# mattiagualtieri/multimodal-path-omic

Hardware: AMD Instinct MI355X
Metric: slides/sec (fwd+bwd) at 15k-patch bags (higher is better)
Workload: dtype bf16; 1 GPU; MCAT medium whole model fwd+bwd+Adam, 15000x1024 bf16 patch bag + 6x256 omic tokens per slide, ces loss; parallelism=dp1, resident_windows=2, launch=hipgraph(fwd+bwd+adam), setup_replays_before_warmup=40, training_state_rewound_every=48

## Files before the change

### include/mpo_hip.h

```cpp
#ifndef MPO_HIP_H
#define MPO_HIP_H
#include <stddef.h>
#include <stdint.h>

#define MPO_ABI_VERSION 14

#ifdef __cplusplus
extern "C" {
#endif

typedef struct ihipStream_t* mpo_stream_t;

enum { MPO_F32 = 0, MPO_BF16 = 1 };

typedef struct mpo_bag_plan {
    const int32_t* wg_start;
    int32_t n_wg;
    int32_t rows_per_wg;
} mpo_bag_plan;
int mpo_coattn_target_workgroups(void);
enum { MPO_ACT_NONE_ = 0, MPO_ACT_RELU_ = 1, MPO_ACT_ELU_ = 2, MPO_ACT_TANH_ = 3, MPO_ACT_SIGMOID_ = 4 };

int mpo_abi_version(void);
const char* mpo_last_error(void);
// ... 102 lines not shown
                        mpo_stream_t stream);

int mpo_key_projection(const void* hbag_bf16, int64_t rows, int embed, const float* w_k, const float* b_k, float* kbag,
                       mpo_stream_t stream);
size_t mpo_nacagat_saved_floats(int n_slides, int n_q, int embed);
size_t mpo_nacagat_workspace_bytes(int n_slides, int n_q, int embed, int max_rows, int total_rows);
int mpo_coattn_nacagat_forward(const void* kbag, int k_dtype, const void* hbag, int bag_dtype, const int32_t* cu_rows, int n_slides,
                               int total_rows, int max_rows, const float* query, int n_q, int embed,
                               const float* in_proj_weight, const float* in_proj_bias,
                               const float* out_proj_weight, const float* out_proj_bias,
                               float drop_p, uint64_t seed, uint64_t offset, const uint64_t* rng_epoch,
                               float* q_proj, float* out, float* attn_map, float* score_maps,
                               float* saved, const mpo_bag_plan* plan ,
                               void* workspace, size_t workspace_bytes, mpo_stream_t stream);
int mpo_coattn_nacagat_backward(const void* kbag, int k_dtype, const void* hbag, int bag_dtype,
                                const int32_t* cu_rows, int n_slides, int total_rows, int max_rows,
                                const float* query, int n_q, int embed,
                                const float* in_proj_weight, const float* in_proj_bias, const float* out_proj_weight,
                                float drop_p, uint64_t seed, uint64_t offset, const uint64_t* rng_epoch,
                                const float* saved, const float* score_maps, const float* attn_map,
                                const float* d_out, const float* d_attn_map, const float* d_q_proj,
                                float* d_query, int d_query_accumulate ,
                                void* d_kbag, int dk_dtype, float* d_kbag_colsum ,
                                void* d_hbag ,
                                float* d_ctx ,
                                float* d_in_proj_weight, float* d_in_proj_bias,
                                float* d_out_proj_weight, float* d_out_proj_bias, const mpo_bag_plan* plan ,
                                void* workspace, size_t workspace_bytes, mpo_stream_t stream);

int mpo_nacagat_patch_grad(const int32_t* cu_rows, int n_slides, int total_rows, int max_rows, int n_q, int embed,
                           const float* attn_map, const float* d_ctx, const void* addend_bf16, const void* hbag_bf16,
                           void* d_bag_bf16, float relu_gate, float* d_bias, const mpo_bag_plan* plan ,
                           void* workspace, size_t workspace_bytes, mpo_stream_t stream);

int mpo_nacagat_patch_grad_fused(const int32_t* cu_rows, int n_slides, int total_rows, int max_rows, int n_q, int embed,
                                 const float* attn_map, const float* d_ctx, const void* d_kbag_bf16, const float* w_k,
                                 const void* hbag_bf16, void* d_bag_bf16, float relu_gate, float* d_bias,
                                 const mpo_bag_plan* plan , void* workspace, size_t workspace_bytes,
                                 mpo_stream_t stream);


size_t mpo_encoder_saved_floats(int n_slides, int T, int d, int ff, int heads, int layers);
size_t mpo_encoder_workspace_bytes(int n_slides, int T, int d, int ff);
uint64_t mpo_encoder_rng_span(int n_slides, int T, int d, int ff, int layers);
int mpo_encoder_forward(const float* x, int n_branches, int n_slides, int T, int d, int ff, int heads, int layers,
                        const float* const* params, float drop_p, uint64_t seed, uint64_t offset, const uint64_t* rng_epoch,
                        float* y, float* saved, mpo_stream_t stream);
int mpo_encoder_backward(const float* x, int n_branches, int n_slides, int T, int d, int ff, int heads, int layers,
                         const float* const* params, float drop_p, uint64_t seed, uint64_t offset, const uint64_t* rng_epoch,
                         const float* saved, const float* dy, float* dx, float* const* grads,
                         void* workspace, size_t workspace_bytes, mpo_stream_t stream);

size_t mpo_bag_self_attention_saved_floats(int n_bags, int M, int d, int heads);
size_t mpo_bag_self_attention_workspace_bytes(int n_bags, int M, int d, int heads);
int mpo_set_bag_self_attention_bf16x3(int enabled);
int mpo_bag_self_attention_forward(const float* qkv, int n_bags, int M, int d, int heads, float drop_p, uint64_t seed, uint64_t offset,
                                   const uint64_t* rng_epoch, float* out, float* saved, float* attn_map, mpo_stream_t stream);
int mpo_bag_self_attention_backward(const float* qkv, const float* out, const float* saved, const float* d_out, int n_bags, int M, int d,
                                    int heads, float drop_p, uint64_t seed, uint64_t offset, const uint64_t* rng_epoch, float* d_qkv,
                                    void* workspace, size_t workspace_bytes, mpo_stream_t stream);

size_t mpo_gated_pool_saved_floats(int n_slides, int L, int d);
size_t mpo_gated_pool_workspace_bytes(int n_slides, int L, int d);
uint64_t mpo_gated_pool_rng_span(int n_slides, int L, int d);
int mpo_gated_pool_forward(const float* x, int n_branches, int n_slides, int L, int d, const float* const* params,
                           float head_drop_p, float rho_drop_p, uint64_t seed, uint64_t offset, const uint64_t* rng_epoch,
                           float* scores, float* h, int h_interleaved, float* saved, mpo_stream_t stream);
int mpo_gated_pool_backward(const float* x, int n_branches, int n_slides, int L, int d, const float* const* params,
                            float head_drop_p, float rho_drop_p, const float* saved, const float* h,
                            const float* dh, int h_interleaved, const float* d_scores_ext , float* dx,
                            float* const* grads,
                            void* workspace, size_t workspace_bytes, mpo_stream_t stream);

size_t mpo_fusion_head_saved_floats(int n_slides, int hidden, int dout, int n_classes);
size_t mpo_fusion_head_workspace_bytes(int n_slides, int hidden, int dout, int n_classes);
int mpo_fusion_head_forward(const float* hcat, int n_slides, int din, int hidden, int dout, int n_classes,
                            const float* const* params, float* hazards, float* survs, float* y, float* saved,
                            mpo_stream_t stream);
int mpo_fusion_head_backward(const float* hcat, int n_slides, int din, int hidden, int dout, int n_classes,
                             const float* const* params, const float* saved, const float* hazards,
                             const float* survs, const float* y, const float* d_hazards, const float* d_survs,
                             const float* d_y, float* d_hcat, float* const* grads,
                             void* workspace, size_t workspace_bytes, mpo_stream_t stream);

int mpo_survival_head_forward(const float* logits, int n_slides, int n_classes, float* hazards, float* survs, float* y,
                              mpo_stream_t stream);
int mpo_survival_head_backward(const float* hazards, const float* survs, const float* y, const float* d_hazards,
                               const float* d_survs, const float* d_y, int n_slides, int n_classes, float* d_logits,
                               mpo_stream_t stream);

int mpo_ces_loss_forward(const float* hazards, const float* survs, const int64_t* label, const float* censorship,
                         int n_slides, int n_classes, float alpha, float eps, float* loss, float* risk, mpo_stream_t stream);
int mpo_ces_loss_backward(const float* hazards, const float* survs, const int64_t* label, const float* censorship,
                          int n_slides, int n_classes, float alpha, float eps, const float* d_loss, int d_loss_is_scalar,
                          float* d_hazards, float* d_survs, mpo_stream_t stream);

size_t mpo_fusion_head_loss_saved_floats(int n_slides, int hidden, int dout, int n_classes);
int mpo_fusion_head_loss_forward(const float* hcat, int n_slides, int din, int hidden, int dout, int n_classes,
                                 const float* const* params, const int64_t* label, const float* censorship,
                                 const float* slide_weight, float alpha, float eps, float* hazards, float* survs, float* y,
                                 float* loss, float* risk , float* saved, mpo_stream_t stream);
int mpo_fusion_head_loss_backward(const float* hcat, int n_slides, int din, int hidden, int dout, int n_classes,
                                  const float* const* params, const float* saved, float* d_hcat, float* const* grads,
                                  void* workspace, size_t workspace_bytes, mpo_stream_t stream);

int mpo_sct_loss_forward(const float* y, const int64_t* label, const float* censorship, int n_slides, int n_classes,
                         float eps, float* loss, mpo_stream_t stream);
int mpo_sct_loss_backward(const float* y, const int64_t* label, const float* censorship, int n_slides, int n_classes,
                          float eps, const float* d_loss, int d_loss_is_scalar, float* d_y, mpo_stream_t stream);
int mpo_fusion_head_sct_loss_forward(const float* hcat, int n_slides, int din, int hidden, int dout, int n_classes,
                                     const float* const* params, const int64_t* label, const float* censorship,
                                     const float* slide_weight, float eps, float* hazards, float* survs, float* y,
                                     float* loss, float* risk , float* saved, mpo_stream_t stream);

int mpo_ge_head_loss_forward(const float* h, int n_bags, int d, int n_classes, const float* const* params,
                             const int64_t* label, float* y, float* loss, mpo_stream_t stream);
int mpo_ge_head_loss_backward(const float* h, int n_bags, int d, int n_classes, const float* const* params,
                              const int64_t* label, const float* d_loss, float* d_h, float* const* grads,
                              mpo_stream_t stream);

size_t mpo_cag_saved_floats(int rows, int hidden);
size_t mpo_cag_workspace_bytes(int rows, int hidden);
int mpo_cag_forward(const float* q, const float* q_hat, int rows, int dim, int hidden, const float* const* params,
                    float* c_out, float* saved, const float* residual ,
                    float* sum_out , mpo_stream_t stream);
int mpo_cag_backward(const float* q, const float* q_hat, int rows, int dim, int hidden, const float* const* params,
                     const float* saved, const float* c_out, const float* d_c, float* d_q, int d_q_accumulate, float* d_q_hat,
                     float* const* grads, void* workspace, size_t workspace_bytes, mpo_stream_t stream);

size_t mpo_omic_snn_saved_floats(int n_slides, int n_groups, int d);
size_t mpo_omic_snn_workspace_bytes(int n_slides, int n_groups, int d);
uint64_t mpo_omic_snn_rng_span(int n_slides, int n_groups, int d);
int mpo_omic_snn_forward(const float* const* x, const int* widths, int n_groups, int n_slides, int d,
                         const float* const* params, float drop_p, uint64_t seed, uint64_t offset,
                         const uint64_t* rng_epoch, float* g_bag, float* saved, mpo_stream_t stream);
int mpo_omic_snn_backward(const float* const* x, const int* widths, int n_groups, int n_slides, int d,
                          const float* const* params, float drop_p, uint64_t seed, uint64_t offset,
                          const uint64_t* rng_epoch, const float* g_bag, const float* saved, const float* d_g_bag,
                          float* const* grads, void* workspace, size_t workspace_bytes, mpo_stream_t stream);

int mpo_coattn_splits(int n_slides, int max_rows);
int mpo_coattn_fwd_bagpass(const void* bag, int bag_dtype, const int32_t* cu_rows, int n_slides, int embed,
                           const float* qk2, float* part_ml, float* part_ctx, float* raw_logits ,
                           int n_q, int max_rows, const mpo_bag_plan* plan , mpo_stream_t stream);
int mpo_nacagat_fwd_bagpass(const float* kbag, const int32_t* cu_rows, int n_slides, int embed, const float* qs2,
                            const float* tq, float* a_map, float* g_map, int n_q, int max_rows,
                            const mpo_bag_plan* plan , mpo_stream_t stream);
int mpo_coattn_bwd_bagpass(const void* bag, int bag_dtype, const int32_t* cu_rows, int n_slides, int embed,
                           const float* qk2, const float* lse2, const float* dctx, const float* delta,
                           const float* d_attn_map , void* d_bag, float* part_dqk,
                           int n_q, int max_rows, const mpo_bag_plan* plan , mpo_stream_t stream);

#include "mpo_bag_sample.h"

#ifdef __cplusplus
}
#endif
#endif
```

### multimodal_path_omic_amd/_lib.py

```python
from __future__ import annotations

import ctypes
import os
import re
from ctypes import c_char_p, c_float, c_int, c_int64, c_size_t, c_uint64, c_void_p

import torch

_HERE = os.path.dirname(os.path.abspath(__file__))
LIB_PATH = os.path.join(_HERE, "libmpo_hip.so")
HEADER_PATH = os.path.join(os.path.dirname(_HERE), "include", "mpo_hip.h")
COMPANION_HEADER_PATHS = [os.path.join(os.path.dirname(_HERE), "include", "mpo_bag_sample.h")]

_SCALARS = {"int": c_int, "int32_t": c_int, "int64_t": c_int64, "uint64_t": c_uint64, "size_t": c_size_t, "float": c_float,
            "mpo_stream_t": c_void_p}
_DECL = re.compile(r"^[ \t]*([\w \t*]+?)[ \t]*\b(mpo_\w+)[ \t]*\(([^()]*)\)\s*;", re.M)


def _ctype(entry: str, decl: str):
    if "*" in decl or decl.rstrip().endswith("]"):
        return c_void_p
    words = [w for w in decl.split() if w != "const"]
    if not 1 <= len(words) <= 2 or words[0] not in _SCALARS:
        raise RuntimeError(f"include/mpo_hip.h: {entry}: no ctypes type for '{' '.join(decl.split())}'")
    return _SCALARS[words[0]]


def parse_header(text: str):
    version = re.search(r"^[ \t]*#[ \t]*define[ \t]+MPO_ABI_VERSION[ \t]+(\d+)[ \t]*$", text, re.M)
    text = re.sub(r"/\*.*?\*/", " ", text, flags=re.S)
    text = re.sub(r"//[^\n]*|^[ \t]*#.*$", " ", text, flags=re.M)
    signatures, parsed = {}, set()
    for m in _DECL.finditer(text):
        ret, name, args = m.groups()
        parsed.add(m.start(2))
        if ret.replace("*", " * ").split() == ["const", "char", "*"]:
            res = c_char_p
        elif "*" in ret:
            raise RuntimeError(f"include/mpo_hip.h: {name}: no ctypes type for the return type '{ret.strip()}'")
        else:
            res = _ctype(name, ret)
        signatures[name] = (res, [] if args.strip() in ("", "void") else [_ctype(name, a) for a in args.split(",")])
    for m in re.finditer(r"\b(mpo_\w+)\s*\(", text):
        if m.start(1) not in parsed:
            raise RuntimeError(f"include/mpo_hip.h: {m.group(1)}: not a whole declaration: "
                               f"'{' '.join(text[m.start():m.start() + 120].split())}'")
    constants = {}
    for body in re.findall(r"\benum\s*\{([^}]*)\}", text):
        for item in body.split(","):
            m = re.fullmatch(r"\s*(MPO_\w+)\s*=\s*(\d+)\s*", item)
            if not m:
                raise RuntimeError(f"include/mpo_hip.h: enum item '{item.strip()}' is not NAME = integer")
            constants[m.group(1)] = int(m.group(2))
    return signatures, constants, int(version.group(1)) if version else None


def _read_header():
    if not os.path.exists(HEADER_PATH):
        raise RuntimeError(f"{HEADER_PATH} is missing: the package binds libmpo_hip.so from its public header and ships "
                           "with it (repository layout: include/ beside the package)")
    with open(HEADER_PATH) as f:
        signatures, constants, version = parse_header(f.read())
    if version is None or not signatures:
        raise RuntimeError(f"{HEADER_PATH}: no MPO_ABI_VERSION / no entry declarations found")
    return signatures, constants, version


def _read_companions():
    out = {}
    for path in COMPANION_HEADER_PATHS:
        if not os.path.exists(path):
            raise RuntimeError(f"{path} is missing: include/mpo_hip.h includes it and the package binds its entries")
        with open(path) as f:
            signatures, constants, version = parse_header(f.read())
        if not signatures or constants or version is not None:
            raise RuntimeError(f"{path}: a companion header declares entries only (no enum, no MPO_ABI_VERSION)")
        for name in signatures:
            if name in _signatures or name in out:
                raise RuntimeError(f"{path}: {name} is declared twice")
        out.update(signatures)
    return out


_signatures, _constants, ABI_VERSION = _read_header()
MPO_F32, MPO_BF16 = _constants["MPO_F32"], _constants["MPO_BF16"]
ACT = {k[len("MPO_ACT_"):-1].lower(): v for k, v in _constants.items() if k.startswith("MPO_ACT_")}
OPTIM = {k[len("MPO_OPTIM_"):].lower(): v for k, v in _constants.items() if k.startswith("MPO_OPTIM_")}
GEMM_ROUTE = {k[len("MPO_GEMM_ROUTE_"):].lower(): v for k, v in _constants.items() if k.startswith("MPO_GEMM_ROUTE_")}
_companion_signatures = _read_companions()


class BagPlanC(ctypes.Structure):
    _fields_ = [("wg_start", c_void_p), ("n_wg", ctypes.c_int32), ("rows_per_wg", ctypes.c_int32)]


_REBUILD = "run `python -c 'import __graft_entry__ as g; g.build()'`"
_lib = None


def exported_symbols():
    return list(_signatures)


def companion_symbols():
    return list(_companion_signatures)


def check_abi_version(found: int, expected: int):
    if found != expected:
        raise RuntimeError(f"{LIB_PATH} reports ABI version {found}, include/mpo_hip.h describes {expected}: the library is "
                           f"stale ({_REBUILD}). There is no CPU fallback.")


def lib():
    global _lib
    if _lib is None:
        if not os.path.exists(LIB_PATH):
            raise RuntimeError(
                f"{LIB_PATH} is missing: the HIP extension has not been built ({_REBUILD}). There is no CPU fallback.")
        handle = ctypes.CDLL(LIB_PATH)
        for name, (res, args) in {**_signatures, **_companion_signatures}.items():
            fn = getattr(handle, name)
            fn.restype = res
            fn.argtypes = args
        check_abi_version(handle.mpo_abi_version(), ABI_VERSION)
        _lib = handle
    return _lib


def call(name: str, *args):
    check(getattr(lib(), name)(*args), name)


def check(rc: int, what: str):
    if rc != 0:
        msg = lib().mpo_last_error()
        raise RuntimeError(f"{what} failed (rc={rc}): {msg.decode() if msg else '?'}")


def ptr(t):
    if t is None:
        return None
    if not t.is_cuda:
        raise RuntimeError("libmpo_hip operates on GPU tensors only (got a CPU tensor); there is no CPU fallback")
    if not t.is_contiguous():
        raise RuntimeError("libmpo_hip needs contiguous tensors")
    return t.data_ptr()


def ptr_array(tensors):
    arr = (c_void_p * len(tensors))()
    for i, t in enumerate(tensors):
        arr[i] = ptr(t)
    return arr


def stream_of(t):
    return torch.cuda.current_stream(t.device).cuda_stream


def bag_dtype_code(t):
    if t.dtype == torch.float32:
        return MPO_F32
    if t.dtype == torch.bfloat16:
        return MPO_BF16
    raise RuntimeError(f"bag dtype must be float32 or bfloat16, got {t.dtype}")
```

### multimodal_path_omic_amd/csrc/capi.hip

```cpp
#include <stdarg.h>
#include <stdio.h>
#include <stdlib.h>

#include <algorithm>

#include "../../include/mpo_hip.h"
#include "coattn_tile.h"
#include "mpo_common.h"
#include "mpo_kernels.h"
#include "mpo_layout.h"

static thread_local char g_err[512] = "";

void mpo_set_error(const char* fmt, ...) {
    va_list ap;
    va_start(ap, fmt);
    vsnprintf(g_err, sizeof(g_err), fmt, ap);
    va_end(ap);
}

template <typename T> struct K1Saved { T *qs, *qk2, *ctx, *attn, *lse2; };
template <class A> K1Saved<typename A::elem> k1_saved(A& a, size_t R, size_t E) {
    return {a.floats(R * E), a.floats(R * E), a.floats(R * E), a.floats(R * E), a.floats(R)};
}
// ... 448 lines not shown
            RC(mpo_launch_bag_outer_gated(reinterpret_cast<const float*>(static_cast<const char*>(kbag) + h * half_k), cu_rows,
                                          n_slides, EH, W.ds1_map, qth, W.dg_map, tqh, static_cast<char*>(d_kbag) + h * half_dk,
                                          dk_dtype == MPO_F32, W.part_cs, n_q, splits, stream));
        BagFinish f{};
        f.part_cs = d_kbag_colsum ? W.part_cs : nullptr; f.colsum = d_kbag_colsum ? d_kbag_colsum + h * EH : nullptr; f.cs_cols = EH;
        if (h == 0) {
            f.zero[0] = d_in_w + (size_t)E * E; f.n_zero[0] = E * E;
            if (d_kbag_colsum != d_in_b + E) { f.zero[1] = d_in_b + E; f.n_zero[1] = E; }
        }
        if (one_pass) { f.part[0] = W.part; f.out[0] = W.dqt; f.part[1] = W.part2; f.out[1] = W.dtq; f.n_red = 2; }
        RC(mpo_launch_bag_finish(f, n_slides, n_q, EH, splits, stream));
    }
    if (one_pass) RC(query_side());
    if (d_ctx == nullptr)
        for (int h = 0; h < NH; ++h)
            RC(mpo_launch_bag_outer(cu_rows, n_slides, EH, attn_map, NH > 1 ? hb[h] : dctx, nullptr, nullptr,
                                    static_cast<char*>(d_hbag) + h * half_h, f32, n_q, splits, stream));
    return 0;
}

struct K2PatchGrad {
    BagPlan splits;
    float* part_cs;
};
static int k2_patch_grad_begin(K2PatchGrad& pg, int n_slides, int max_rows, int embed, bool colsum, const mpo_bag_plan* plan_,
                               void* workspace, size_t workspace_bytes) {
    pg.splits = make_plan(plan_, n_slides, max_rows);
    RC(check_plan(pg.splits, n_slides));
    WsCarve ws(workspace, workspace_bytes);
    pg.part_cs = k2_patch_grad_ws(ws, plan_parts(pg.splits), embed, colsum);
    MPO_CHECK(ws.ok(), "nacagat patch grad: workspace too small (%zu bytes)", workspace_bytes);
    return 0;
}
static int k2_patch_grad_end(const K2PatchGrad& pg, float* d_bias, int embed, hipStream_t stream) {
    return d_bias ? mpo_launch_colsum(pg.part_cs, d_bias, (int)plan_parts(pg.splits), embed, embed, 0, stream) : 0;
}

int mpo_nacagat_patch_grad(const int32_t* cu_rows, int n_slides, int total_rows, int max_rows, int n_q, int embed,
                           const float* attn_map, const float* d_ctx, const void* addend_bf16, const void* hbag_bf16,
                           void* d_bag_bf16, float relu_gate, float* d_bias, const mpo_bag_plan* plan_,
                           void* workspace, size_t workspace_bytes, mpo_stream_t stream) {
    RC(check_common(MPO_BF16, n_slides, total_rows, max_rows, n_q, embed));
    MPO_CHECK(attn_map && d_ctx && addend_bf16 && hbag_bf16 && d_bag_bf16, "nacagat patch grad: null operand");
    MPO_CHECK(((reinterpret_cast<uintptr_t>(addend_bf16) | reinterpret_cast<uintptr_t>(hbag_bf16) |
                reinterpret_cast<uintptr_t>(d_bag_bf16)) & 15) == 0, "nacagat patch grad: bag operands must be 16-byte aligned");
    K2PatchGrad pg;
    RC(k2_patch_grad_begin(pg, n_slides, max_rows, embed, d_bias != nullptr, plan_, workspace, workspace_bytes));
    RC(mpo_launch_bag_outer_gate(cu_rows, n_slides, embed, attn_map, d_ctx, addend_bf16, hbag_bf16, d_bag_bf16, relu_gate,
                                 pg.part_cs, n_q, pg.splits, stream));
    return k2_patch_grad_end(pg, d_bias, embed, stream);
}

int mpo_nacagat_patch_grad_fused(const int32_t* cu_rows, int n_slides, int total_rows, int max_rows, int n_q, int embed,
                                 const float* attn_map, const float* d_ctx, const void* d_kbag_bf16, const float* w_k,
                                 const void* hbag_bf16, void* d_bag_bf16, float relu_gate, float* d_bias,
                                 const mpo_bag_plan* plan_, void* workspace, size_t workspace_bytes, mpo_stream_t stream) {
    RC(check_common(MPO_BF16, n_slides, total_rows, max_rows, n_q, embed));
    MPO_CHECK(attn_map && d_ctx && d_kbag_bf16 && w_k && hbag_bf16 && d_bag_bf16, "nacagat patch grad: null operand");
    MPO_CHECK(d_bag_bf16 != d_kbag_bf16, "nacagat patch grad (fused): d_bag must not alias d_kbag");
    MPO_CHECK(((reinterpret_cast<uintptr_t>(d_kbag_bf16) | reinterpret_cast<uintptr_t>(hbag_bf16) |
                reinterpret_cast<uintptr_t>(d_bag_bf16)) & 15) == 0, "nacagat patch grad: bag operands must be 16-byte aligned");
    K2PatchGrad pg;
    RC(k2_patch_grad_begin(pg, n_slides, max_rows, embed, d_bias != nullptr, plan_, workspace, workspace_bytes));
    RC(mpo_launch_k2_patch_grad(cu_rows, d_kbag_bf16, w_k, attn_map, d_ctx, hbag_bf16, d_bag_bf16, relu_gate, pg.part_cs, n_q, embed,
                                pg.splits, stream));
    return k2_patch_grad_end(pg, d_bias, embed, stream);
}

int mpo_coattn_fwd_bagpass(const void* bag, int bag_dtype, const int32_t* cu_rows, int n_slides, int embed,
                           const float* qk2, float* part_ml, float* part_ctx, float* raw_logits, int n_q, int max_rows,
                           const mpo_bag_plan* plan_, mpo_stream_t stream) {
    const BagPlan plan = make_plan(plan_, n_slides, max_rows);
    RC(check_plan(plan, n_slides));
    return mpo_launch_coattn_fwd_partial(bag, bag_dtype == MPO_F32, cu_rows, n_slides, embed, qk2, part_ml, part_ctx,
                                         raw_logits, n_q, plan, stream);
}
int mpo_map_block_dot(const float* a_map, const float* b_map, const int32_t* cu_rows, int n_slides, int n_q, float* out,
                      mpo_stream_t stream) {
    MPO_CHECK(a_map && b_map && cu_rows && out && n_slides >= 1 && n_q >= 1, "map block dot: bad argument");
    return mpo_launch_map_rowdot(a_map, b_map, cu_rows, out, n_slides, n_q, 0, stream);
}
int mpo_map_block_scale(const float* a_map, const float* scale, const int32_t* cu_rows, int n_slides, int n_q, float* out,
                        mpo_stream_t stream) {
    MPO_CHECK(a_map && scale && cu_rows && out && n_slides >= 1 && n_q >= 1, "map block scale: bad argument");
    return mpo_launch_map_block_scale(a_map, scale, cu_rows, out, n_slides, n_q, stream);
}
int mpo_key_projection(const void* hbag_bf16, int64_t rows, int embed, const float* w_k, const float* b_k, float* kbag,
                       mpo_stream_t stream) {
    MPO_CHECK(rows >= 1 && rows <= 0x7fffffff, "key projection: %lld rows out of range", (long long)rows);
    return mpo_launch_key_proj(hbag_bf16, w_k, b_k, kbag, (int)rows, embed, stream);
}
int mpo_nacagat_fwd_bagpass(const float* kbag, const int32_t* cu_rows, int n_slides, int embed, const float* qs2,
                            const float* tq, float* a_map, float* g_map, int n_q, int max_rows, const mpo_bag_plan* plan_,
                            mpo_stream_t stream) {
    const BagPlan plan = make_plan(plan_, n_slides, max_rows);
    RC(check_plan(plan, n_slides));
    return mpo_launch_bag_rowdot_gated(kbag, 1, cu_rows, n_slides, embed, qs2, tq, a_map, g_map, n_q, plan, stream);
}
int mpo_coattn_bwd_bagpass(const void* bag, int bag_dtype, const int32_t* cu_rows, int n_slides, int embed,
                           const float* qk2, const float* lse2, const float* dctx, const float* delta,
                           const float* d_attn_map, void* d_bag, float* part_dqk, int n_q, int max_rows,
                           const mpo_bag_plan* plan_, mpo_stream_t stream) {
    const BagPlan plan = make_plan(plan_, n_slides, max_rows);
    RC(check_plan(plan, n_slides));
    MPO_CHECK(delta, "coattn backward bag pass: delta is required here");
    return mpo_launch_coattn_bwd(bag, bag_dtype == MPO_F32, cu_rows, n_slides, embed, qk2, lse2, dctx, delta, nullptr, nullptr,
                                 d_attn_map, d_bag, part_dqk, nullptr, n_q, plan, 0.f, stream);
}

int mpo_patch_epilogue_forward(void* h_bf16, const float* bias, int64_t rows, int cols, float drop_p, uint64_t seed,
                               uint64_t offset, const uint64_t* rng_epoch, mpo_stream_t stream) {
    MPO_CHECK(h_bf16 && bias, "patch epilogue: null operand");
    MPO_CHECK(rows >= 0, "patch epilogue: %lld rows", (long long)rows);
    MPO_CHECK(((reinterpret_cast<uintptr_t>(h_bf16) | reinterpret_cast<uintptr_t>(bias)) & 15) == 0,
              "patch epilogue: h and bias must be 16-byte aligned");
    return mpo_launch_bias_relu_dropout_bf16(h_bf16, bias, (size_t)rows, cols, drop_p, seed, offset,
                                             reinterpret_cast<const unsigned long long*>(rng_epoch), stream);
}
int mpo_colsum_bf16(const void* x_bf16, float* out, int64_t rows, int cols, mpo_stream_t stream) {
    MPO_CHECK(x_bf16 && out, "bf16 column sum: null operand");
    MPO_CHECK(rows >= 0, "bf16 column sum: %lld rows", (long long)rows);
    MPO_CHECK((reinterpret_cast<uintptr_t>(x_bf16) & 15) == 0, "bf16 column sum: x must be 16-byte aligned (bf16 x 8 loads)");
    return mpo_launch_colsum_bf16(x_bf16, out, (size_t)rows, cols, stream);
}
size_t mpo_patch_epilogue_backward_workspace_bytes(int64_t n, int cols) { return one_block_workspace_bytes(patch_epilogue_bwd_floats(n, cols)); }
int mpo_patch_epilogue_backward(const void* h_bf16, const void* dy_bf16, void* g_bf16, int64_t n, int cols, float drop_p,
                                float* d_bias, void* workspace, size_t workspace_bytes, mpo_stream_t stream) {
    MPO_CHECK(h_bf16 && dy_bf16 && g_bf16, "patch epilogue backward: null operand");
    MPO_CHECK(((reinterpret_cast<uintptr_t>(h_bf16) | reinterpret_cast<uintptr_t>(dy_bf16) |
                reinterpret_cast<uintptr_t>(g_bf16)) & 15) == 0,
              "patch epilogue backward: h, dy and g must be 16-byte aligned (bf16 x 8 loads)");
    if (!d_bias) return mpo_launch_relu_dropout_bwd_bf16(h_bf16, dy_bf16, g_bf16, (size_t)n, drop_p, cols, nullptr, stream);
    WsCarve ws(workspace, workspace_bytes);
    float* part = ws.floats(patch_epilogue_bwd_floats(n, cols));
    MPO_CHECK(workspace && ws.ok(), "patch epilogue backward: workspace too small (%zu bytes)", workspace_bytes);
    RC(mpo_launch_relu_dropout_bwd_bf16(h_bf16, dy_bf16, g_bf16, (size_t)n, drop_p, cols, part, stream));
    return mpo_launch_colsum(part, d_bias, mpo_relu_dropout_bwd_blocks((size_t)n, 1), cols, cols, 0, stream);
}

size_t mpo_patch_weight_grad_workspace_bytes(int embed, int patch_dim) {
    return one_block_workspace_bytes(mpo_patch_wgrad_partial_floats(embed, patch_dim));
}
int mpo_patch_weight_grad(const void* g_bf16, const void* patches_bf16, int64_t total_rows, int embed, int patch_dim,
                          float* d_weight, int workgroups, void* workspace, size_t workspace_bytes, mpo_stream_t stream) {
    MPO_CHECK(g_bf16 && patches_bf16 && d_weight, "patch weight gradient: null argument");
    MPO_CHECK(total_rows >= 1 && total_rows < (int64_t)1 << 31, "patch weight gradient: %lld rows", (long long)total_rows);
    WsCarve ws(workspace, workspace_bytes);
    float* part = ws.floats(mpo_patch_wgrad_partial_floats(embed, patch_dim));
    MPO_CHECK(ws.ok(), "patch weight gradient: workspace too small (%zu bytes)", workspace_bytes);
    return mpo_launch_patch_wgrad(g_bf16, patches_bf16, total_rows, embed, patch_dim, part, d_weight, workgroups,
                                  static_cast<hipStream_t>(stream));
}

int mpo_adam_step_flat(float* params, const float* grads, float* exp_avg, float* exp_avg_sq, int64_t n, float lr,
                       float beta1, float beta2, float eps, float weight_decay, int step, const int32_t* step_dev,
                       mpo_stream_t stream) {
    MPO_CHECK(step >= 1 || step_dev, "adam: step counts from 1 (got %d)", step);
    return mpo_launch_adam_flat(params, grads, exp_avg, exp_avg_sq, (size_t)n, lr, beta1, beta2, eps, weight_decay,
                                step < 1 ? 1 : step, step_dev, stream);
}

int mpo_optim_step_flat(int algorithm, float* params, const float* grads, float* state1, float* state2, int64_t n, float lr,
                        const float* lr_dev, float beta1, float beta2, float eps, float weight_decay, float l1, int step,
                        const int32_t* step_dev, mpo_stream_t stream) {
    MPO_CHECK(algorithm >= MPO_OPTIM_ADAM && algorithm <= MPO_OPTIM_SGD, "flat optimiser: unknown algorithm %d", algorithm);
    MPO_CHECK(n >= 0, "flat optimiser: n = %lld", (long long)n);
    MPO_CHECK(params && grads, "flat optimiser: null parameter or gradient buffer");
    const bool stateful = algorithm != MPO_OPTIM_SGD;
    MPO_CHECK(!stateful || (state1 && state2), "flat optimiser: algorithm %d needs both state buffers", algorithm);
    const auto misaligned = [](const void* q) { return (reinterpret_cast<uintptr_t>(q) & 3u) != 0; };
    MPO_CHECK(!misaligned(params) && !misaligned(grads) && !misaligned(state1) && !misaligned(state2) && !misaligned(lr_dev) &&
              !misaligned(step_dev), "flat optimiser: buffers must be 4-byte aligned");
    const bool counted = algorithm == MPO_OPTIM_ADAM || algorithm == MPO_OPTIM_ADAMAX;
    MPO_CHECK(!counted || step >= 1 || step_dev, "flat optimiser: step counts from 1 (got %d)", step);
    return mpo_launch_optim_flat(algorithm, params, grads, state1, state2, (size_t)n, lr, lr_dev, beta1, beta2, eps,
                                 weight_decay, l1, step < 1 ? 1 : step, step_dev, static_cast<hipStream_t>(stream));
}
size_t mpo_abs_sum_flat_workspace_bytes(int64_t n) {
    return n < 0 ? 0 : mpo_abs_sum_partials((size_t)n) * sizeof(float);
}
int mpo_abs_sum_flat(const float* x, int64_t n, float* out, void* workspace, size_t workspace_bytes, mpo_stream_t stream) {
    MPO_CHECK(n >= 1, "abs sum: n = %lld", (long long)n);
    MPO_CHECK(x && out && workspace, "abs sum: null argument");
    MPO_CHECK((reinterpret_cast<uintptr_t>(x) & 3u) == 0 && (reinterpret_cast<uintptr_t>(out) & 3u) == 0 &&
              (reinterpret_cast<uintptr_t>(workspace) & 3u) == 0, "abs sum: pointers must be 4-byte aligned");
    MPO_CHECK(workspace_bytes >= mpo_abs_sum_flat_workspace_bytes(n), "abs sum: workspace too small (%zu bytes)",
              workspace_bytes);
    return mpo_launch_abs_sum(x, (size_t)n, static_cast<float*>(workspace), out, static_cast<hipStream_t>(stream));
}

int mpo_set_gemm_fast_path(int enabled) { return mpo_gemm_fast_path(enabled); }
int mpo_gemm_last_route(void) { return mpo_gemm_route_last(); }
int mpo_gemm_last_group_routes(void) { return mpo_gemm_route_group_take(); }
int mpo_set_coattn_bwd_two_wave(int enabled) { return mpo_coattn_bwd8_enable(enabled); }
int mpo_set_coattn_bwd_f32_vector(int enabled) { return mpo_coattn_bwd_f32_enable(enabled); }
int mpo_set_nacagat_one_pass_key_grad(int enabled) {
    const int was = g_k2_one_pass_key ? 1 : 0;
    g_k2_one_pass_key = enabled != 0;
    return was;
}

int mpo_step_counters_bump(uint64_t* rng_epoch, int32_t* adam_step, mpo_stream_t stream) {
    MPO_CHECK(rng_epoch || adam_step, "step counters: nothing to bump");
    return mpo_launch_counters_bump(reinterpret_cast<unsigned long long*>(rng_epoch), adam_step, static_cast<hipStream_t>(stream));
}

}
```

### multimodal_path_omic_amd/csrc/gemm_f32.hip

```cpp
#include "../../include/mpo_hip.h"
#include "mpo_common.h"
#include "mpo_kernels.h"
#include "gemm_f32_gate.h"

namespace {

constexpr int DB = 16;
constexpr int DMAXB = 8;
}
void mpo_direct_single_nb4(const GemmArgs& g, int layout, dim3 grid, hipStream_t stream);
void mpo_direct_single_nb8(const GemmArgs& g, int layout, dim3 grid, hipStream_t stream);
void mpo_direct_group_nb4(const GemmGroup& grp, dim3 grid, hipStream_t stream);
void mpo_direct_group_nb8(const GemmGroup& grp, dim3 grid, hipStream_t stream);
void mpo_fast_group(const GemmGroup& grp, int gate_classes, int nbmax, dim3 grid, hipStream_t stream);
void mpo_fast_single(const GemmArgs& g, int layout, int gate_classes, int nbmax, dim3 grid, hipStream_t stream);
void mpo_rows_single(const GemmArgs& g, int layout, int gate_class, hipStream_t stream);
int mpo_longk_single(const GemmArgs& g, int gate_class, hipStream_t stream);
namespace {
inline int direct_nbmax(int k) { return k <= 256 ? 4 : DMAXB; }
bool g_fast_path = true;
int g_last_route = MPO_GEMM_ROUTE_NONE;
int g_group_routes = 0;
inline bool aligned16(const void* p) { return (reinterpret_cast<uintptr_t>(p) & 15) == 0; }
inline int gate_class(const GemmArgs& g, bool need_aligned_gate) {
    const bool gate_ok = g.gate != nullptr && (!need_aligned_gate || aligned16(g.gate));
    switch (g.gate_mode) {
        case MPO_GATE_NONE: return 0;
        case MPO_GATE_RNG: return 2;
        case MPO_GATE_RELU: case MPO_GATE_ELU: case MPO_GATE_TANH: case MPO_GATE_SIGMOID: case MPO_GATE_MUL: return gate_ok ? 1 : -1;
        case MPO_GATE_ELU_ADROP: return gate_ok ? 3 : -1;
        default: return -1;
    }
}
inline int fast_class(const GemmArgs& g) {
    if (!g_fast_path) return -1;
    if (g.M <= 0 || g.N <= 0 || (g.M & 15) || (g.N & 15) || g.K < 16 || (g.K & 15)) return -1;
    if ((g.lda & 3) || (g.ldb & 3) || !aligned16(g.A) || !aligned16(g.B)) return -1;
    return gate_class(g, true);
}
inline int rows_class(const GemmArgs& g, int layout) {
    if (!g_fast_path || !(layout & 2) || g.M < 512 || (g.N & 63) || g.K < 64 || (g.K & 63) || g.bias_grad != nullptr) return -1;
    if ((g.lda & 3) || !aligned16(g.A)) return -1;
    if ((layout & 1) && ((g.ldb & 3) || !aligned16(g.B))) return -1;
    return gate_class(g, true);
}
inline int longk_class(const GemmArgs& g, int layout) {
    if (!g_fast_path || layout != 0 || g.K < 2048 || (g.M & 31) || (g.N & 63) || (g.lda & 3)) return -1;
    if (g.bias || g.mask || g.residual || g.act != MPO_ACT_NONE || g.drop_p > 0.f) return -1;
    return gate_class(g, false);
}
inline void launch_longk(const GemmArgs& g, int gate_class, hipStream_t stream) {
    if (int e = mpo_longk_single(g, gate_class, stream)) mpo_set_error("long-K weight gradient: zero-fill failed (hip error %d)", e);
}
void launch_direct_single(const GemmArgs& g, int layout, dim3 grid, hipStream_t stream) {
    const int rc = rows_class(g, layout);
    if (rc >= 0) { g_last_route = MPO_GEMM_ROUTE_ROWS; mpo_rows_single(g, layout, rc, stream); return; }
    const int lc = longk_class(g, layout);
    if (lc >= 0) { g_last_route = MPO_GEMM_ROUTE_LONGK; launch_longk(g, lc, stream); return; }
    const int fc = fast_class(g);
    if (fc >= 0) { g_last_route = MPO_GEMM_ROUTE_FAST; mpo_fast_single(g, layout, fc, direct_nbmax(g.K), grid, stream); return; }
    if (direct_nbmax(g.K) == 4) { g_last_route = MPO_GEMM_ROUTE_GENERAL_NB4; mpo_direct_single_nb4(g, layout, grid, stream); }
    else { g_last_route = MPO_GEMM_ROUTE_GENERAL_NB8; mpo_direct_single_nb8(g, layout, grid, stream); }
}
inline bool group_extent(const GemmGroup& grp, dim3& grid) {
    int mx = 0, nx = 0;
    for (int i = 0; i < grp.n; ++i) { mx = std::max(mx, grp.g[i].M); nx = std::max(nx, grp.g[i].N); }
    grid = dim3((nx + DB - 1) / DB, (mx + DB - 1) / DB, grp.n);
    return mx > 0 && nx > 0;
}
void launch_direct_group(const GemmGroup& all, dim3 grid, hipStream_t stream) {
    GemmGroup grp;
    grp.n = 0;
    for (int i = 0; i < all.n; ++i) {
        const int rc = rows_class(all.g[i], all.g[i].layout), lc = longk_class(all.g[i], all.g[i].layout);
        if (rc >= 0) { g_group_routes |= 1 << MPO_GEMM_ROUTE_ROWS; mpo_rows_single(all.g[i], all.g[i].layout, rc, stream); }
        else if (lc >= 0) { g_group_routes |= 1 << MPO_GEMM_ROUTE_LONGK; launch_longk(all.g[i], lc, stream); }
        else grp.g[grp.n++] = all.g[i];
    }
    if (grp.n == 0) return;
    if (grp.n != all.n) group_extent(grp, grid);
    int kmax = 0, classes = 0;
    bool fast = true;
    for (int i = 0; i < grp.n; ++i) {
        kmax = grp.g[i].K > kmax ? grp.g[i].K : kmax;
        const int fc = fast_class(grp.g[i]);
        fast = fast && fc >= 0;
        if (fc > 0) classes |= 1 << fc;
    }
    fast = fast && (classes & (classes - 1)) == 0;
    const size_t wgs = (size_t)grid.x * grid.y * grid.z;
    const int nb = (wgs > 1024 || direct_nbmax(kmax) == 4) ? 4 : DMAXB;
    g_group_routes |= 1 << (fast ? MPO_GEMM_ROUTE_FAST : nb == 4 ? MPO_GEMM_ROUTE_GENERAL_NB4 : MPO_GEMM_ROUTE_GENERAL_NB8);
    if (fast) { mpo_fast_group(grp, classes >> 3 ? 3 : classes >> 2 ? 2 : 1, nb, grid, stream); return; }
    if (nb == 4) mpo_direct_group_nb4(grp, grid, stream);
    else mpo_direct_group_nb8(grp, grid, stream);
}

__global__ __launch_bounds__(256)
void colsum_kernel(const float* __restrict__ x, float* __restrict__ out, int M, int N, int ld, int accumulate) {
    __shared__ float red[16][17];
    const int c = threadIdx.x & 15, rg = threadIdx.x >> 4;
    const int n = blockIdx.x * 16 + c;
    float s = 0.f;
    if (n < N)
        for (int m = rg; m < M; m += 16) s += x[(size_t)m * ld + n];
    red[rg][c] = s;
    __syncthreads();
    if (rg == 0 && n < N) {
        float t = 0.f;
#pragma unroll
        for (int k = 0; k < 16; ++k) t += red[k][c];
        out[n] = accumulate ? out[n] + t : t;
    }
}

}

int mpo_gemm_fast_path(int enabled) {
    const int was = g_fast_path ? 1 : 0;
    g_fast_path = enabled != 0;
    return was;
}

int mpo_gemm_route_last() { return g_last_route; }
int mpo_gemm_route_group_take() {
    const int was = g_group_routes;
    g_group_routes = 0;
    return was;
}

int mpo_launch_gemm(const GemmArgs& g, int a_kc, int b_kc, hipStream_t stream) {
    if (g.M <= 0 || g.N <= 0) return 0;
    MPO_CHECK(g.K > 0, "gemm: K must be positive (got %d)", g.K);
    dim3 dgrid((g.N + DB - 1) / DB, (g.M + DB - 1) / DB);
    launch_direct_single(g, 2 * (a_kc ? 1 : 0) + (b_kc ? 1 : 0), dgrid, stream);
    MPO_LAUNCH_CHECK();
    return 0;
}

static int launch_group(const char* what, GemmGroup grp, int layout, hipStream_t stream) {
    MPO_CHECK(grp.n >= 1 && grp.n <= 8, "%s: 1..8 members (got %d)", what, grp.n);
    for (int i = 0; i < grp.n; ++i) {
        MPO_CHECK(grp.g[i].K > 0, "%s: member %d has K = %d", what, i, grp.g[i].K);
        if (layout >= 0) grp.g[i].layout = layout;
        else MPO_CHECK(grp.g[i].layout >= 0 && grp.g[i].layout <= 3, "%s: member %d has layout %d", what, i, grp.g[i].layout);
    }
    dim3 dgrid;
    if (!group_extent(grp, dgrid)) return 0;
    launch_direct_group(grp, dgrid, stream);
    MPO_LAUNCH_CHECK();
    return 0;
}
int mpo_launch_gemm_group(const GemmGroup& grp, int a_kc, int b_kc, hipStream_t stream) {
    return launch_group("grouped gemm", grp, 2 * (a_kc ? 1 : 0) + (b_kc ? 1 : 0), stream);
}
int mpo_launch_gemm_mixed(const GemmGroup& grp, hipStream_t stream) { return launch_group("mixed grouped gemm", grp, -1, stream); }

int mpo_launch_colsum(const float* x, float* out, int M, int N, int ld, int accumulate, hipStream_t stream) {
    if (N <= 0) return 0;
    colsum_kernel<<<(N + 15) / 16, 256, 0, stream>>>(x, out, M, N, ld, accumulate);
    MPO_LAUNCH_CHECK();
    return 0;
}
```

### multimodal_path_omic_amd/csrc/gemm_f32_fast.h

```cpp
#pragma once
#include "gemm_f32_gate.h"

namespace {

constexpr int FB = 16;

struct FastLds {
    float part[4][256];
    float bsum[4][16];
};


template <bool KC>
__device__ __forceinline__ f32x4 fast_frag(const float* __restrict__ p, int ld, int mn, int k0) {
    if (KC) return *reinterpret_cast<const f32x4*>(p + (size_t)mn * ld + k0);
    f32x4 r;
#pragma unroll
    for (int j = 0; j < 4; ++j) r[j] = p[(size_t)(k0 + j) * ld + mn];
    return r;
}

template <bool A_KC, bool B_KC, int GC>
struct FastCtx {
    const GemmArgs& g;
    const GateFn& gf;
    int m, n, kq, lane;
    bool want_bsum;
    template <int NB>
    __device__ __forceinline__ void chunk(int kbase, f32x4& acc0, f32x4& acc1, float& bsum) const {
        f32x4 a[NB], b[NB], gv[NB];
#pragma unroll
        for (int u = 0; u < NB; ++u) {
            const int k0 = kbase + 16 * u + 4 * kq;
            a[u] = fast_frag<A_KC>(g.A, g.lda, m, k0);
            b[u] = fast_frag<B_KC>(g.B, g.ldb, n, k0);
            if (GC == 1 || GC == 3) gv[u] = fast_frag<A_KC>(gf.g, g.lda, m, k0);
        }
#pragma unroll
        for (int u = 0; u < NB; ++u) {
            const int k0 = kbase + 16 * u + 4 * kq;
            if (GC == 1) {
#pragma unroll
                for (int j = 0; j < 4; ++j) a[u][j] *= gf(gv[u][j], 0);
            } else if (GC >= 2) {
                if (A_KC) {
                    const uint64_t ctr = gf.off + (((size_t)m * g.lda + k0) >> 2);
                    const uint4 r = draw4x32((uint32_t)ctr, (uint32_t)(ctr >> 32), (uint32_t)gf.seed, (uint32_t)(gf.seed >> 32));
                    const uint32_t w[4] = {r.x, r.y, r.z, r.w};
#pragma unroll
                    for (int j = 0; j < 4; ++j) a[u][j] *= gf.with_word(GC == 3 ? gv[u][j] : 0.f, w[j]);
                } else {
                    const int lq = lane & 3;
                    const size_t idx_own = (size_t)(k0 + lq) * g.lda + (m & ~3);
                    const uint64_t ctr = gf.off + (idx_own >> 2);
                    const uint4 r = draw4x32((uint32_t)ctr, (uint32_t)(ctr >> 32), (uint32_t)gf.seed, (uint32_t)(gf.seed >> 32));
                    const uint32_t own[4] = {r.x, r.y, r.z, r.w};
                    uint32_t w[4];
#pragma unroll
                    for (int t = 0; t < 4; ++t) {
                        const int pick = lq ^ t;
                        const uint32_t send = pick == 0 ? own[0] : pick == 1 ? own[1] : pick == 2 ? own[2] : own[3];
                        const uint32_t got = (uint32_t)__shfl_xor((int)send, t);
#pragma unroll
                        for (int j = 0; j < 4; ++j) if (j == (lq ^ t)) w[j] = got;
                    }
#pragma unroll
                    for (int j = 0; j < 4; ++j) a[u][j] *= gf.with_word(GC == 3 ? gv[u][j] : 0.f, w[j]);
                }
            }
            if (want_bsum) bsum += (a[u][0] + a[u][1]) + (a[u][2] + a[u][3]);
            acc0 = __builtin_amdgcn_mfma_f32_16x16x4f32(a[u][0], b[u][0], acc0, 0, 0, 0);
            acc1 = __builtin_amdgcn_mfma_f32_16x16x4f32(a[u][1], b[u][1], acc1, 0, 0, 0);
            acc0 = __builtin_amdgcn_mfma_f32_16x16x4f32(a[u][2], b[u][2], acc0, 0, 0, 0);
            acc1 = __builtin_amdgcn_mfma_f32_16x16x4f32(a[u][3], b[u][3], acc1, 0, 0, 0);
        }
    }
};

template <bool A_KC, bool B_KC, int GC, int NBMAX>
__device__ __forceinline__ void gemm_f32_fast_body(const GemmArgs& g, FastLds& lds) {
    if ((int)blockIdx.y * FB >= g.M || (int)blockIdx.x * FB >= g.N) return;
    const int tid = threadIdx.x, lane = tid & 63, wave = __builtin_amdgcn_readfirstlane(tid >> 6);
    const int m0 = blockIdx.y * FB, n0 = blockIdx.x * FB;
    const int i16 = lane & 15, kq = lane >> 4;
    GateFn gf;
    gf.g = g.gate; gf.mode = g.gate_mode; gf.p = g.gate_p; gf.seed = g.gate_seed;
    gf.off = epoch_offset(g.gate_off, g.rng_epoch);
    gf.inv_keep = g.gate_p > 0.f ? 1.0f / (1.0f - g.gate_p) : 1.0f;
    const bool want_bsum = g.bias_grad != nullptr && blockIdx.x == 0;

    const int erow = tid >> 4, ecol = tid & 15;
    const size_t eo = (size_t)(m0 + erow) * g.ldc + n0 + ecol;
    const float e_bias = g.bias ? g.bias[n0 + ecol] : 0.f;
    const float e_mask = g.mask ? g.mask[eo] : 1.0f;
    const float e_res = g.residual ? g.residual[eo] : 0.f;
    const float e_old = g.accumulate ? g.C[eo] : 0.f;
    float e_keep = 1.0f;
    if (g.drop_p > 0.f) {
        const unsigned long long doff = epoch_offset(g.drop_off, g.rng_epoch);
        e_keep = dropout_keep(g.drop_seed, doff, eo, g.drop_p, g.alpha_dropout ? 1.0f : 1.0f / (1.0f - g.drop_p));
    }

    const int kw = ((g.K + 63) >> 6) << 4;
    const int kbeg = wave * kw;
    const int nkb = max(0, min(kw, g.K - kbeg)) >> 4;
    f32x4 acc0 = {0.f, 0.f, 0.f, 0.f}, acc1 = acc0;
    float bsum = 0.f;
    FastCtx<A_KC, B_KC, GC> cx{g, gf, m0 + i16, n0 + i16, kq, lane, want_bsum};
    int kb = 0;
    for (; kb + NBMAX <= nkb; kb += NBMAX) cx.template chunk<NBMAX>(kbeg + 16 * kb, acc0, acc1, bsum);
    const int rem = nkb - kb;
    if (rem >= 4) { cx.template chunk<4>(kbeg + 16 * kb, acc0, acc1, bsum); kb += 4; }
    switch (nkb - kb) {
        case 3: cx.template chunk<3>(kbeg + 16 * kb, acc0, acc1, bsum); break;
        case 2: cx.template chunk<2>(kbeg + 16 * kb, acc0, acc1, bsum); break;
        case 1: cx.template chunk<1>(kbeg + 16 * kb, acc0, acc1, bsum); break;
        default: break;
    }
#pragma unroll
    for (int r = 0; r < 4; ++r) lds.part[wave][(4 * kq + r) * 16 + i16] = acc0[r] + acc1[r];
    if (want_bsum) {
        bsum += __shfl_xor(bsum, 16);
        bsum += __shfl_xor(bsum, 32);
        if (lane < 16) lds.bsum[wave][lane] = bsum;
    }
    __syncthreads();
    {
        float v = (lds.part[0][tid] + lds.part[1][tid]) + (lds.part[2][tid] + lds.part[3][tid]);
        v = (v + e_bias) * g.alpha;
        v = apply_act(v, g.act);
        if (g.drop_p > 0.f) {
            if (g.alpha_dropout) v = alpha_drop_a(g.drop_p) * (e_keep != 0.f ? v : kAlphaPrime) + alpha_drop_b(g.drop_p);
            else v *= e_keep;
        }
        v = v * e_mask + e_res + e_old;
        g.C[eo] = v;
    }
    if (want_bsum && tid < FB)
        g.bias_grad[m0 + tid] = (lds.bsum[0][tid] + lds.bsum[1][tid]) + (lds.bsum[2][tid] + lds.bsum[3][tid]);
}

template <bool A_KC, bool B_KC, int GCL, int NBMAX>
__device__ __forceinline__ void gemm_f32_fast_member(const GemmArgs& g, FastLds& lds) {
    if (g.gate_mode == MPO_GATE_NONE) gemm_f32_fast_body<A_KC, B_KC, 0, NBMAX>(g, lds);
    else gemm_f32_fast_body<A_KC, B_KC, GCL, NBMAX>(g, lds);
}

template <int GCL, int NBMAX>
__global__ __launch_bounds__(256) __attribute__((amdgpu_waves_per_eu((GCL == 2 && NBMAX == 4) ? 6 : 1, 8)))
void gemm_f32_fast_group_kernel(GemmGroup grp) {
    __shared__ FastLds lds;
    const GemmArgs& g = grp.g[blockIdx.z];
    switch (g.layout) {
        case 3: gemm_f32_fast_member<true, true, GCL, NBMAX>(g, lds); break;
        case 2: gemm_f32_fast_member<true, false, GCL, NBMAX>(g, lds); break;
        case 1: gemm_f32_fast_member<false, true, GCL, NBMAX>(g, lds); break;
        default: gemm_f32_fast_member<false, false, GCL, NBMAX>(g, lds); break;
    }
}
template <bool A_KC, bool B_KC, int GCL, int NBMAX>
__global__ __launch_bounds__(256)
void gemm_f32_fast_single_kernel(GemmArgs g) {
    __shared__ FastLds lds;
    gemm_f32_fast_member<A_KC, B_KC, GCL, NBMAX>(g, lds);
}

}
```

### multimodal_path_omic_amd/csrc/mpo_kernels.h

```cpp
#pragma once
#include <hip/hip_runtime.h>
#include <stddef.h>

#include <stdint.h>
enum { MPO_ACT_NONE = 0, MPO_ACT_RELU = 1, MPO_ACT_ELU = 2, MPO_ACT_TANH = 3, MPO_ACT_SIGMOID = 4 };
enum { MPO_GATE_NONE = 0, MPO_GATE_RELU = 1, MPO_GATE_ELU = 2, MPO_GATE_TANH = 3, MPO_GATE_SIGMOID = 4,
       MPO_GATE_RNG = 5, MPO_GATE_MUL = 6, MPO_GATE_ELU_ADROP = 7 };

struct GemmArgs {
    const float* A = nullptr;
    const float* B = nullptr;
    float* C = nullptr;
    const float* bias = nullptr;
    const float* residual = nullptr;
    const float* mask = nullptr;
    int M = 0, N = 0, K = 0;
    int lda = 0, ldb = 0, ldc = 0;
    float alpha = 1.0f;
    int act = MPO_ACT_NONE;
    int accumulate = 0;
    int alpha_dropout = 0;
    float drop_p = 0.f;
    uint64_t drop_seed = 0, drop_off = 0;
    const float* gate = nullptr;
    int gate_mode = MPO_GATE_NONE;
    float gate_p = 0.f;
    uint64_t gate_seed = 0, gate_off = 0;
    float* bias_grad = nullptr;
    const unsigned long long* rng_epoch = nullptr;
    int layout = 3;
};

struct DropSpec {
    float p = 0.f;
    uint64_t seed = 0, off = 0;
    const unsigned long long* epoch = nullptr;
};
struct GateSpec {
    const float* g = nullptr;
    int mode = MPO_GATE_NONE;
    float p = 0.f;
    uint64_t seed = 0, off = 0;
    const unsigned long long* epoch = nullptr;
};

int mpo_launch_gemm(const GemmArgs& g, int a_kc, int b_kc, hipStream_t stream);
struct GemmGroup {
    GemmArgs g[8];
    int n = 0;
};
int mpo_launch_gemm_group(const GemmGroup& grp, int a_kc, int b_kc, hipStream_t stream);
int mpo_launch_gemm_mixed(const GemmGroup& grp, hipStream_t stream);
int mpo_launch_colsum(const float* x, float* out, int M, int N, int ld, int accumulate, hipStream_t stream);

inline GemmArgs mpo_args_fwd(const float* x, const float* w, const float* b, float* y, int R, int I, int O,
                             float alpha, int act, const float* residual = nullptr, DropSpec drop = DropSpec()) {
    GemmArgs g;
    g.A = x; g.B = w; g.C = y; g.bias = b; g.residual = residual;
    g.M = R; g.N = O; g.K = I; g.lda = I; g.ldb = I; g.ldc = O; g.alpha = alpha; g.act = act;
    g.drop_p = drop.p; g.drop_seed = drop.seed; g.drop_off = drop.off; g.rng_epoch = drop.epoch;
    g.layout = 3;
    return g;
}
inline int mpo_linear_fwd(const float* x, const float* w, const float* b, float* y, int R, int I, int O,
                          float alpha, int act, hipStream_t s, const float* residual = nullptr,
                          DropSpec drop = DropSpec()) {
    return mpo_launch_gemm(mpo_args_fwd(x, w, b, y, R, I, O, alpha, act, residual, drop), 1, 1, s);
}
inline GemmArgs mpo_args_bwd_input(const float* dy, const float* w, float* dx, int R, int I, int O, float alpha,
                                   int accumulate, GateSpec gate = GateSpec()) {
    GemmArgs g;
    g.A = dy; g.B = w; g.C = dx;
    g.M = R; g.N = I; g.K = O; g.lda = O; g.ldb = I; g.ldc = I; g.alpha = alpha; g.accumulate = accumulate;
    g.gate = gate.g; g.gate_mode = gate.mode; g.gate_p = gate.p; g.gate_seed = gate.seed; g.gate_off = gate.off;
    g.rng_epoch = gate.epoch;
    g.layout = 2;
    return g;
}
inline int mpo_linear_bwd_input(const float* dy, const float* w, float* dx, int R, int I, int O, float alpha,
                                int accumulate, hipStream_t s, GateSpec gate = GateSpec()) {
    return mpo_launch_gemm(mpo_args_bwd_input(dy, w, dx, R, I, O, alpha, accumulate, gate), 1, 0, s);
}
inline GemmArgs mpo_args_bwd_weight(const float* dy, const float* x, float* dw, float* db, int R, int I, int O,
                                    float alpha, GateSpec gate = GateSpec()) {
    GemmArgs g;
    g.A = dy; g.B = x; g.C = dw;
    g.M = O; g.N = I; g.K = R; g.lda = O; g.ldb = I; g.ldc = I; g.alpha = alpha;
    g.gate = gate.g; g.gate_mode = gate.mode; g.gate_p = gate.p; g.gate_seed = gate.seed; g.gate_off = gate.off;
    g.rng_epoch = gate.epoch;
    g.bias_grad = db;
    g.layout = 0;
    return g;
}
inline int mpo_linear_bwd_weight(const float* dy, const float* x, float* dw, float* db, int R, int I, int O,
                                 float alpha, hipStream_t s, GateSpec gate = GateSpec()) {
    return mpo_launch_gemm(mpo_args_bwd_weight(dy, x, dw, db, R, I, O, alpha, gate), 0, 0, s);
}
inline int mpo_linear_bwd_pair(const GemmArgs& dx, const GemmArgs& dw, hipStream_t s) {
    GemmGroup grp;
    grp.g[0] = dx; grp.g[1] = dw; grp.n = 2;
    return mpo_launch_gemm_mixed(grp, s);
}
inline int mpo_gemm_together(hipStream_t s, const GemmArgs& a, const GemmArgs& b, const GemmArgs* c = nullptr,
                             const GemmArgs* d = nullptr) {
    GemmGroup grp;
    grp.g[0] = a; grp.g[1] = b; grp.n = 2;
    if (c) grp.g[grp.n++] = *c;
    if (d) grp.g[grp.n++] = *d;
    return mpo_launch_gemm_mixed(grp, s);
}

struct BagPlan;
extern "C" int mpo_coattn_splits(int n_slides, int max_rows);
int mpo_launch_pack_patch_weight(const float* w, void* out, int embed, int patch_dim, hipStream_t stream);
int mpo_launch_patch_fc_fwd(const void* x, const void* w_packed, const float* bias, const int* cu, void* h_out, int embed, int patch_dim,
                            float drop_p, unsigned long long seed, unsigned long long offset, const unsigned long long* epoch,
                            const BagPlan& plan, hipStream_t stream);
int mpo_launch_coattn_fwd_partial(const void* bag, int bag_f32, const int* cu, int n_slides, int embed,
                                  const float* qk2, float* part_ml, float* part_ctx, float* s_out,
                                  int n_q, const BagPlan& plan, hipStream_t stream);
int mpo_launch_coattn_combine(const float* part_ml, const float* part_ctx, float* ctx, float* lse2,
                              int n_slides, int n_q, int embed, const BagPlan& plan, hipStream_t stream);
int mpo_launch_coattn_normalize(float* a, const float* lse2, const int* cu, int n_slides, int n_q, int max_rows,
                                float drop_p, unsigned long long seed, unsigned long long offset, hipStream_t stream);
int mpo_launch_coattn_bwd(const void* bag, int bag_f32, const int* cu, int n_slides, int embed,
                          const float* qk2, const float* lse2, const float* dctx, const float* delta ,
                          const float* ctx, const float* a_map, const float* da_map,
                          void* dbag, float* part_dqk, float* part_colsum , int n_q, const BagPlan& plan,
                          float relu_gate, hipStream_t stream);
bool mpo_coattn_bwd8_covers(int bag_f32, int embed, int n_q, const float* da_map);
int mpo_coattn_bwd_f32_enable(int enabled);
bool mpo_coattn_bwd_f32_covers(int bag_f32, int embed, int n_q, const float* da_map);
int mpo_launch_coattn_bwd_f32(const void* bag, const int* cu, const float* qk2, const float* lse2, const float* dctx,
                              const float* delta, const float* ctx, const float* da_map, void* dbag, float* part_dqk,
                              float* part_colsum, int n_q, const BagPlan& plan, hipStream_t stream);
int mpo_coattn_bwd8_enable(int enabled);
int mpo_launch_coattn_bwd8(const void* bag, const int* cu, const float* qk2, const float* lse2, const float* dctx,
                           const float* delta, const float* ctx, void* dbag, float* part_dqk, float* part_colsum, int n_q,
                           const BagPlan& plan, float relu_gate, hipStream_t stream);
size_t mpo_patch_fc_f32_workspace_floats();
size_t mpo_patch_wgrad_f32_workspace_floats();
int mpo_launch_patch_fc_f32(const float* x, const float* w, const float* bias, float* h, long long total_rows, int embed,
                            int patch_dim, float drop_p, unsigned long long seed, unsigned long long offset,
                            const unsigned long long* epoch, float x_scale, float* ws, hipStream_t stream);
int mpo_launch_patch_wgrad_f32(const float* dh, const float* hbag, const float* x, long long total_rows, int embed, int patch_dim,
                               float gate, float* d_weight, float* d_bias, float* ws, hipStream_t stream);
int mpo_launch_k2_patch_grad(const int* cu, const void* dk_bf16, const float* w_k, const float* amap, const float* dctx,
                             const void* hbag_bf16, void* out_bf16, float gate, float* part_colsum, int n_q, int embed,
                             const BagPlan& plan, hipStream_t stream);
int mpo_gemm_fast_path(int enabled);
int mpo_gemm_route_last();
int mpo_gemm_route_group_take();
size_t mpo_patch_wgrad_partial_floats(int embed, int patch_dim);
int mpo_launch_patch_wgrad(const void* g_bf16, const void* x_bf16, int64_t total_rows, int embed, int patch_dim, float* part,
                           float* d_weight, int workgroups, hipStream_t stream);
struct BagFinish {
    const float* part[2];
    float* out[2];
    int n_red;
    const float* part_cs;
    float* colsum;
    int cs_cols;
    float* zero[2];
    int n_zero[2];
};
int mpo_launch_bag_finish(const BagFinish& f, int n_slides, int n_q, int embed, const BagPlan& plan, hipStream_t stream);
int mpo_launch_coattn_bwd_reduce(const float* part_dqk, float* dqk, int n_slides, int n_q, int embed, const BagPlan& plan,
                                 hipStream_t stream);
int mpo_launch_rowdot(const float* a, const float* b, float* out, int rows, int cols, hipStream_t stream);
int mpo_launch_map_block_scale(const float* a_map, const float* scale, const int* cu, float* out, int n_slides, int n_q,
                               hipStream_t stream);
int mpo_launch_map_rowdot(const float* a_map, const float* da_map, const int* cu, float* delta, int n_slides, int n_q,
                          int accumulate, hipStream_t stream);

int mpo_launch_bag_rowdot(const void* bag, int bag_f32, const int* cu, int n_slides, int embed, const float* r,
                          float* map, float alpha, int n_q, const BagPlan& plan, hipStream_t stream);
int mpo_launch_bag_colacc(const void* bag, int bag_f32, const int* cu, int n_slides, int embed, const float* wmap,
                          float* part, int n_q, const BagPlan& plan, hipStream_t stream);
int mpo_launch_bag_outer(const int* cu, int n_slides, int embed, const float* w1, const float* z1, const float* w2,
                         const float* z2, void* dx, int out_f32, int n_q, const BagPlan& plan, hipStream_t stream);
int mpo_launch_gated_softmax_fwd(const float* amap_a, const float* gmap, const int* cu, float* out_map, float* lse2,
                                 float* asum, int n_slides, int n_q, float drop_p, unsigned long long seed,
                                 unsigned long long offset, const unsigned long long* epoch, hipStream_t stream);
int mpo_launch_gated_softmax_bwd(const float* amap_a, const float* gmap, const int* cu, const float* lse2,
                                 const float* dasum, const float* d_ext, float* da_map, float* dg_map, int n_slides,
                                 int n_q, float drop_p, unsigned long long seed, unsigned long long offset,
                                 const unsigned long long* epoch, hipStream_t stream);
int mpo_launch_qprep(const float* q, float* qt, float* qs2, float* tq, int n, float c_nat, hipStream_t stream);
int mpo_launch_qprep_bwd(const float* dqt, const float* dtq, const float* tq, const float* d_ext, float* dq, int n,
                         float c_nat, hipStream_t stream);
int mpo_launch_row_scaled_bias(float* y, const float* s, const float* bias, int rows, int cols, hipStream_t stream);

constexpr int kMaxBranches = 4;
struct LnBranches {
    const float* w[kMaxBranches] = {};
    const float* b[kMaxBranches] = {};
    float* dw[kMaxBranches] = {};
    float* db[kMaxBranches] = {};
    int rows_per_branch = 0, n = 0;
};
int mpo_launch_ln_fwd_br(const float* x, const LnBranches& p, float* y, float* stats, int rows, int d, float eps, hipStream_t s);
int mpo_launch_ln_bwd_br(const float* dy, const float* x, const float* stats, const LnBranches& p, float* dx, int rows, int d,
                         int accumulate, int what, hipStream_t s);
int mpo_launch_ln_bwd_params_only(const float* dy, const float* x, const float* stats, float* dw, float* db, int rows, int d,
                                  hipStream_t s);
constexpr int kSmallAttnMaxT = 16;
// ... 95 lines not shown
```

### multimodal_path_omic_amd/csrc/patch_wgrad.hip

```cpp
#include "coattn_tile.h"
#include "mpo_kernels.h"

namespace {

constexpr int WG_E = 256;
constexpr int WG_CB = 256;
constexpr int WG_BK = 32;
constexpr int WG_STAGES = 4;
constexpr int WG_TILE = WG_BK * 512;
constexpr int WG_STAGE = 2 * WG_TILE;
constexpr int WG_LDS = WG_STAGES * WG_STAGE;
constexpr int WG_WAVES = 8;
constexpr int WG_WGS = 256;

__device__ __forceinline__ void wait_vm(int n) {
    switch (n) {
        case 0: __builtin_amdgcn_s_waitcnt(0x0F70); break;
        case 4: __builtin_amdgcn_s_waitcnt(0x0F74); break;
        default: __builtin_amdgcn_s_waitcnt(0x0F78); break;
    }
}

__global__ __launch_bounds__(WG_WAVES * 64, 1)
void patch_wgrad_kernel(const __bf16* __restrict__ g, const __bf16* __restrict__ x, int total_rows, int patch_dim,
                        int g_dim,
                        int e_rows,
                        int rows_per_range, float* __restrict__ part) {
    using G = TileGeom<WG_E>;
    __shared__ __attribute__((aligned(1024))) char lds[WG_LDS];
    const int lane = threadIdx.x & 63;
    const int wave = __builtin_amdgcn_readfirstlane(threadIdx.x >> 6);
    const int n_cb = patch_dim < WG_CB ? 1 : patch_dim / WG_CB;
    const int xcd = blockIdx.x & 7, slot = blockIdx.x >> 3;
    const int rr = xcd + 8 * (slot / n_cb), cb = slot % n_cb;
    const int rb = min(total_rows, rr * rows_per_range), re = min(total_rows, rb + rows_per_range);
    const int n_chunks = (re - rb + WG_BK - 1) / WG_BK;

    const bool x_tile = wave >= 4;
    const char* src_base = x_tile ? reinterpret_cast<const char*>(x) + (size_t)cb * WG_CB * 2 : reinterpret_cast<const char*>(g);
    const size_t src_row = x_tile ? (size_t)patch_dim * 2 : (size_t)g_dim * 2;
    const int cmask = x_tile ? (patch_dim < WG_CB ? patch_dim / 8 - 1 : 31) : e_rows / 8 - 1;
    const unsigned src_row32 = (unsigned)src_row;
    auto issue = [&](int chunk) {
        char* stage = lds + (chunk % WG_STAGES) * WG_STAGE + (x_tile ? WG_TILE : 0);
#pragma unroll
        for (int i = 0; i < 4; ++i) {
            const int k = 4 * (wave & 3) + i;
            const int r = 2 * k + (lane >> 5), cs = lane & 31;
            const int c = (cs ^ ((r & 7) << 1)) & cmask;
            const int grow = min(rb + chunk * WG_BK + r, total_rows - 1);
            const unsigned off = (unsigned)grow * src_row32 + (unsigned)(c * 16);
            const unsigned dst = (unsigned)(uintptr_t)(__attribute__((address_space(3))) char*)(stage + k * 1024);
#pragma clang diagnostic push
#pragma clang diagnostic ignored "-Winline-asm"
            asm volatile("s_mov_b32 m0, %2\n\ts_nop 0\n\tglobal_load_lds_dwordx4 %0, %1"
                         :: "v"(off), "s"(src_base), "s"(dst) : "memory", "m0");
#pragma clang diagnostic pop
        }
    };

    const int wm = wave & 3, wn = wave >> 2;
    f32x4 acc[4][8];
#pragma unroll
    for (int i = 0; i < 4; ++i)
#pragma unroll
        for (int j = 0; j < 8; ++j) acc[i][j] = f32x4{0.f, 0.f, 0.f, 0.f};

    auto arrive = [&](int m) {
        wait_vm(4 * min(WG_STAGES - 2, n_chunks - 1 - m));
        asm volatile("" ::: "memory");
        char* stage = lds + (m % WG_STAGES) * WG_STAGE;
        if (!x_tile && rb + (m + 1) * WG_BK > re) {
#pragma unroll
            for (int i = 0; i < 4; ++i) {
                const int k = 4 * (wave & 3) + i;
                const int r = 2 * k + (lane >> 5);
                if (rb + m * WG_BK + r >= re)
                    *reinterpret_cast<f32x4*>(stage + k * 1024 + lane * 16) = f32x4{0.f, 0.f, 0.f, 0.f};
            }
        }
        asm volatile("s_waitcnt lgkmcnt(0)\n\ts_barrier" ::: "memory");
        if (m + WG_STAGES - 1 < n_chunks) issue(m + WG_STAGES - 1);
    };
    auto load_frags = [&](int m, bf16x8 (&fa)[4], bf16x8 (&fb)[8]) {
        const char* gt = lds + (m % WG_STAGES) * WG_STAGE;
        const char* xt = gt + WG_TILE;
#pragma unroll
        for (int i = 0; i < 4; ++i) fa[i] = col_frag<WG_E>(gt, 4 * wm + i, lane);
#pragma unroll
        for (int j = 0; j < 8; ++j) fb[j] = col_frag<WG_E>(xt, 8 * wn + j, lane);
    };
    auto mma = [&](const bf16x8 (&fa)[4], const bf16x8 (&fb)[8]) {
#pragma unroll
        for (int j = 0; j < 8; ++j)
#pragma unroll
            for (int i = 0; i < 4; ++i) acc[i][j] = mfma_bf16(fa[i], fb[j], acc[i][j]);
    };

    for (int c = 0; c < min(WG_STAGES - 1, n_chunks); ++c) issue(c);
    bf16x8 pa[4], pb[8], qa[4], qb[8];
    if (n_chunks > 0) {
        arrive(0);
        load_frags(0, pa, pb);
    }
    int n = 0;
    auto half = [&](int m, bf16x8 (&la)[4], bf16x8 (&lb)[8], const bf16x8 (&ca)[4], const bf16x8 (&cb_)[8]) {
        __builtin_amdgcn_s_waitcnt(0x0F78);
        asm volatile("s_waitcnt lgkmcnt(0)\n\ts_barrier" ::: "memory");
        load_frags(m, la, lb);
        mma(ca, cb_);
        issue(m + WG_STAGES - 1);
#pragma unroll
        for (int k = 0; k < 24; ++k) {
            __builtin_amdgcn_sched_group_barrier(0x008, 1, 0);
            __builtin_amdgcn_sched_group_barrier(0x100, 1, 0);
        }
        __builtin_amdgcn_sched_group_barrier(0x008, 8, 0);
    };
    for (; n + 5 < n_chunks; n += 2) {
        half(n + 1, qa, qb, pa, pb);
        half(n + 2, pa, pb, qa, qb);
    }
    for (; n < n_chunks; n += 2) {
        if (n + 1 < n_chunks) {
            arrive(n + 1);
            load_frags(n + 1, qa, qb);
        }
        mma(pa, pb);
        if (n + 1 < n_chunks) {
            if (n + 2 < n_chunks) {
                arrive(n + 2);
                load_frags(n + 2, pa, pb);
            }
            mma(qa, qb);
        }
    }
    if (64 * wm >= e_rows || 128 * wn >= patch_dim) return;
    float* out = part + ((size_t)rr * e_rows) * patch_dim + (size_t)cb * WG_CB;
#pragma unroll
    for (int i = 0; i < 4; ++i)
#pragma unroll
        for (int j = 0; j < 8; ++j)
#pragma unroll
            for (int r = 0; r < 4; ++r)
                out[(size_t)(16 * (4 * wm + i) + 4 * (lane >> 4) + r) * patch_dim + 16 * (8 * wn + j) + (lane & 15)] = acc[i][j][r];
}

__global__ __launch_bounds__(256)
void patch_wgrad_reduce_kernel(const float* __restrict__ part, float* __restrict__ out, int n4, int n_parts, int accumulate) {
    const int i = blockIdx.x * 256 + threadIdx.x;
    if (i >= n4) return;
    f32x4 a = {0.f, 0.f, 0.f, 0.f};
    if (accumulate) a = *reinterpret_cast<const f32x4*>(out + (size_t)i * 4);
#pragma unroll 8
    for (int s = 0; s < n_parts; ++s) a += *reinterpret_cast<const f32x4*>(part + ((size_t)s * n4 + i) * 4);
    *reinterpret_cast<f32x4*>(out + (size_t)i * 4) = a;
}

}

size_t mpo_patch_wgrad_partial_floats(int embed, int patch_dim) {
    const int n_cb = patch_dim / WG_CB > 0 ? patch_dim / WG_CB : 1;
    return (size_t)(WG_WGS / n_cb) * (embed < WG_E ? embed : WG_E) * patch_dim;
}

int mpo_launch_patch_wgrad(const void* g, const void* x, int64_t total_rows, int embed, int patch_dim, float* part, float* d_weight,
                           int workgroups, hipStream_t stream) {
    MPO_CHECK((embed == 128 || embed == 256 || embed == 512) &&
              (patch_dim == 128 || (patch_dim >= WG_CB && patch_dim % WG_CB == 0 && (256 % (patch_dim / WG_CB)) == 0)),
              "patch weight gradient: built for embed in {128, 256, 512} and patch_dim in {128, 256, 512, 1024, 2048} (got %d, %d)", embed, patch_dim);
    MPO_CHECK(total_rows >= 1, "patch weight gradient: no rows");
    MPO_CHECK(((reinterpret_cast<uintptr_t>(g) | reinterpret_cast<uintptr_t>(x)) & 15) == 0, "patch weight gradient: operands must be 16-byte aligned");
    const int n_cb = patch_dim < WG_CB ? 1 : patch_dim / WG_CB;
    MPO_CHECK(workgroups == 0 || (workgroups >= 8 * n_cb && workgroups <= WG_WGS && workgroups % (8 * n_cb) == 0),
              "patch weight gradient: workgroups must be 0 or a multiple of %d up to %d (got %d)", 8 * n_cb, WG_WGS, workgroups);
    const int ranges = (workgroups ? workgroups : WG_WGS) / n_cb;
    const int e_rows = embed < WG_E ? embed : WG_E;
    const int wide = patch_dim > embed ? patch_dim : embed;
    const int64_t seg_rows = ((((int64_t)1 << 32) - 1) / ((int64_t)wide * 2)) / WG_BK * WG_BK;
    const __bf16* gb = static_cast<const __bf16*>(g);
    const __bf16* xb = static_cast<const __bf16*>(x);
    for (int64_t s0 = 0; s0 < total_rows; s0 += seg_rows) {
        const int rows = (int)(total_rows - s0 < seg_rows ? total_rows - s0 : seg_rows);
        const int rpr = ((rows + ranges - 1) / ranges + WG_BK - 1) / WG_BK * WG_BK;
        for (int c0 = 0; c0 < embed; c0 += WG_E) {
            patch_wgrad_kernel<<<ranges * n_cb, WG_WAVES * 64, 0, stream>>>(gb + (size_t)s0 * embed + c0, xb + (size_t)s0 * patch_dim, rows, patch_dim,
                                                                          embed, e_rows, rpr, part);
            MPO_LAUNCH_CHECK();
            const int n4 = e_rows * patch_dim / 4;
            patch_wgrad_reduce_kernel<<<(n4 + 255) / 256, 256, 0, stream>>>(part, d_weight + (size_t)c0 * patch_dim, n4, ranges, s0 > 0);
            MPO_LAUNCH_CHECK();
        }
    }
    return 0;
}
```

### multimodal_path_omic_amd/csrc/tail_api.hip

```cpp
#include <algorithm>
#include <vector>

#include "../../include/mpo_hip.h"
#include "mpo_common.h"
#include "mpo_kernels.h"
#include "mpo_layout.h"

namespace {

using SavedCount = Count<kPad64>;

inline DropSpec stream_of(float p, uint64_t seed, uint64_t base, uint64_t stride, int k, const uint64_t* epoch) {
    DropSpec d;
    d.p = p; d.seed = seed; d.off = base + stride * (uint64_t)k;
    d.epoch = reinterpret_cast<const unsigned long long*>(epoch);
    return d;
}
inline GateSpec gate(const float* g, int mode, float p = 0.f) {
    GateSpec s;
    s.g = g; s.mode = mode; s.p = p;
    return s;
}
inline GateSpec gate_rng(DropSpec d) {
    GateSpec s;
    s.mode = d.p > 0.f ? MPO_GATE_RNG : MPO_GATE_NONE; s.p = d.p; s.seed = d.seed; s.off = d.off; s.epoch = d.epoch;
    return s;
}

#define PAIR(dxa, dwa) RC(mpo_linear_bwd_pair((dxa), (dwa), stream))

enum { P_INW, P_INB, P_OUTW, P_OUTB, P_L1W, P_L1B, P_L2W, P_L2B, P_N1W, P_N1B, P_N2W, P_N2B, P_PER_LAYER };

template <typename T> struct EncLayerSaved { T *qkv, *psave, *o, *s1, *st1, *x1, *f, *s2, *st2, *x2; };
template <typename C>
void enc_carve(C& c, EncLayerSaved<typename C::elem>* out, int B, int T, int d, int ff, int H) {
    const size_t R = (size_t)B * T;
    EncLayerSaved<typename C::elem> s;
    s.qkv = c.floats(R * 3 * d);
    s.psave = c.floats(T <= kSmallAttnMaxT ? (size_t)B * 2 * H * T * T : mpo_bag_sa_saved_floats(B, T, d, H));
    s.o = c.floats(R * d);
    s.s1 = c.floats(R * d); s.st1 = c.floats(2 * R); s.x1 = c.floats(R * d); s.f = c.floats(R * ff);
    s.s2 = c.floats(R * d); s.st2 = c.floats(2 * R); s.x2 = c.floats(R * d);
    if (out) *out = s;
}
struct EncLayerWs { float *ds2, *df, *dx1, *ds1, *dob, *dqkv, *din, *sa; };
template <typename C>
void enc_bwd_ws(C& c, EncLayerWs* W, int layers, size_t R, size_t d, size_t ff, size_t sa_floats) {
    for (int l = layers - 1; l >= 0; --l)
        W[l] = {c.floats(R * d), c.floats(R * ff), c.floats(R * d), c.floats(R * d), c.floats(R * d), c.floats(R * 3 * d),
                l == 0 ? nullptr : c.floats(R * d), sa_floats ? c.floats(sa_floats) : nullptr};
}
inline uint64_t enc_stream_stride(int B, int T, int d, int ff) {
    const uint64_t R = (uint64_t)B * T;
    const uint64_t m = R * (uint64_t)(ff > 3 * d ? ff : 3 * d);
    return m / 4 + 2;
}

template <typename T> struct PoolSaved { T *a, *b, *ab, *w, *hpool; };
template <class A> PoolSaved<typename A::elem> pool_saved(A& c, size_t B, size_t L, size_t d) {
    const size_t R = B * L;
    return {c.floats(R * d), c.floats(R * d), c.floats(R * d), c.floats(R), c.floats(B * d)};
}
struct PoolWs { float *dhpool, *dscores, *dab, *da, *db; };
template <class A> PoolWs pool_ws(A& c, size_t B, size_t L, size_t d) {
    const size_t R = B * L;
    return {c.floats(B * d), c.floats(R), c.floats(R * d), c.floats(R * d), c.floats(R * d)};
}
inline uint64_t pool_stream_stride(uint64_t B, uint64_t L, uint64_t d) { return B * L * d / 4 + 2 + kMaxBranches; }

template <typename T> struct HeadSaved { T *z1, *z2, *logits, *dlogits; };
template <class A> HeadSaved<typename A::elem> head_saved(A& c, size_t B, size_t hidden, size_t dout, size_t n_classes, bool with_loss) {
    return {c.floats(B * hidden), c.floats(B * dout), c.floats(B * n_classes), with_loss ? c.floats(B * n_classes) : nullptr};
}
struct HeadWs { float *dlogits, *dz2, *dz1; };
template <class A> HeadWs head_ws(A& c, size_t B, size_t hidden, size_t dout, size_t n_classes) {
    return {c.floats(B * n_classes), c.floats(B * dout), c.floats(B * hidden)};
}

template <typename T> struct CagSaved { T *u1, *u2, *u3, *t1, *t3, *g, *e, *m, *sg, *se; };
template <class A> CagSaved<typename A::elem> cag_saved(A& c, size_t rows, size_t hidden) {
    const size_t n = rows * hidden;
    return {c.floats(n), c.floats(n), c.floats(n), c.floats(n), c.floats(n), c.floats(n), c.floats(n), c.floats(n),
            c.floats(2 * rows), c.floats(2 * rows)};
}
struct CagWs { float *dm, *dG, *dE, *ds12, *ds3; };
template <class A> CagWs cag_ws(A& c, size_t rows, size_t hidden) {
    const size_t n = rows * hidden;
    return {c.floats(n), c.floats(n), c.floats(n), c.floats(n), c.floats(n)};
}

template <class A> std::vector<typename A::elem*> snn_blocks(A& c, int n_groups, size_t n_slides, size_t d) {
    std::vector<typename A::elem*> b(n_groups > 0 ? n_groups : 0);
    for (auto& p : b) p = c.floats(n_slides * d);
    return b;
}
inline uint64_t snn_stream_stride(uint64_t n_slides, uint64_t n_groups, uint64_t d) { return n_slides * n_groups * d / 4 + 2; }

inline DropSpec drop_br(DropSpec d, int br, size_t elems_per_branch) { d.off += (uint64_t)br * ((elems_per_branch + 3) / 4); return d; }
inline GateSpec gate_rng_br(DropSpec d, int br, size_t elems_per_branch) { return gate_rng(drop_br(d, br, elems_per_branch)); }
inline int launch_in_groups(const std::vector<GemmArgs>& list, int a_kc, int b_kc, hipStream_t stream) {
    for (size_t i0 = 0; i0 < list.size(); i0 += 8) {
        GemmGroup grp;
        for (size_t i = i0; i < list.size() && i < i0 + 8; ++i) grp.g[grp.n++] = list[i];
        RC(mpo_launch_gemm_group(grp, a_kc, b_kc, stream));
    }
    return 0;
}
struct GroupBuilder {
    GemmGroup g;
    int add(const GemmArgs& a) {
        if (g.n >= 8) { mpo_set_error("grouped gemm: more than 8 members"); return 1; }
        g.g[g.n++] = a;
        return 0;
    }
    int launch(hipStream_t s) { return g.n ? mpo_launch_gemm_mixed(g, s) : 0; }
};
template <class MkDx, class MkDw> int launch_pairs(int n_branches, hipStream_t stream, MkDx&& mk_dx, MkDw&& mk_dw) {
    GroupBuilder g;
    for (int br = 0; br < n_branches; ++br) {
        RC(g.add(mk_dx(br)));
        RC(g.add(mk_dw(br)));
    }
    return g.launch(stream);
}
}

extern "C" {

size_t mpo_encoder_saved_floats(int n_slides, int T, int d, int ff, int heads, int layers) {
    SavedCount c;
    for (int l = 0; l < layers; ++l) enc_carve(c, nullptr, n_slides, T, d, ff, heads);
    return c.n_floats();
}
size_t mpo_encoder_workspace_bytes(int n_slides, int T, int d, int ff) {
    size_t sa = 0;
    for (int H = 1; H <= d && T > kSmallAttnMaxT; ++H)
        if (d % H == 0) sa = std::max(sa, mpo_bag_sa_bwd_floats(n_slides, T, d, H));
    WsCount c;
    EncLayerWs W[8];
    enc_bwd_ws(c, W, 8, (size_t)n_slides * T, d, ff, sa);
    return c.workspace_bytes();
}
uint64_t mpo_encoder_rng_span(int n_slides, int T, int d, int ff, int layers) {
    return enc_stream_stride(n_slides, T, d, ff) * 4 * (uint64_t)layers;
}

int mpo_encoder_forward(const float* x, int n_branches, int n_slides, int T, int d, int ff, int heads, int layers,
                        const float* const* params, float drop_p, uint64_t seed, uint64_t offset, const uint64_t* rng_epoch,
                        float* y, float* saved, mpo_stream_t stream) {
    MPO_CHECK(n_slides >= 1 && layers >= 1 && d % heads == 0, "encoder: bad geometry (slides %d, layers %d, d %d, heads %d)",
              n_slides, layers, d, heads);
    MPO_CHECK(n_branches >= 1 && n_branches <= kMaxBranches, "encoder: 1..%d branches (got %d)", kMaxBranches, n_branches);
    MPO_CHECK(drop_p <= 0.f || T > kSmallAttnMaxT || (uint64_t)heads * T <= (uint64_t)(ff > 3 * d ? ff : 3 * d),
              "encoder: heads * T = %d * %d exceeds max(ff, 3 d) = %d: the attention dropout stream would overlap the next one",
              heads, T, ff > 3 * d ? ff : 3 * d);
    if (T <= kSmallAttnMaxT) RC(mpo_check_mha_small(T, d, heads));
    const int NB = n_branches, R = n_slides * T, RT = NB * R, BT = NB * n_slides;
    const uint64_t stride = enc_stream_stride(BT, T, d, ff);
    Carve<kPad64> c(saved);
    const float* in = x;
    for (int l = 0; l < layers; ++l) {
        EncLayerSaved<float> S;
        enc_carve(c, &S, BT, T, d, ff, heads);
        const uint64_t base = offset + stride * 4 * (uint64_t)l;
        const DropSpec d0 = stream_of(drop_p, seed, base, stride, 0, rng_epoch), d1 = stream_of(drop_p, seed, base, stride, 1, rng_epoch),
                       d2 = stream_of(drop_p, seed, base, stride, 2, rng_epoch), d3 = stream_of(drop_p, seed, base, stride, 3, rng_epoch);
        float* out = (l == layers - 1) ? y : S.x2;
        auto P = [&](int br, int i) { return params[((size_t)br * layers + l) * P_PER_LAYER + i]; };
        LnBranches n1, n2;
        n1.n = n2.n = NB; n1.rows_per_branch = n2.rows_per_branch = R;
        for (int br = 0; br < NB; ++br) { n1.w[br] = P(br, P_N1W); n1.b[br] = P(br, P_N1B); n2.w[br] = P(br, P_N2W); n2.b[br] = P(br, P_N2B); }
        const size_t Rd = (size_t)R * d, Rf = (size_t)R * ff, Rq = (size_t)R * 3 * d;
        GroupBuilder q, o, f1, f2;
        for (int br = 0; br < NB; ++br) {
            RC(q.add(mpo_args_fwd(in + br * Rd, P(br, P_INW), P(br, P_INB), S.qkv + br * Rq, R, d, 3 * d, 1.0f, MPO_ACT_NONE)));
            RC(o.add(mpo_args_fwd(S.o + br * Rd, P(br, P_OUTW), P(br, P_OUTB), S.s1 + br * Rd, R, d, d, 1.0f, MPO_ACT_NONE,
                                  in + br * Rd, drop_br(d1, br, Rd))));
            RC(f1.add(mpo_args_fwd(S.x1 + br * Rd, P(br, P_L1W), P(br, P_L1B), S.f + br * Rf, R, d, ff, 1.0f, MPO_ACT_RELU, nullptr,
                                   drop_br(d2, br, Rf))));
            RC(f2.add(mpo_args_fwd(S.f + br * Rf, P(br, P_L2W), P(br, P_L2B), S.s2 + br * Rd, R, ff, d, 1.0f, MPO_ACT_NONE,
                                   S.x1 + br * Rd, drop_br(d3, br, Rd))));
        }
        RC(q.launch(stream));
        if (T <= kSmallAttnMaxT) RC(mpo_launch_mha_small_fwd(S.qkv, S.o, S.psave, BT, T, d, heads, d0.p, d0.seed, d0.off, d0.epoch, stream));
        else RC(mpo_launch_bag_sa_fwd(S.qkv, BT, T, d, heads, d0.p, d0.seed, d0.off, d0.epoch, S.o, S.psave, nullptr, stream));
        RC(o.launch(stream));
        RC(mpo_launch_ln_fwd_br(S.s1, n1, S.x1, S.st1, RT, d, 1e-5f, stream));
        RC(f1.launch(stream));
        RC(f2.launch(stream));
        RC(mpo_launch_ln_fwd_br(S.s2, n2, out, S.st2, RT, d, 1e-5f, stream));
        in = out;
    }
    return 0;
}

int mpo_encoder_backward(const float* x, int n_branches, int n_slides, int T, int d, int ff, int heads, int layers,
                         const float* const* params, float drop_p, uint64_t seed, uint64_t offset, const uint64_t* rng_epoch,
                         const float* saved, const float* dy, float* dx, float* const* grads,
                         void* workspace, size_t workspace_bytes, mpo_stream_t stream) {
    MPO_CHECK(n_branches >= 1 && n_branches <= kMaxBranches, "encoder: 1..%d branches (got %d)", kMaxBranches, n_branches);
    const int NB = n_branches, R = n_slides * T, RT = NB * R, BT = NB * n_slides;
    const uint64_t stride = enc_stream_stride(BT, T, d, ff);
    MPO_CHECK(layers <= 8, "encoder: at most 8 layers (got %d)", layers);
    EncLayerSaved<const float> S[8];
    Carve<kPad64, const float> c(saved);
    for (int l = 0; l < layers; ++l) enc_carve(c, &S[l], BT, T, d, ff, heads);
    WsCarve ws(workspace, workspace_bytes);
    EncLayerWs W[8];
    enc_bwd_ws(ws, W, layers, RT, d, ff, T <= kSmallAttnMaxT ? 0 : mpo_bag_sa_bwd_floats(BT, T, d, heads));
    MPO_CHECK(ws.ok(), "encoder backward: workspace too small (%zu bytes)", workspace_bytes);
    const float* dcur = dy;
    const size_t Rd = (size_t)R * d, Rf = (size_t)R * ff, Rq = (size_t)R * 3 * d;
    for (int l = layers - 1; l >= 0; --l) {
        float *ds2 = W[l].ds2, *df = W[l].df, *dx1 = W[l].dx1, *ds1 = W[l].ds1, *dob = W[l].dob, *dqkv = W[l].dqkv;
        float* din = l == 0 ? dx : W[l].din;
        auto P = [&](int br, int i) { return params[((size_t)br * layers + l) * P_PER_LAYER + i]; };
        auto G = [&](int br, int i) { return grads[((size_t)br * layers + l) * P_PER_LAYER + i]; };
        const float* in = l == 0 ? x : S[l - 1].x2;
        const uint64_t base = offset + stride * 4 * (uint64_t)l;
        const DropSpec d1 = stream_of(drop_p, seed, base, stride, 1, rng_epoch), d3 = stream_of(drop_p, seed, base, stride, 3, rng_epoch);
        LnBranches n1, n2;
        n1.n = n2.n = NB; n1.rows_per_branch = n2.rows_per_branch = R;
        for (int br = 0; br < NB; ++br) {
            n1.w[br] = P(br, P_N1W); n1.dw[br] = G(br, P_N1W); n1.db[br] = G(br, P_N1B);
            n2.w[br] = P(br, P_N2W); n2.dw[br] = G(br, P_N2W); n2.db[br] = G(br, P_N2B);
        }
        auto pairs = [&](auto&& mk_dx, auto&& mk_dw) { return launch_pairs(NB, stream, mk_dx, mk_dw); };
        RC(mpo_launch_ln_bwd_br(dcur, S[l].s2, S[l].st2, n2, ds2, RT, d, 0, 3, stream));
        RC(pairs([&](int br) { return mpo_args_bwd_input(ds2 + br * Rd, P(br, P_L2W), df + br * Rf, R, ff, d, 1.0f, 0, gate_rng_br(d3, br, Rd)); },
                 [&](int br) { return mpo_args_bwd_weight(ds2 + br * Rd, S[l].f + br * Rf, G(br, P_L2W), G(br, P_L2B), R, ff, d, 1.0f, gate_rng_br(d3, br, Rd)); }));
        RC(pairs([&](int br) {
                     GemmArgs g;
                     g.A = df + br * Rf; g.B = P(br, P_L1W); g.C = dx1 + br * Rd; g.residual = ds2 + br * Rd;
                     g.M = R; g.N = d; g.K = ff; g.lda = ff; g.ldb = d; g.ldc = d;
                     g.gate = S[l].f + br * Rf; g.gate_mode = MPO_GATE_RELU; g.gate_p = drop_p; g.layout = 2;
                     return g;
                 },
                 [&](int br) { return mpo_args_bwd_weight(df + br * Rf, S[l].x1 + br * Rd, G(br, P_L1W), G(br, P_L1B), R, d, ff, 1.0f,
                                                          gate(S[l].f + br * Rf, MPO_GATE_RELU, drop_p)); }));
        RC(mpo_launch_ln_bwd_br(dx1, S[l].s1, S[l].st1, n1, ds1, RT, d, 0, 3, stream));
        RC(pairs([&](int br) { return mpo_args_bwd_input(ds1 + br * Rd, P(br, P_OUTW), dob + br * Rd, R, d, d, 1.0f, 0, gate_rng_br(d1, br, Rd)); },
                 [&](int br) { return mpo_args_bwd_weight(ds1 + br * Rd, S[l].o + br * Rd, G(br, P_OUTW), G(br, P_OUTB), R, d, d, 1.0f, gate_rng_br(d1, br, Rd)); }));
        if (T <= kSmallAttnMaxT) {
            RC(mpo_launch_mha_small_bwd(S[l].qkv, S[l].psave, dob, dqkv, BT, T, d, heads, stream));
        } else {
            const DropSpec d0 = stream_of(drop_p, seed, base, stride, 0, rng_epoch);
            RC(mpo_launch_bag_sa_bwd(S[l].qkv, S[l].o, S[l].psave, dob, BT, T, d, heads, d0.p, d0.seed, d0.off, d0.epoch, dqkv, W[l].sa, stream));
        }
        RC(pairs([&](int br) {
                     GemmArgs g;
                     g.A = dqkv + br * Rq; g.B = P(br, P_INW); g.C = din + br * Rd; g.residual = ds1 + br * Rd;
                     g.M = R; g.N = d; g.K = 3 * d; g.lda = 3 * d; g.ldb = d; g.ldc = d; g.layout = 2;
                     return g;
                 },
                 [&](int br) { return mpo_args_bwd_weight(dqkv + br * Rq, in + br * Rd, G(br, P_INW), G(br, P_INB), R, d, 3 * d, 1.0f); }));
        dcur = din;
    }
    return 0;
}

size_t mpo_bag_self_attention_saved_floats(int n_bags, int M, int d, int heads) { return mpo_bag_sa_saved_floats(n_bags, M, d, heads); }
size_t mpo_bag_self_attention_workspace_bytes(int n_bags, int M, int d, int heads) { return mpo_bag_sa_bwd_floats(n_bags, M, d, heads) * sizeof(float); }
int mpo_set_bag_self_attention_bf16x3(int enabled) { return mpo_bag_sa_set_bf16x3(enabled); }
int mpo_bag_self_attention_forward(const float* qkv, int n_bags, int M, int d, int heads, float drop_p, uint64_t seed, uint64_t offset,
                                   const uint64_t* rng_epoch, float* out, float* saved, float* attn_map, mpo_stream_t stream) {
    MPO_CHECK(qkv && out && saved, "bag self-attention: NULL buffer");
    return mpo_launch_bag_sa_fwd(qkv, n_bags, M, d, heads, drop_p, seed, offset, (const unsigned long long*)rng_epoch, out, saved,
                                 attn_map, (hipStream_t)stream);
}
int mpo_bag_self_attention_backward(const float* qkv, const float* out, const float* saved, const float* d_out, int n_bags, int M, int d,
                                    int heads, float drop_p, uint64_t seed, uint64_t offset, const uint64_t* rng_epoch, float* d_qkv,
                                    void* workspace, size_t workspace_bytes, mpo_stream_t stream) {
    MPO_CHECK(qkv && out && saved && d_out && d_qkv, "bag self-attention backward: NULL buffer");
    MPO_CHECK(workspace && workspace_bytes >= mpo_bag_self_attention_workspace_bytes(n_bags, M, d, heads),
              "bag self-attention backward: workspace too small (%zu bytes)", workspace_bytes);
    return mpo_launch_bag_sa_bwd(qkv, out, saved, d_out, n_bags, M, d, heads, drop_p, seed, offset, (const unsigned long long*)rng_epoch,
                                 d_qkv, static_cast<float*>(workspace), (hipStream_t)stream);
}

size_t mpo_gated_pool_saved_floats(int n_slides, int L, int d) { SavedCount c; pool_saved(c, n_slides, L, d); return c.n_floats(); }
size_t mpo_gated_pool_workspace_bytes(int n_slides, int L, int d) { WsCount c; pool_ws(c, n_slides, L, d); return c.workspace_bytes(); }
uint64_t mpo_gated_pool_rng_span(int n_slides, int L, int d) { return 3 * pool_stream_stride(n_slides, L, d); }

static bool pool_fuses_scorer(int n_branches, int L, int d) { return n_branches <= 2 && L <= 64 && d <= 1024; }

int mpo_gated_pool_forward(const float* x, int n_branches, int n_slides, int L, int d, const float* const* params,
                           float head_drop_p, float rho_drop_p, uint64_t seed, uint64_t offset, const uint64_t* rng_epoch,
                           float* scores, float* h, int h_interleaved, float* saved, mpo_stream_t stream) {
    MPO_CHECK(n_branches >= 1 && n_branches <= kMaxBranches, "gated pool: 1..%d branches (got %d)", kMaxBranches, n_branches);
    MPO_CHECK(!h_interleaved || (d & 3) == 0, "gated pool: interleaved h needs d %% 4 == 0 (got %d)", d);
    const int NB = n_branches, R = n_slides * L, RT = NB * R, BT = NB * n_slides;
    const uint64_t stride = pool_stream_stride(BT, L, d);
    const size_t Rd = (size_t)R * d, Bd = (size_t)n_slides * d;
    Carve<kPad64> c(saved);
    const PoolSaved<float> S = pool_saved(c, BT, L, d);
    float *a = S.a, *b = S.b, *ab = S.ab, *w = S.w, *hpool = S.hpool;
    auto P = [&](int br, int i) { return params[br * 8 + i]; };
    const DropSpec s0 = stream_of(head_drop_p, seed, offset, stride, 0, rng_epoch), s1 = stream_of(head_drop_p, seed, offset, stride, 1, rng_epoch),
                   s2 = stream_of(rho_drop_p, seed, offset, stride, 2, rng_epoch);
    const bool fuse_ab = pool_fuses_scorer(NB, L, d);
    GroupBuilder gab, gsc, grho;
    for (int br = 0; br < NB; ++br) {
        RC(gab.add(mpo_args_fwd(x + br * Rd, P(br, 0), P(br, 1), a + br * Rd, R, d, d, 1.0f, MPO_ACT_TANH, nullptr, drop_br(s0, br, Rd))));
        RC(gab.add(mpo_args_fwd(x + br * Rd, P(br, 2), P(br, 3), b + br * Rd, R, d, d, 1.0f, MPO_ACT_SIGMOID, nullptr, drop_br(s1, br, Rd))));
        if (!fuse_ab)
            RC(gsc.add(mpo_args_fwd(ab + br * Rd, P(br, 4), P(br, 5), scores + (size_t)br * R, R, d, 1, 1.0f, MPO_ACT_NONE)));
        if (h_interleaved) {
            DropSpec sd = s2;
            sd.off += (uint64_t)br * (d / 4);
            GemmArgs m = mpo_args_fwd(hpool + br * Bd, P(br, 6), P(br, 7), h + (size_t)br * d, n_slides, d, d, 1.0f, MPO_ACT_RELU,
                                      nullptr, sd);
            m.ldc = NB * d;
            RC(grho.add(m));
        } else {
            RC(grho.add(mpo_args_fwd(hpool + br * Bd, P(br, 6), P(br, 7), h + br * Bd, n_slides, d, d, 1.0f, MPO_ACT_RELU, nullptr,
                                     drop_br(s2, br, Bd))));
        }
    }
    RC(gab.launch(stream));
    if (fuse_ab) {
        PoolScorer ps;
        for (int br = 0; br < NB; ++br) { ps.wc[br] = P(br, 4); ps.bc[br] = P(br, 5); }
        ps.n_slides = n_slides;
        RC(mpo_launch_pool_score_fwd(a, b, x, ps, scores, w, hpool, BT, L, d, stream));
    } else {
        RC(mpo_launch_ew_mul(a, b, ab, RT * d, stream));
        RC(gsc.launch(stream));
        RC(mpo_launch_pool_fwd(scores, x, w, hpool, BT, L, d, stream));
    }
    RC(grho.launch(stream));
    return 0;
}

int mpo_gated_pool_backward(const float* x, int n_branches, int n_slides, int L, int d, const float* const* params,
                            float head_drop_p, float rho_drop_p, const float* saved, const float* h,
                            const float* dh, int h_interleaved, const float* d_scores_ext, float* dx, float* const* grads,
                            void* workspace, size_t workspace_bytes, mpo_stream_t stream) {
    MPO_CHECK(n_branches >= 1 && n_branches <= 2, "gated pool backward: 1..2 branches (got %d)", n_branches);
    const int NB = n_branches, R = n_slides * L, RT = NB * R, BT = NB * n_slides;
    const size_t Rd = (size_t)R * d, Bd = (size_t)n_slides * d;
    Carve<kPad64, const float> c(saved);
    const PoolSaved<const float> S = pool_saved(c, BT, L, d);
    const float *a = S.a, *b = S.b, *ab = S.ab, *w = S.w, *hpool = S.hpool;
    WsCarve ws(workspace, workspace_bytes);
    const PoolWs W = pool_ws(ws, BT, L, d);
    MPO_CHECK(ws.ok(), "gated pool backward: workspace too small (%zu bytes)", workspace_bytes);
    float *dhpool = W.dhpool, *dscores = W.dscores, *dab = W.dab, *da = W.da, *db = W.db;
    auto P = [&](int br, int i) { return params[br * 8 + i]; };
    auto G = [&](int br, int i) { return grads[br * 8 + i]; };
    auto pairs = [&](auto&& mk_dx, auto&& mk_dw) { return launch_pairs(NB, stream, mk_dx, mk_dw); };
    const size_t h_off = h_interleaved ? (size_t)d : Bd;
    const int h_ld = h_interleaved ? NB * d : d;
    RC(pairs([&](int br) { GemmArgs m = mpo_args_bwd_input(dh + br * h_off, P(br, 6), dhpool + br * Bd, n_slides, d, d, 1.0f, 0, gate(h + br * h_off, MPO_GATE_RELU, rho_drop_p)); m.lda = h_ld; return m; },
             [&](int br) { GemmArgs m = mpo_args_bwd_weight(dh + br * h_off, hpool + br * Bd, G(br, 6), G(br, 7), n_slides, d, d, 1.0f, gate(h + br * h_off, MPO_GATE_RELU, rho_drop_p)); m.lda = h_ld; return m; }));
    if (pool_fuses_scorer(NB, L, d)) {
        PoolScorer ps;
        for (int br = 0; br < NB; ++br) { ps.wc[br] = P(br, 4); ps.bc[br] = P(br, 5); }
        ps.n_slides = n_slides;
        RC(mpo_launch_pool_score_bwd(dhpool, x, w, d_scores_ext, a, b, ps, dscores, dx, da, db, BT, L, d, stream));
    } else {
        RC(mpo_launch_pool_bwd(dhpool, x, w, d_scores_ext, dscores, dx, BT, L, d, stream));
        RC(pairs([&](int br) { return mpo_args_bwd_input(dscores + (size_t)br * R, P(br, 4), dab + br * Rd, R, d, 1, 1.0f, 0); },
                 [&](int br) { return mpo_args_bwd_weight(dscores + (size_t)br * R, ab + br * Rd, G(br, 4), G(br, 5), R, d, 1, 1.0f); }));
        RC(mpo_launch_ew_mul2(dab, b, a, da, db, RT * d, stream));
    }
    {
        GroupBuilder first, second;
        for (int br = 0; br < NB; ++br) {
            const GateSpec ga = gate(a + br * Rd, MPO_GATE_TANH, head_drop_p), gb = gate(b + br * Rd, MPO_GATE_SIGMOID, head_drop_p);
            RC(first.add(mpo_args_bwd_input(da + br * Rd, P(br, 0), dx + br * Rd, R, d, d, 1.0f, 1, ga)));
            RC(second.add(mpo_args_bwd_input(db + br * Rd, P(br, 2), dx + br * Rd, R, d, d, 1.0f, 1, gb)));
            RC(first.add(mpo_args_bwd_weight(da + br * Rd, x + br * Rd, G(br, 0), G(br, 1), R, d, d, 1.0f, ga)));
            RC(first.add(mpo_args_bwd_weight(db + br * Rd, x + br * Rd, G(br, 2), G(br, 3), R, d, d, 1.0f, gb)));
            if (pool_fuses_scorer(NB, L, d)) {
                const float* ds = dscores + (size_t)br * R;
                GemmArgs m3;
                m3.A = a + br * Rd; m3.lda = d;
                m3.gate = b + br * Rd; m3.gate_mode = MPO_GATE_MUL;
                m3.B = ds; m3.ldb = 1;
                m3.C = G(br, 4); m3.ldc = 1;
                m3.M = d; m3.N = 1; m3.K = R; m3.layout = 0;
                RC(second.add(m3));
                RC(second.add(mpo_args_bwd_weight(ds, ds, dab + br, G(br, 5), R, 1, 1, 1.0f)));
            }
        }
        RC(first.launch(stream));
        RC(second.launch(stream));
    }
    return 0;
}

size_t mpo_fusion_head_saved_floats(int n_slides, int hidden, int dout, int n_classes) {
    SavedCount c;
    head_saved(c, n_slides, hidden, dout, n_classes, false);
    return c.n_floats();
}
size_t mpo_fusion_head_loss_saved_floats(int n_slides, int hidden, int dout, int n_classes) {
    SavedCount c;
    head_saved(c, n_slides, hidden, dout, n_classes, true);
    return c.n_floats();
}
size_t mpo_fusion_head_workspace_bytes(int n_slides, int hidden, int dout, int n_classes) {
    WsCount c;
    head_ws(c, n_slides, hidden, dout, n_classes);
    return c.workspace_bytes();
}

static int head_mlp_forward(const float* hcat, int n_slides, int din, int hidden, int dout, int n_classes, const float* const* P,
                            const HeadSaved<float>& S, hipStream_t stream) {
    RC(mpo_linear_fwd(hcat, P[0], P[1], S.z1, n_slides, din, hidden, 1.0f, MPO_ACT_RELU, stream));
    RC(mpo_linear_fwd(S.z1, P[2], P[3], S.z2, n_slides, hidden, dout, 1.0f, MPO_ACT_RELU, stream));
    return mpo_linear_fwd(S.z2, P[4], P[5], S.logits, n_slides, dout, n_classes, 1.0f, MPO_ACT_NONE, stream);
}
static int head_mlp_backward(const float* hcat, int n_slides, int din, int hidden, int dout, int n_classes, const float* const* P,
                             const HeadSaved<const float>& S, const float* dlogits, const HeadWs& W, float* d_hcat,
                             float* const* G, hipStream_t stream) {
    PAIR(mpo_args_bwd_input(dlogits, P[4], W.dz2, n_slides, dout, n_classes, 1.0f, 0),
         mpo_args_bwd_weight(dlogits, S.z2, G[4], G[5], n_slides, dout, n_classes, 1.0f));
    PAIR(mpo_args_bwd_input(W.dz2, P[2], W.dz1, n_slides, hidden, dout, 1.0f, 0, gate(S.z2, MPO_GATE_RELU)),
         mpo_args_bwd_weight(W.dz2, S.z1, G[2], G[3], n_slides, hidden, dout, 1.0f, gate(S.z2, MPO_GATE_RELU)));
    PAIR(mpo_args_bwd_input(W.dz1, P[0], d_hcat, n_slides, din, hidden, 1.0f, 0, gate(S.z1, MPO_GATE_RELU)),
         mpo_args_bwd_weight(W.dz1, hcat, G[0], G[1], n_slides, din, hidden, 1.0f, gate(S.z1, MPO_GATE_RELU)));
    return 0;
}

int mpo_fusion_head_forward(const float* hcat, int n_slides, int din, int hidden, int dout, int n_classes,
                            const float* const* P, float* hazards, float* survs, float* y, float* saved,
                            mpo_stream_t stream) {
    Carve<kPad64> c(saved);
    const HeadSaved<float> S = head_saved(c, n_slides, hidden, dout, n_classes, false);
    RC(head_mlp_forward(hcat, n_slides, din, hidden, dout, n_classes, P, S, stream));
    return mpo_launch_head_fwd(S.logits, hazards, survs, y, n_slides, n_classes, stream);
}

int mpo_fusion_head_backward(const float* hcat, int n_slides, int din, int hidden, int dout, int n_classes,
                             const float* const* P, const float* saved, const float* hazards, const float* survs,
                             const float* y, const float* d_hazards, const float* d_survs, const float* d_y,
                             float* d_hcat, float* const* G, void* workspace, size_t workspace_bytes,
                             mpo_stream_t stream) {
    Carve<kPad64, const float> c(saved);
    const HeadSaved<const float> S = head_saved(c, n_slides, hidden, dout, n_classes, false);
    WsCarve ws(workspace, workspace_bytes);
    const HeadWs W = head_ws(ws, n_slides, hidden, dout, n_classes);
    MPO_CHECK(ws.ok(), "fusion head backward: workspace too small (%zu bytes)", workspace_bytes);
    RC(mpo_launch_head_bwd(hazards, survs, y, d_hazards, d_survs, d_y, W.dlogits, n_slides, n_classes, stream));
    return head_mlp_backward(hcat, n_slides, din, hidden, dout, n_classes, P, S, W.dlogits, W, d_hcat, G, stream);
}

int mpo_fusion_head_loss_forward(const float* hcat, int n_slides, int din, int hidden, int dout, int n_classes,
                                 const float* const* P, const int64_t* label, const float* censorship,
                                 const float* slide_weight, float alpha, float eps, float* hazards, float* survs, float* y,
                                 float* loss, float* risk, float* saved, mpo_stream_t stream) {
    MPO_CHECK(hcat && P && label && censorship && slide_weight && hazards && survs && y && loss && saved,
              "fusion head + loss forward: null argument");
    Carve<kPad64> c(saved);
    const HeadSaved<float> S = head_saved(c, n_slides, hidden, dout, n_classes, true);
    RC(head_mlp_forward(hcat, n_slides, din, hidden, dout, n_classes, P, S, stream));
    return mpo_launch_head_loss(S.logits, reinterpret_cast<const long long*>(label), censorship, slide_weight, hazards, survs, y,
                                loss, risk, S.dlogits, n_slides, n_classes, alpha, eps, static_cast<hipStream_t>(stream));
}
int mpo_fusion_head_sct_loss_forward(const float* hcat, int n_slides, int din, int hidden, int dout, int n_classes,
                                     const float* const* P, const int64_t* label, const float* censorship,
                                     const float* slide_weight, float eps, float* hazards, float* survs, float* y,
                                     float* loss, float* risk, float* saved, mpo_stream_t stream) {
    MPO_CHECK(hcat && P && label && censorship && slide_weight && hazards && survs && y && loss && saved,
              "fusion head + sct loss forward: null argument");
    Carve<kPad64> c(saved);
    const HeadSaved<float> S = head_saved(c, n_slides, hidden, dout, n_classes, true);
    RC(head_mlp_forward(hcat, n_slides, din, hidden, dout, n_classes, P, S, stream));
    return mpo_launch_head_sct_loss(S.logits, reinterpret_cast<const long long*>(label), censorship, slide_weight, hazards, survs,
                                    y, loss, risk, S.dlogits, n_slides, n_classes, eps, static_cast<hipStream_t>(stream));
}
int mpo_fusion_head_loss_backward(const float* hcat, int n_slides, int din, int hidden, int dout, int n_classes,
                                  const float* const* P, const float* saved, float* d_hcat, float* const* G,
                                  void* workspace, size_t workspace_bytes, mpo_stream_t stream) {
    Carve<kPad64, const float> c(saved);
    const HeadSaved<const float> S = head_saved(c, n_slides, hidden, dout, n_classes, true);
    WsCarve ws(workspace, workspace_bytes);
    const HeadWs W = head_ws(ws, n_slides, hidden, dout, n_classes);
    MPO_CHECK(ws.ok(), "fusion head + loss backward: workspace too small (%zu bytes)", workspace_bytes);
    return head_mlp_backward(hcat, n_slides, din, hidden, dout, n_classes, P, S, S.dlogits, W, d_hcat, G, stream);
}

int mpo_survival_head_forward(const float* logits, int n_slides, int n_classes, float* hazards, float* survs, float* y,
                              mpo_stream_t stream) {
    MPO_CHECK(logits && hazards && survs && y, "survival head forward: null argument");
    return mpo_launch_head_fwd(logits, hazards, survs, y, n_slides, n_classes, static_cast<hipStream_t>(stream));
}
int mpo_survival_head_backward(const float* hazards, const float* survs, const float* y, const float* d_hazards,
                               const float* d_survs, const float* d_y, int n_slides, int n_classes, float* d_logits,
                               mpo_stream_t stream) {
    MPO_CHECK(hazards && survs && y && d_logits, "survival head backward: null argument");
    return mpo_launch_head_bwd(hazards, survs, y, d_hazards, d_survs, d_y, d_logits, n_slides, n_classes,
                               static_cast<hipStream_t>(stream));
}

int mpo_ces_loss_forward(const float* hazards, const float* survs, const int64_t* label, const float* censorship,
                         int n_slides, int n_classes, float alpha, float eps, float* loss, float* risk, mpo_stream_t stream) {
    MPO_CHECK(hazards && survs && label && censorship && loss, "ces loss forward: null argument");
    return mpo_launch_ces_loss_fwd(hazards, survs, reinterpret_cast<const long long*>(label), censorship, loss, risk,
                                   n_slides, n_classes, alpha, eps, static_cast<hipStream_t>(stream));
}
int mpo_ces_loss_backward(const float* hazards, const float* survs, const int64_t* label, const float* censorship,
                          int n_slides, int n_classes, float alpha, float eps, const float* d_loss, int d_loss_is_scalar,
                          float* d_hazards, float* d_survs, mpo_stream_t stream) {
    MPO_CHECK(hazards && survs && label && censorship && d_loss && d_hazards && d_survs, "ces loss backward: null argument");
    return mpo_launch_ces_loss_bwd(hazards, survs, reinterpret_cast<const long long*>(label), censorship, d_loss,
                                   d_loss_is_scalar, d_hazards, d_survs, n_slides, n_classes, alpha, eps,
                                   static_cast<hipStream_t>(stream));
}

int mpo_sct_loss_forward(const float* y, const int64_t* label, const float* censorship, int n_slides, int n_classes,
                         float eps, float* loss, mpo_stream_t stream) {
    MPO_CHECK(y && label && censorship && loss, "sct loss forward: null argument");
    MPO_CHECK(n_classes >= 1 && n_classes <= 16, "sct loss: n_classes %d not in 1..16", n_classes);
    return mpo_launch_sct_loss_fwd(y, reinterpret_cast<const long long*>(label), censorship, loss, n_slides, n_classes, eps,
                                   static_cast<hipStream_t>(stream));
}
int mpo_sct_loss_backward(const float* y, const int64_t* label, const float* censorship, int n_slides, int n_classes,
                          float eps, const float* d_loss, int d_loss_is_scalar, float* d_y, mpo_stream_t stream) {
    MPO_CHECK(y && label && censorship && d_loss && d_y, "sct loss backward: null argument");
    MPO_CHECK(n_classes >= 1 && n_classes <= 16, "sct loss: n_classes %d not in 1..16", n_classes);
    return mpo_launch_sct_loss_bwd(y, reinterpret_cast<const long long*>(label), censorship, d_loss, d_loss_is_scalar, d_y,
                                   n_slides, n_classes, eps, static_cast<hipStream_t>(stream));
}

// ... 134 lines not shown
```

### multimodal_path_omic_amd/harness.py

```python
from __future__ import annotations

from dataclasses import dataclass
from typing import List, Sequence

import numpy as np
import torch

from .ops import BagBatch


def ces_loss(hazards, survs, label, censorship, alpha: float = 0.75, eps: float = 1e-7, reduction: str = "mean"):
    y = label.view(-1, 1).long()
    c = censorship.view(-1, 1).float()
    s_pad = torch.cat([torch.ones_like(c), survs], 1)
    reg = -(1 - c) * (torch.log(torch.gather(s_pad, 1, y).clamp(min=eps))
                      + torch.log(torch.gather(hazards, 1, y).clamp(min=eps)))
    s_y = torch.gather(survs, 1, y).clamp(min=eps)
    ce = -(c * torch.log(s_y) + (1 - c) * torch.log(1 - s_y))
    loss = ((1 - alpha) * ce + alpha * reg).view(-1)
    if reduction == "mean":
        return loss.mean()
    if reduction == "sum":
        return loss.sum()
    return loss


def risk_score(survs):
    return -survs.sum(dim=1)


def concordance_index_censored(event, time, risk, tied_tol: float = 1e-8) -> float:
    event = np.asarray(event, dtype=bool)
    time = np.asarray(time, dtype=np.float64)
    risk = np.asarray(risk, dtype=np.float64)
    later = (time[None, :] > time[:, None]) | ((time[None, :] == time[:, None]) & ~event[None, :])
    comparable = later & event[:, None]
    np.fill_diagonal(comparable, False)
    den = comparable.sum()
    if den == 0:
        raise ValueError("no comparable pairs")
    diff = risk[:, None] - risk[None, :]
    ties = np.abs(diff) <= tied_tol
    num = ((diff > 0) & ~ties & comparable).sum() + 0.5 * (ties & comparable).sum()
    return float(num) / float(den)


def make_window(slides: Sequence[dict], device, bag_dtype=torch.float32):
    bags = BagBatch.from_list([s["wsi"].to(device=device, dtype=bag_dtype, non_blocking=True) for s in slides])
    n_groups = len(slides[0]["omics"])
    omics = [torch.stack([s["omics"][i] for s in slides]).to(device, non_blocking=True) for i in range(n_groups)]
    labels = torch.tensor([s["survival_class"] for s in slides], dtype=torch.int64).to(device, non_blocking=True)
    cens = torch.tensor([float(s["censorship"]) for s in slides]).to(device, non_blocking=True)
    return bags, omics, labels, cens


CE_REFUSAL = ("loss 'ce' cannot train these models: the reference computes nn.CrossEntropyLoss()(Y, label.unsqueeze(0)) "
              "with Y (1, C) and a (1, 1) target (models/mcat/main.py:46-47), which torch rejects on the first slide "
              "('0D or 1D target tensor expected') -- there is no behaviour to reproduce; use 'ces' or 'sct'")


def make_ge_window(slides: Sequence[dict], device, bag_dtype=torch.float32):
    bags = BagBatch.from_list([s["wsi"].to(device=device, dtype=bag_dtype, non_blocking=True) for s in slides])
    labels = torch.tensor([int(s["gene_expr_class"]) for s in slides], dtype=torch.int64).to(device, non_blocking=True)
    return bags, labels


def sample_window_rows(model, bags: BagBatch, sample_rows) -> BagBatch:
    if not sample_rows or not model.training:
        return bags
    from . import ops
    x = bags.data
    return ops.RowSampler(bags.n_slides, int(sample_rows), x.shape[1], x.dtype, x.device, static=False).bind(bags)()


def train_ge_window(model, bags: BagBatch, labels, grad_acc_step: int, l1: float = 0.0, sample_rows: "int | None" = None):
    if sample_rows and sample_rows < model.MIN_WINDOW_ROWS:
        raise ValueError(f"sample_rows {sample_rows}: the gene-expression model's window step needs at least "
                         f"{model.MIN_WINDOW_ROWS} rows per bag")
    bags = sample_window_rows(model, bags, sample_rows)
    w = _slide_weights(bags.n_slides, grad_acc_step, labels.device)
    _, att = model.forward_window(bags, need_maps=False, ce_targets=(labels, w))
    per_bag = att["loss"]
    per_bag.backward(w)
    return _with_penalty(model, per_bag.detach(), l1)


def train_window(model, bags: BagBatch, omics, labels, cens, grad_acc_step: int, loss: str = "ces", lambda_reg: float = 0.01,
                 alpha: float = 0.75, l1: float = 0.0, sample_rows: "int | None" = None):
    from . import ops
    bags = sample_window_rows(model, bags, sample_rows)
    if loss == "cesar":
        hazards, survs, _, att = model.forward_window(bags, omics, inference=True)
        per_slide, risk = ops.ces_loss(hazards, survs, labels, cens, alpha)
        per_slide = per_slide + lambda_reg * ops.map_block_norm(att["coattn"])
    elif loss in ("ces", "sct"):
        if getattr(model, "fusion", None) == "concat":
            w = _slide_weights(bags.n_slides, grad_acc_step, labels.device)
            _, _, _, att = model.forward_window(bags, omics, ces_targets=(labels, cens, w), fused_loss=loss, alpha=alpha)
            per_slide, risk = att["loss"], att["risk"]
            per_slide.backward(w)
            return _with_penalty(model, per_slide.detach(), l1), risk
        hazards, survs, y, _ = model.forward_window(bags, omics)
        if loss == "ces":
            per_slide, risk = ops.ces_loss(hazards, survs, labels, cens, alpha)
        else:
            per_slide, risk = ops.sct_loss(y, labels, cens), risk_score(survs.detach())
    elif loss == "ce":
        raise ValueError(CE_REFUSAL)
    else:
        raise ValueError(f"loss '{loss}' is not built (ces | sct | cesar)")
    per_slide.backward(_slide_weights(per_slide.numel(), grad_acc_step, per_slide.device))
    return _with_penalty(model, per_slide.detach(), l1), risk


def _with_penalty(model, per_slide, l1: float):
    return per_slide if not l1 else per_slide + l1 * weights_abs_sum(model)


def weights_abs_sum(model) -> torch.Tensor:
    from . import ops
    bases, rest = {}, []
    for p in model.parameters():
        base = getattr(p, "_mpo_flat_param_base", None)
        if base is not None and p.untyped_storage().data_ptr() == base.untyped_storage().data_ptr():
            bases[id(base)] = base
        else:
            rest.append(p)
    parts = [ops.flat_abs_sum(b) for b in bases.values()] + [ops.flat_abs_sum(p.detach().float()) for p in rest]
    return parts[0] if len(parts) == 1 else torch.cat(parts).sum(0, keepdim=True)


LOSSES = {"mcat": ("ces", "sct"), "nacagat": ("ces", "sct", "cesar"), "ge_nacagat": ("ce",)}
OPTIMISERS = ("adam", "adamax", "adadelta", "sgd")


@dataclass
class TrainOptions:
    loss: str
    alpha: float
    lambda_reg: float
    grad_acc_step: int
    optimizer: str
    lr: float
    weight_decay: float
    l1: float
    gamma: "float | None"

    def train_kwargs(self) -> dict:
        return dict(loss=self.loss, alpha=self.alpha, lambda_reg=self.lambda_reg, l1=self.l1)

    def make_optimizer(self, bucket):
        from .dp import FlatOptimizer
        wd = 0.0 if self.optimizer == "sgd" else self.weight_decay
        return FlatOptimizer(bucket, self.optimizer, lr=self.lr, weight_decay=wd, l1_lambda=self.l1)

    def make_scheduler(self, opt):
        from .dp import FlatExponentialLR
        return None if self.gamma is None else FlatExponentialLR(opt, self.gamma)


def training_options(training: dict, model: str = "mcat") -> TrainOptions:
    if model not in LOSSES:
        raise ValueError(f"model '{model}' has no training loop here ({' | '.join(LOSSES)})")
    loss = training["loss"]
    if loss == "ce" and "ce" not in LOSSES[model]:
        raise ValueError(CE_REFUSAL)
    if loss not in LOSSES[model]:
        raise ValueError(f'Loss "{loss}" not implemented for {model} ({" | ".join(LOSSES[model])})')
    alpha, lambda_reg = (0.75, 0.01) if loss == "cesar" else (float(training.get("alpha", 0.75)), 0.01)
    name = training.get("optimizer")
    name = name if name in OPTIMISERS else "adam"
    lam = training.get("lambda")
    gamma = float(training["gamma"]) if training.get("scheduler") == "exp" else None
    return TrainOptions(loss=loss, alpha=alpha, lambda_reg=lambda_reg, grad_acc_step=int(training["grad_acc_step"]),
                        optimizer=name, lr=float(training["lr"]), weight_decay=float(training.get("weight_decay") or 0.0),
                        l1=float(lam) if lam else 0.0, gamma=gamma)


_slide_weight_cache = {}


def _slide_weights(n: int, grad_acc_step: int, device) -> torch.Tensor:
    key = (n, grad_acc_step, str(device))
    w = _slide_weight_cache.get(key)
    if w is None:
        w = _slide_weight_cache[key] = torch.full((n,), 1.0 / grad_acc_step, device=device, dtype=torch.float32)
    return w


class GraphedWindowStep:

    def __init__(self, model, bucket, window, grad_acc_step: int, opt=None, warmup: int = 2, pool=None,
                 split_patch_grad: bool = False, prime: bool = True, loss: str = "ces", alpha: float = 0.75,
                 lambda_reg: float = 0.01, l1: "float | None" = None, rng_base: "int | None" = None,
                 sample_rows: "int | None" = None):
        from . import ops
        calls_on_entry = ops._rng_calls
        self.model, self.bucket, self.opt = model, bucket, opt
        self.l1 = float(getattr(opt, "l1_lambda", 0.0) if l1 is None else l1)
        self.train_kwargs = dict(loss=loss, alpha=alpha, lambda_reg=lambda_reg, l1=self.l1)
        self.window, self.acc = window, grad_acc_step
        self.split = bool(split_patch_grad)
        self.ge = len(window) == 2
        if self.ge and self.split:
            raise ValueError("split_patch_grad is built for the fusion models' data-parallel steps, not for the "
                             "gene-expression model")
        if self.ge and loss not in ("ces", "ce"):
            raise ValueError(f"loss '{loss}' is not built for the gene-expression model (ce)")
        if self.split and opt is not None:
            raise ValueError("split_patch_grad is for steps whose optimiser runs after an all-reduce (opt=None)")
        self.tail_graph = None
        self.sampler = None
        if sample_rows:
            reason = self._sampling_refusal(window[0], int(sample_rows))
            if reason:
                raise ValueError(f"GraphedWindowStep(sample_rows={sample_rows}): {reason}")
            x = window[0].data
            self.sampler = ops.RowSampler(window[0].n_slides, int(sample_rows), x.shape[1], x.dtype, x.device).bind(window[0])
        else:
            window[0].plan()
        dev = bucket.flat.device
        if ops._rng_epoch_tensor is None:
            ops.set_rng_epoch(torch.zeros(1, dtype=torch.int64, device=dev))
        self.epoch = ops._rng_epoch_tensor
        keep = None if opt is None else [t.clone() for t in opt.state_tensors()]
        keep_epoch = self.epoch.clone()
        side = torch.cuda.Stream(device=dev)
        side.wait_stream(torch.cuda.current_stream(dev))
        with torch.cuda.stream(side):
            for _ in range(warmup):
                self._body()
            if keep is not None:
                for t, k in zip(opt.state_tensors(), keep):
                    t.copy_(k)
            self.epoch.copy_(keep_epoch)
        torch.cuda.current_stream(dev).wait_stream(side)
        self.graph = torch.cuda.CUDAGraph()
        if rng_base is not None:
            ops._rng_calls = int(rng_base)
        self.rng_base = ops._rng_calls
        bag_data = window[0].data
# ... 101 lines not shown
```

### multimodal_path_omic_amd/ops.py

```python
from __future__ import annotations

import ctypes
import math
from dataclasses import dataclass
from typing import List, Optional

import torch

from . import _lib as L


plan_workgroups = None
wgrad_workgroups = None


@dataclass
class BagBatch:
    data: torch.Tensor
    cu: torch.Tensor
    lengths: List[int]
    _plan: object = None

    def __post_init__(self):
        if len(self.lengths) == 0 or any(int(m) <= 0 for m in self.lengths):
# ... 78 lines not shown
        return view.view(p.shape)
    return torch.empty_like(p)


_rng_epoch_tensor = None


def set_rng_epoch(t):
    global _rng_epoch_tensor
    _rng_epoch_tensor = t


def _epoch():
    return L.ptr(_rng_epoch_tensor) if _rng_epoch_tensor is not None else None


def _workspace(nbytes, device):
    return torch.empty(max(int(nbytes), 256), dtype=torch.uint8, device=device)


class LinearFn(torch.autograd.Function):

    @staticmethod
    def forward(ctx, x, weight, bias, act: str = "none"):
        x2 = x.reshape(-1, x.shape[-1]).contiguous()
        y = torch.empty(x2.shape[0], weight.shape[0], device=x.device, dtype=torch.float32)
        L.call("mpo_linear_forward", L.ptr(x2), L.ptr(weight), L.ptr(bias), L.ptr(y), x2.shape[0],
               weight.shape[1], weight.shape[0], 1.0, L.ACT[act], L.stream_of(x))
        ctx.save_for_backward(x2, weight, y)
        ctx.act = act
        ctx.has_bias = bias is not None
        ctx.xshape = x.shape
        return y.view(*x.shape[:-1], weight.shape[0])

    @staticmethod
    def backward(ctx, dy):
        x2, weight, y = ctx.saved_tensors
        dy = dy.reshape(-1, dy.shape[-1]).contiguous()
        if ctx.act == "relu":
            dy = dy * (y > 0)
        elif ctx.act == "tanh":
            dy = dy * (1 - y * y)
        elif ctx.act == "sigmoid":
            dy = dy * (y * (1 - y))
        elif ctx.act == "elu":
            dy = dy * torch.where(y > 0, torch.ones_like(y), y + 1)
        dy = dy.contiguous()
        R, I, O = x2.shape[0], weight.shape[1], weight.shape[0]
        dx = torch.empty_like(x2) if ctx.needs_input_grad[0] else None
        dw = torch.empty_like(weight)
        db = torch.empty(O, device=dy.device, dtype=torch.float32) if ctx.has_bias else None
        s = L.stream_of(dy)
        if dx is not None:
            L.call("mpo_linear_backward_input", L.ptr(dy), L.ptr(weight), L.ptr(dx), R, I, O, 1.0, 0, s)
        L.call("mpo_linear_backward_weight", L.ptr(dy), L.ptr(x2), L.ptr(dw), L.ptr(db), R, I, O, 1.0, s)
        return (dx.view(ctx.xshape) if dx is not None else None), dw, db, None


def linear(x, weight, bias=None, act="none"):
    return LinearFn.apply(x, weight, bias, act)


class CoAttnMCATFn(torch.autograd.Function):

    @staticmethod
    def forward(ctx, query, bag_data, in_w, in_b, out_w, out_b, batch: BagBatch, need_weights: bool,
                bag_relu_gate: float = 0.0):
        lib = L.lib()
        ctx.set_materialize_grads(False)
        ctx.bag_relu_gate = float(bag_relu_gate)
        ctx.bag_bias = getattr(bag_data, "_mpo_bias_param", None)
        n_slides = batch.n_slides
        R, E = query.shape
        n_q = R // n_slides
        dev = query.device
        query = query.contiguous()
        out = torch.empty(R, E, device=dev, dtype=torch.float32)
        amap = torch.empty(n_q * batch.total_rows, device=dev, dtype=torch.float32) if need_weights else None
        saved = torch.empty(lib.mpo_coattn_saved_floats(n_slides, n_q, E), device=dev, dtype=torch.float32)
        ws = _workspace(lib.mpo_coattn_workspace_bytes(n_slides, n_q, E, batch.max_rows), dev)
        L.call("mpo_coattn_mcat_forward",
            L.ptr(bag_data), L.bag_dtype_code(bag_data), L.ptr(batch.cu), n_slides, batch.total_rows, batch.max_rows,
            L.ptr(query), n_q, E, L.ptr(in_w), L.ptr(in_b), L.ptr(out_w), L.ptr(out_b),
            L.ptr(out), L.ptr(amap), L.ptr(saved), batch.plan(), L.ptr(ws), ws.numel(), L.stream_of(query))
        ctx.save_for_backward(query, bag_data, in_w, out_w, saved, amap)
        ctx.param_refs = (in_w, in_b, out_w, out_b)
        ctx.batch = batch
        ctx.n_q = n_q
        return out, amap

    @staticmethod
    def backward(ctx, d_out, d_map):
        lib = L.lib()
        query, bag_data, in_w, out_w, saved, amap = ctx.saved_tensors
        batch, n_q = ctx.batch, ctx.n_q
        R, E = query.shape
        dev = query.device
        d_out = d_out.contiguous() if d_out is not None else torch.zeros(R, E, device=dev)
        if d_map is not None:
            d_map = d_map.contiguous()
        d_query = torch.empty_like(query)
        d_bag = torch.empty_like(bag_data)
        colsum = _bias_grad_slot(ctx.bag_bias, E, dev) if ctx.bag_relu_gate != 0.0 else None
        d_in_w, d_in_b, d_out_w, d_out_b = (grad_out(p) for p in ctx.param_refs)
        ws = _workspace(lib.mpo_coattn_workspace_bytes(batch.n_slides, n_q, E, batch.max_rows), dev)
        L.call("mpo_coattn_mcat_backward",
            L.ptr(bag_data), L.bag_dtype_code(bag_data), L.ptr(batch.cu), batch.n_slides, batch.total_rows,
            batch.max_rows, L.ptr(query), n_q, E, L.ptr(in_w), L.ptr(out_w), L.ptr(saved), L.ptr(amap),
            L.ptr(d_out), L.ptr(d_map), L.ptr(d_query), 0, L.ptr(d_bag), L.ptr(colsum), L.ptr(d_in_w), L.ptr(d_in_b),
            L.ptr(d_out_w), L.ptr(d_out_b), ctx.bag_relu_gate, batch.plan(), L.ptr(ws), ws.numel(), L.stream_of(query))
        if colsum is not None:
            d_bag._mpo_colsum = colsum
        return d_query, d_bag, d_in_w, d_in_b, d_out_w, d_out_b, None, None, None


def coattn_mcat(query, batch: BagBatch, in_w, in_b, out_w, out_b, need_weights: bool, bag_relu_gate: float = 0.0):
    return CoAttnMCATFn.apply(query, batch.data, in_w, in_b, out_w, out_b, batch, need_weights, bag_relu_gate)


stats = {"colsum_handoffs": 0, "qpass_in_place": 0, "qpass_copied": 0, "head_loss_ces": 0, "head_loss_sct": 0,
         "head_loss_ce": 0}


def _query_grad_buffer(d_qpass, owned: bool, query):
    if d_qpass is None:
        return torch.empty_like(query), False
    if owned:
        stats["qpass_in_place"] += 1
        return d_qpass.contiguous(), True
    stats["qpass_copied"] += 1
    return d_qpass.clone(memory_format=torch.contiguous_format), True


def _bias_grad_slot(bag_param, E, dev):
    if bag_param is not None and getattr(bag_param, "_mpo_grad_view", None) is not None and bag_param.grad is None \
            and bag_param.numel() == E and not getattr(bag_param, "_mpo_slice_taken", False):
        return bag_param._mpo_grad_view.view(E)
    return torch.empty(E, device=dev, dtype=torch.float32)

defer_patch_weight_grad = False
_deferred_patch = []

def flush_patch_weight_grads():
    for g, x, dw in _deferred_patch:
        patch_weight_grad(g, x, dw)
    _deferred_patch.clear()

def _patch_weight_grad_now_or_deferred(g, x, dw, weight):
    if defer_patch_weight_grad and getattr(weight, "_mpo_grad_view", None) is not None \
            and dw.data_ptr() == weight._mpo_grad_view.data_ptr():
        _deferred_patch.append((g, x, dw))
    else:
        patch_weight_grad(g, x, dw)


class PatchFcFn(torch.autograd.Function):

    @staticmethod
    def forward(ctx, x, weight, bias, drop_p: float, pre_gated_grad: bool, batch=None):
        lib = L.lib()
        if not patch_fc_kernel_supported(x, weight):
            raise ValueError(f"patch layer: built for a contiguous bf16 window through Linear(512 | 1024 | 2048, 128 | 256 | 512) "
                             f"(patch_dim in {set(PATCH_DIMS)}; got {x.dtype} {tuple(x.shape)} through a weight {tuple(weight.shape)})")
        if batch is None:
            batch = BagBatch(x, make_cu([x.shape[0]], x.device), [x.shape[0]])
        h = torch.empty(x.shape[0], weight.shape[0], device=x.device, dtype=torch.bfloat16)
        seed, off = _reserve(h.numel() // 16 + 2) if drop_p > 0 else (0, 0)
        ws = _workspace(lib.mpo_patch_fc_workspace_bytes(weight.shape[0], weight.shape[1]), x.device)
        L.call("mpo_patch_fc_forward", L.ptr(x), L.ptr(batch.cu), batch.n_slides, batch.total_rows, batch.max_rows,
               x.shape[1], L.ptr(weight), L.ptr(bias), weight.shape[0], float(drop_p), seed, off,
               _epoch(), L.ptr(h), batch.plan(), L.ptr(ws), ws.numel(), L.stream_of(x))
        drop_p = _realised_drop(drop_p) if drop_p > 0 else 0.0
        ctx.save_for_backward(x, h)
        ctx.param_refs = (weight, bias)
        ctx.drop_p, ctx.pre_gated = float(drop_p), bool(pre_gated_grad)
        return h

    @staticmethod
    def backward(ctx, dh):
        lib = L.lib()
        x, h = ctx.saved_tensors
        dh = dh.contiguous()
        if ctx.pre_gated:
            g = dh
        else:
            g = None
        dw, db = (grad_out(p) for p in ctx.param_refs)
        if g is None:
            g = torch.empty_like(dh)
            ws = _workspace(lib.mpo_patch_epilogue_backward_workspace_bytes(g.numel(), g.shape[1]), g.device)
            L.call("mpo_patch_epilogue_backward", L.ptr(h), L.ptr(dh), L.ptr(g), g.numel(), g.shape[1], ctx.drop_p,
                   L.ptr(db), L.ptr(ws), ws.numel(), L.stream_of(g))
        else:
            ready = getattr(dh, "_mpo_colsum", None)
            if ready is not None and ready.shape == db.shape:
                if ready.data_ptr() != db.data_ptr():
                    db.copy_(ready)
                stats["colsum_handoffs"] += 1
            else:
                _colsum_two_stage(g, db)
        _patch_weight_grad_now_or_deferred(g, x, dw, ctx.param_refs[0])
        return None, dw, db, None, None, None


def _colsum_two_stage(g: torch.Tensor, out: torch.Tensor, block: int = 256) -> torch.Tensor:
    rows, d = g.shape
    main = rows // block * block
    if main:
        torch.sum(g[:main].view(rows // block, block, d).sum(1, dtype=torch.float32), 0, out=out)
    else:
        out.zero_()
    if main < rows:
        out += g[main:].sum(0, dtype=torch.float32)
    return out


def patch_weight_grad(g: torch.Tensor, x: torch.Tensor, out: torch.Tensor) -> torch.Tensor:
    e, k = out.shape
    if not (g.dtype == torch.bfloat16 and x.dtype == torch.bfloat16 and e in (128, 256, 512) and k in (128, 256, 512, 1024, 2048)
            and g.shape == (x.shape[0], e) and x.shape[1] == k
            and g.is_contiguous() and x.is_contiguous() and out.is_contiguous() and out.dtype == torch.float32):
        raise ValueError(f"patch weight gradient: g {g.dtype} {tuple(g.shape)} x {x.dtype} {tuple(x.shape)} -> {tuple(out.shape)} is not a "
                         f"geometry the kernel is built for (contiguous bf16, embed 128/256/512, patch_dim 128/256/512/1024/2048)")
    lib = L.lib()
    ws = _workspace(lib.mpo_patch_weight_grad_workspace_bytes(e, k), g.device)
    wgs = int(wgrad_workgroups or 0)
    if wgs and k != 1024:
        wgs = 0
    L.call("mpo_patch_weight_grad", L.ptr(g), L.ptr(x), g.shape[0], e, k, L.ptr(out), wgs, L.ptr(ws), ws.numel(),
           L.stream_of(g))
    return out


class PatchFcF32Fn(torch.autograd.Function):

    @staticmethod
    def forward(ctx, x, weight, bias, drop_p: float):
        lib = L.lib()
        h = torch.empty(x.shape[0], weight.shape[0], device=x.device, dtype=torch.float32)
        seed, off = _reserve(h.numel() // 16 + 2) if drop_p > 0 else (0, 0)
        ws = _workspace(lib.mpo_patch_fc_f32_workspace_bytes(0), x.device)
        L.call("mpo_patch_fc_f32_forward", L.ptr(x), x.shape[0], x.shape[1], L.ptr(weight), L.ptr(bias), weight.shape[0],
               float(drop_p), seed, off, _epoch(), feature_scale(x), L.ptr(h), L.ptr(ws), ws.numel(),
               L.stream_of(x))
        ctx.save_for_backward(x, h)
        ctx.param_refs = (weight, bias)
        ctx.gate = 1.0 / (1.0 - _realised_drop(drop_p)) if drop_p > 0 else 1.0
        return h

    @staticmethod
    def backward(ctx, dh):
        lib = L.lib()
        x, h = ctx.saved_tensors
        dh = dh.contiguous()
        dw, db = (grad_out(p) for p in ctx.param_refs)
        ws = _workspace(lib.mpo_patch_fc_f32_workspace_bytes(1), x.device)
        L.call("mpo_patch_fc_f32_backward", L.ptr(dh), L.ptr(h), L.ptr(x), x.shape[0], h.shape[1], x.shape[1], ctx.gate, L.ptr(dw),
               L.ptr(db), L.ptr(ws), ws.numel(), L.stream_of(x))
        return None, dw, db, None


def feature_scale(x) -> float:
    if x.numel() == 0:
        return 1.0
    try:
        key = (x._version, x.data_ptr(), tuple(x.shape))
    except RuntimeError:
        key = None
    cached = getattr(x, "_mpo_feature_scale", None) if key is not None else None
    if cached is not None and cached[:3] == key:
        return cached[3]
    if x.is_cuda and torch.cuda.is_current_stream_capturing():
        raise RuntimeError("feature_scale(x) needs one host read: call ops.feature_scale(window.data) before capturing the graph")
    m = float(x.detach().abs().amax())
    s = math.ldexp(1.0, max(-100, min(100, 15 - math.frexp(m)[1]))) if (m > 0.0 and math.isfinite(m)) else 1.0
    if key is not None:
        try:
            x._mpo_feature_scale = (*key, s)
        except AttributeError:
            pass
    return s


def patch_fc_f32_supported(x, weight) -> bool:
    return x.dtype == torch.float32 and x.is_contiguous() and tuple(weight.shape) == (256, 1024)


def patch_fc_f32(x, weight, bias, drop_p: float):
    return PatchFcF32Fn.apply(x, weight, bias, float(drop_p))


class PatchCoAttnMCATFn(torch.autograd.Function):

    @staticmethod
    def forward(ctx, x, patch_w, patch_b, query, in_w, in_b, out_w, out_b, batch: BagBatch, need_weights: bool, drop_p: float,
                tokens: "TokenPair | None" = None, qpass_owned: bool = False):
        lib = L.lib()
        ctx.set_materialize_grads(False)
        n_slides = batch.n_slides
        R, E = query.shape
        n_q = R // n_slides
        dev, T = query.device, batch.total_rows
        query = query.contiguous()
        h_bag = torch.empty(T, E, device=dev, dtype=torch.bfloat16)
        out = tokens.slot(0, (R, E)) if tokens is not None else torch.empty(R, E, device=dev, dtype=torch.float32)
        amap = torch.empty(n_q * T, device=dev, dtype=torch.float32) if need_weights else None
        saved = torch.empty(lib.mpo_coattn_saved_floats(n_slides, n_q, E), device=dev, dtype=torch.float32)
        ws = _workspace(lib.mpo_patch_coattn_workspace_bytes(n_slides, n_q, E, x.shape[1]), dev)
        seed, off = _reserve(T * E // 16 + 2) if drop_p > 0 else (0, 0)
        L.call("mpo_patch_coattn_mcat_forward",
            L.ptr(x), L.ptr(batch.cu), n_slides, T, batch.max_rows, x.shape[1], L.ptr(patch_w), L.ptr(patch_b), float(drop_p),
            seed, off, _epoch(), L.ptr(query), n_q, E, L.ptr(in_w), L.ptr(in_b), L.ptr(out_w), L.ptr(out_b),
            L.ptr(h_bag), L.ptr(out), L.ptr(amap), L.ptr(saved), batch.plan(), L.ptr(ws), ws.numel(), L.stream_of(query))
        ctx.save_for_backward(x, h_bag, query, in_w, out_w, saved, amap)
        ctx.param_refs = (patch_w, patch_b, in_w, in_b, out_w, out_b)
        ctx.batch, ctx.n_q = batch, n_q
        ctx.gate = 1.0 / (1.0 - _realised_drop(drop_p)) if drop_p > 0 else 1.0
        ctx.qpass_owned = bool(qpass_owned)
        ctx.mark_non_differentiable(h_bag)
        return out, amap, h_bag, query.view_as(query)

    @staticmethod
    def backward(ctx, d_out, d_map, _d_h, d_qpass):
        lib = L.lib()
        x, h_bag, query, in_w, out_w, saved, amap = ctx.saved_tensors
        batch, n_q = ctx.batch, ctx.n_q
        R, E = query.shape
        dev = query.device
        d_out = d_out.contiguous() if d_out is not None else torch.zeros(R, E, device=dev)
        d_map = d_map.contiguous() if d_map is not None else None
        d_query, accumulate = _query_grad_buffer(d_qpass, ctx.qpass_owned, query)
        g = torch.empty_like(h_bag)
        patch_w, patch_b, p_in_w, p_in_b, p_out_w, p_out_b = ctx.param_refs
        d_pw, d_pb = grad_out(patch_w), grad_out(patch_b)
        d_in_w, d_in_b, d_out_w, d_out_b = (grad_out(p) for p in (p_in_w, p_in_b, p_out_w, p_out_b))
        ws = _workspace(lib.mpo_coattn_workspace_bytes(batch.n_slides, n_q, E, batch.max_rows), dev)
        L.call("mpo_coattn_mcat_backward",
            L.ptr(h_bag), L.MPO_BF16, L.ptr(batch.cu), batch.n_slides, batch.total_rows, batch.max_rows, L.ptr(query), n_q, E,
            L.ptr(in_w), L.ptr(out_w), L.ptr(saved), L.ptr(amap), L.ptr(d_out), L.ptr(d_map), L.ptr(d_query), int(accumulate),
            L.ptr(g), L.ptr(d_pb), L.ptr(d_in_w), L.ptr(d_in_b), L.ptr(d_out_w), L.ptr(d_out_b), ctx.gate, batch.plan(),
            L.ptr(ws), ws.numel(), L.stream_of(query))
        stats["colsum_handoffs"] += 1
        _patch_weight_grad_now_or_deferred(g, x, d_pw, patch_w)
        return None, d_pw, d_pb, d_query, d_in_w, d_in_b, d_out_w, d_out_b, None, None, None, None, None


class TokenPair:

    def __init__(self, rows: int, d: int, device):
        self.buf = torch.empty(2, rows, d, device=device, dtype=torch.float32)

    def slot(self, i: int, shape):
        return self.buf[i].view(*shape)

    def stack(self, first, second):
        for i, t in enumerate((first, second)):
            if t.data_ptr() != self.buf[i].data_ptr() or t.numel() != self.buf[i].numel() or not t.is_contiguous():
                raise ValueError("TokenPair.stack: the halves must be the tensors produced into slot(0) and slot(1)")
        return _TokenPairFn.apply(first, second, self)


class _TokenPairFn(torch.autograd.Function):
    @staticmethod
    def forward(ctx, first, second, pair):
        ctx.shapes = (first.shape, second.shape)
        return pair.buf.view_as(pair.buf)

    @staticmethod
    def backward(ctx, d):
        return d[0].view(ctx.shapes[0]), d[1].view(ctx.shapes[1]), None


def _realised_drop(p: float) -> float:
    return float(int(p * 256.0 + 0.5)) / 256.0


def patch_coattn_mcat(x_bf16, batch: BagBatch, patch_w, patch_b, drop_p: float, query, in_w, in_b, out_w, out_b,
                      need_weights: bool, tokens: "TokenPair | None" = None, _qpass_owned: bool = False):
    return PatchCoAttnMCATFn.apply(x_bf16, patch_w, patch_b, query, in_w, in_b, out_w, out_b, batch, need_weights,
                                   float(drop_p), tokens, bool(_qpass_owned))


def fused_patch_coattn_supported(x, embed: int, n_q: int) -> bool:
    return x.dtype == torch.bfloat16 and x.shape[1] == 1024 and embed == 256 and n_q <= 8


PATCH_DIMS = (512, 1024, 2048)


def patch_fc_kernel_supported(x, weight) -> bool:
    return (x.dtype == torch.bfloat16 and x.is_contiguous() and x.dim() == 2 and weight.shape[0] in (128, 256, 512)
            and weight.shape[1] in PATCH_DIMS and x.shape[1] == weight.shape[1])


def patch_fc(x_bf16, weight, bias, drop_p: float, pre_gated_grad: bool = False, batch: "BagBatch | None" = None):
    h = PatchFcFn.apply(x_bf16, weight, bias, drop_p, pre_gated_grad, batch)
    if pre_gated_grad:
        h._mpo_bias_param = bias
    if drop_p > 0:
        h._mpo_keep_scale = 1.0 / (1.0 - _realised_drop(drop_p))
    return h


import torch.nn.functional as F


_rng_calls = 0


def _reserve(span: int):
    global _rng_calls
    seed = torch.initial_seed() & 0xFFFFFFFFFFFFFFFF
    off = _rng_calls
    _rng_calls += int(span) + 1
    return seed, off


def gated_scores(x, wa, ba, wb, bb, wc, bc, drop_p: float):
    a = linear(x, wa, ba, "tanh")
    b = linear(x, wb, bb, "sigmoid")
    if drop_p > 0.0:
        a = F.dropout(a, drop_p, True)
        b = F.dropout(b, drop_p, True)
    return linear(a * b, wc, bc)


class CagFn(torch.autograd.Function):

    @staticmethod
    def forward(ctx, q, q_hat, residual, dest, qpass_owned, *params):
        lib = L.lib()
        ctx.set_materialize_grads(False)
        q, q_hat = q.contiguous(), q_hat.contiguous()
        rows, dim = q.shape
        hidden = params[0].shape[0]
        c = torch.empty(rows, hidden, device=q.device, dtype=torch.float32)
        saved = torch.empty(lib.mpo_cag_saved_floats(rows, hidden), device=q.device, dtype=torch.float32)
        pa = L.ptr_array(params)
        total = None
        if residual is not None:
            residual = residual.contiguous()
            total = dest[0].slot(dest[1], (rows, hidden)) if dest is not None else torch.empty_like(c)
        L.call("mpo_cag_forward", L.ptr(q), L.ptr(q_hat), rows, dim, hidden, pa, L.ptr(c), L.ptr(saved), L.ptr(residual),
               L.ptr(total), L.stream_of(q))
        ctx.save_for_backward(q, q_hat, c, saved, *params)
        ctx.param_refs = params
        ctx.has_residual = residual is not None
        ctx.qpass_owned = bool(qpass_owned)
        return (total if total is not None else c), q.view_as(q)

    @staticmethod
    def backward(ctx, dc, d_qpass):
        lib = L.lib()
        q, q_hat, c, saved, *params = ctx.saved_tensors
        rows, dim = q.shape
        hidden = params[0].shape[0]
        if dc is None:
            dc = torch.zeros_like(c)
        dc = dc.contiguous()
        dq, accumulate = _query_grad_buffer(d_qpass, ctx.qpass_owned, q)
        dqh = torch.empty_like(q_hat)
        grads = [grad_out(p) for p in ctx.param_refs]
        ws = _workspace(lib.mpo_cag_workspace_bytes(rows, hidden), q.device)
        pa, ga = L.ptr_array(params), L.ptr_array(grads)
        L.call("mpo_cag_backward", L.ptr(q), L.ptr(q_hat), rows, dim, hidden, pa, L.ptr(saved), L.ptr(c),
               L.ptr(dc), L.ptr(dq), int(accumulate), L.ptr(dqh), ga, L.ptr(ws), ws.numel(),
               L.stream_of(q))
        return (dq, dqh, dc if ctx.has_residual else None, None, None, *grads)


def contextual_gate(q, q_hat, cag, residual=None, dest=None, hand_on: bool = False, _qpass_owned: bool = False):
    out, q_pass = CagFn.apply(q, q_hat, residual, dest, bool(_qpass_owned), cag.fc1[0].weight, cag.fc1[0].bias, cag.fc2[0].weight, cag.fc2[0].bias,
                              cag.fc3[0].weight, cag.fc3[0].bias, cag.G[1].weight, cag.G[1].bias,
                              cag.E[1].weight, cag.E[1].bias, cag.fc_c[0].weight, cag.fc_c[0].bias)
    return (out, q_pass) if hand_on else out


class EncoderFn(torch.autograd.Function):

    @staticmethod
    def forward(ctx, x, geom, drop_p, *params):
        lib = L.lib()
        branches, n_slides, T, d, ff, heads, layers = geom
        x = x.contiguous()
        y = torch.empty_like(x)
        saved = torch.empty(lib.mpo_encoder_saved_floats(branches * n_slides, T, d, ff, heads, layers), device=x.device,
                            dtype=torch.float32)
        seed, off = _reserve(lib.mpo_encoder_rng_span(branches * n_slides, T, d, ff, layers)) if drop_p > 0 else (0, 0)
        pa = L.ptr_array(params)
        L.call("mpo_encoder_forward", L.ptr(x), branches, n_slides, T, d, ff, heads, layers, pa, float(drop_p), seed, off,
               _epoch(), L.ptr(y), L.ptr(saved), L.stream_of(x))
        ctx.save_for_backward(x, saved, *params)
        ctx.param_refs = params
        ctx.geom, ctx.drop = geom, (float(drop_p), seed, off)
        return y

    @staticmethod
    def backward(ctx, dy):
        lib = L.lib()
        x, saved, *params = ctx.saved_tensors
        branches, n_slides, T, d, ff, heads, layers = ctx.geom
        drop_p, seed, off = ctx.drop
        dx = torch.empty_like(x)
        grads = [grad_out(p) for p in ctx.param_refs]
        ws = _workspace(lib.mpo_encoder_workspace_bytes(branches * n_slides, T, d, ff), x.device)
        pa, ga = L.ptr_array(params), L.ptr_array(grads)
        dy = dy.contiguous()
        L.call("mpo_encoder_backward",
            L.ptr(x), branches, n_slides, T, d, ff, heads, layers, pa, drop_p, seed, off, _epoch(), L.ptr(saved), L.ptr(dy),
            L.ptr(dx), ga, L.ptr(ws), ws.numel(), L.stream_of(x))
        return (dx, None, None, *grads)


def _encoder_params(layers):
    params = []
    for ly in layers:
        params += [ly.self_attn.in_proj_weight, ly.self_attn.in_proj_bias, ly.self_attn.out_proj.weight,
                   ly.self_attn.out_proj.bias, ly.linear1.weight, ly.linear1.bias, ly.linear2.weight, ly.linear2.bias,
                   ly.norm1.weight, ly.norm1.bias, ly.norm2.weight, ly.norm2.bias]
    return params


def _encoder_geom(layers):
    l0 = layers[0]
    return (l0.linear1.in_features, l0.linear1.out_features, l0.self_attn.num_heads, len(layers), l0.dropout.p)


def encoder(x, layers, training: bool):
    return encoder_branches([x], [layers], training)[0]


def encoder_branches(xs, layer_stacks, training: bool):
    if len(xs) == 1:
        return [encoder_stacked(xs[0].unsqueeze(0), layer_stacks, training)[0]]
    if any(x.shape != xs[0].shape for x in xs):
        raise ValueError("branch-batched encoders need identical input shapes")
    return list(encoder_stacked(torch.stack(list(xs)), layer_stacks, training).unbind(0))


def encoder_stacked(x, layer_stacks, training: bool):
    nb, b, t, d = x.shape
    g0 = _encoder_geom(layer_stacks[0])
    if len(layer_stacks) != nb or any(_encoder_geom(ls) != g0 for ls in layer_stacks) or g0[0] != d:
        raise ValueError("branch-batched encoders need one layer stack per branch, all of identical geometry")
    params = [p for ls in layer_stacks for p in _encoder_params(ls)]
    geom = (nb, b, t, d, g0[1], g0[2], g0[3])
    y = EncoderFn.apply(x.reshape(nb * b * t, d), geom, g0[4] if training else 0.0, *params)
    return y.view(nb, b, t, d)


class BagSelfAttentionFn(torch.autograd.Function):

    @staticmethod
    def forward(ctx, qkv, heads: int, drop_p: float, need_map: bool):
        lib = L.lib()
        n_bags, m, d3 = qkv.shape
        d = d3 // 3
        qkv = qkv.contiguous()
        out = torch.empty((n_bags, m, d), device=qkv.device, dtype=torch.float32)
        saved = torch.empty(lib.mpo_bag_self_attention_saved_floats(n_bags, m, d, heads), device=qkv.device, dtype=torch.float32)
        amap = torch.empty((n_bags, m, m), device=qkv.device, dtype=torch.float32) if need_map else None
        seed, off = _reserve(1) if drop_p > 0 else (0, 0)
        L.call("mpo_bag_self_attention_forward", L.ptr(qkv), n_bags, m, d, heads, float(drop_p), seed, off, _epoch(), L.ptr(out),
               L.ptr(saved), L.ptr(amap), L.stream_of(qkv))
        ctx.save_for_backward(qkv, out, saved)
        ctx.geom, ctx.drop = (n_bags, m, d, heads), (float(drop_p), seed, off)
        if amap is not None:
            ctx.mark_non_differentiable(amap)
        return out, amap

    @staticmethod
    def backward(ctx, d_out, _d_map):
        lib = L.lib()
        qkv, out, saved = ctx.saved_tensors
        n_bags, m, d, heads = ctx.geom
        drop_p, seed, off = ctx.drop
        d_qkv = torch.empty_like(qkv)
        ws = _workspace(lib.mpo_bag_self_attention_workspace_bytes(n_bags, m, d, heads), qkv.device)
        d_out = d_out.contiguous()
        L.call("mpo_bag_self_attention_backward", L.ptr(qkv), L.ptr(out), L.ptr(saved), L.ptr(d_out), n_bags, m, d, heads, drop_p,
               seed, off, _epoch(), L.ptr(d_qkv), L.ptr(ws), ws.numel(), L.stream_of(qkv))
        return d_qkv, None, None, None


def bag_self_attention(x, mha, training: bool, need_weights: bool = True):
    if mha.in_proj_weight is None or mha.bias_k is not None or mha.add_zero_attn:
        raise NotImplementedError("bag self-attention: packed in_proj, no bias_k / zero-attn (the reference's constructor)")
    if need_weights and mha.num_heads != 1:
        raise NotImplementedError("bag self-attention: the M x M map is returned for one head (models/ge_nacagat/ge_nacagat.py:27)")
    xb = x if x.dim() == 3 else x.unsqueeze(0)
    qkv = linear(xb.float(), mha.in_proj_weight, mha.in_proj_bias)
    out, amap = BagSelfAttentionFn.apply(qkv, mha.num_heads, mha.dropout if training else 0.0, bool(need_weights))
    out = linear(out, mha.out_proj.weight, mha.out_proj.bias)
    if x.dim() == 2:
        out, amap = out[0], (amap[0] if amap is not None else None)
    return out, amap


class GatedPoolFn(torch.autograd.Function):

    @staticmethod
    def forward(ctx, x, geom, head_p, rho_p, interleave, *params):
        lib = L.lib()
        ctx.set_materialize_grads(False)
        branches, n_slides, Lr, d = geom
        bt = branches * n_slides
        x = x.contiguous()
        scores = torch.empty(bt * Lr, device=x.device, dtype=torch.float32)
        h = torch.empty((n_slides, branches * d) if interleave else (bt, d), device=x.device, dtype=torch.float32)
        saved = torch.empty(lib.mpo_gated_pool_saved_floats(bt, Lr, d), device=x.device, dtype=torch.float32)
        seed, off = _reserve(lib.mpo_gated_pool_rng_span(bt, Lr, d)) if (head_p > 0 or rho_p > 0) else (0, 0)
        pa = L.ptr_array(params)
        L.call("mpo_gated_pool_forward", L.ptr(x), branches, n_slides, Lr, d, pa, float(head_p), float(rho_p), seed, off,
               _epoch(), L.ptr(scores), L.ptr(h), int(interleave), L.ptr(saved), L.stream_of(x))
        ctx.save_for_backward(x, saved, h, *params)
        ctx.param_refs = params
        ctx.geom, ctx.drop, ctx.interleave = geom, (float(head_p), float(rho_p)), bool(interleave)
        return scores, h

    @staticmethod
    def backward(ctx, d_scores, dh):
        lib = L.lib()
        x, saved, h, *params = ctx.saved_tensors
        branches, n_slides, Lr, d = ctx.geom
        head_p, rho_p = ctx.drop
        dx = torch.empty_like(x)
        grads = [grad_out(p) for p in ctx.param_refs]
        if dh is None:
            dh = torch.zeros_like(h)
        ws = _workspace(lib.mpo_gated_pool_workspace_bytes(branches * n_slides, Lr, d), x.device)
        pa, ga = L.ptr_array(params), L.ptr_array(grads)
        dh = dh.contiguous()
        d_sc = d_scores.contiguous() if d_scores is not None else None
        L.call("mpo_gated_pool_backward",
            L.ptr(x), branches, n_slides, Lr, d, pa, head_p, rho_p, L.ptr(saved), L.ptr(h), L.ptr(dh), int(ctx.interleave),
            L.ptr(d_sc), L.ptr(dx), ga, L.ptr(ws), ws.numel(), L.stream_of(x))
        return (dx, None, None, None, None, *grads)


def gated_pool(tokens, head, rho, training: bool):
    return gated_pool_branches([tokens], [head], [rho], training)[0]


def gated_pool_branches(tokens, heads, rhos, training: bool):
    if len(tokens) == 1:
        sc, h = gated_pool_stacked(tokens[0].unsqueeze(0), heads, rhos, training)
        return [(sc[0], h[0])]
    if any(t.shape != tokens[0].shape for t in tokens):
        raise ValueError("branch-batched pooling needs identical token shapes")
    sc, h = gated_pool_stacked(torch.stack(list(tokens)), heads, rhos, training)
    return list(zip(sc.unbind(0), h.unbind(0)))


def gated_pool_stacked(tokens, heads, rhos, training: bool, interleave: bool = False):
    nb, b, l, d = tokens.shape
    params = []
    for head, rho in zip(heads, rhos):
        if head.attention_c.weight.shape[0] != 1 or head.attention_a[0].weight.shape != (d, d):
            raise NotImplementedError("gated pooling kernel: n_classes=1 and hidden_dim == input_dim only")
        params += [head.attention_a[0].weight, head.attention_a[0].bias, head.attention_b[0].weight, head.attention_b[0].bias,
                   head.attention_c.weight, head.attention_c.bias, rho[0].weight, rho[0].bias]
    if len(heads) != nb or len(rhos) != nb or len({(h.drop_p, r[2].p) for h, r in zip(heads, rhos)}) != 1:
        raise ValueError("branch-batched pooling needs one head + rho per branch with identical dropout rates")
    scores, h = GatedPoolFn.apply(tokens.reshape(nb * b * l, d), (nb, b, l, d), heads[0].drop_p if training else 0.0,
                                  rhos[0][2].p if training else 0.0, bool(interleave), *params)
    return scores.view(nb, b, 1, l), (h if interleave else h.view(nb, b, d))


class OmicSnnFn(torch.autograd.Function):

    @staticmethod
    def forward(ctx, drop_p, n_groups, tokens, *args):
        lib = L.lib()
        xs, params = [a.contiguous() for a in args[:n_groups]], args[n_groups:]
        n_slides, d = xs[0].shape[0], params[0].shape[0]
        dev = xs[0].device
        widths = (ctypes.c_int * n_groups)(*[int(x.shape[1]) for x in xs])
        g_bag = tokens.slot(1, (n_slides, n_groups, d)) if tokens is not None else \
            torch.empty(n_slides, n_groups, d, device=dev, dtype=torch.float32)
        saved = torch.empty(lib.mpo_omic_snn_saved_floats(n_slides, n_groups, d), device=dev, dtype=torch.float32)
        seed, off = _reserve(lib.mpo_omic_snn_rng_span(n_slides, n_groups, d)) if drop_p > 0 else (0, 0)
        xa, pa = L.ptr_array(xs), L.ptr_array(params)
        L.call("mpo_omic_snn_forward", xa, widths, n_groups, n_slides, d, pa, float(drop_p), seed, off, _epoch(),
               L.ptr(g_bag), L.ptr(saved), L.stream_of(g_bag))
        ctx.save_for_backward(g_bag, saved, *xs, *params)
        ctx.param_refs, ctx.n_groups, ctx.drop = params, n_groups, (float(drop_p), seed, off)
        return g_bag

    @staticmethod
    def backward(ctx, d_g):
        lib = L.lib()
        g_bag, saved, *rest = ctx.saved_tensors
        n = ctx.n_groups
        xs, params = rest[:n], rest[n:]
        n_slides, d = xs[0].shape[0], params[0].shape[0]
        drop_p, seed, off = ctx.drop
        widths = (ctypes.c_int * n)(*[int(x.shape[1]) for x in xs])
        grads = [grad_out(p) for p in ctx.param_refs]
        ws = _workspace(lib.mpo_omic_snn_workspace_bytes(n_slides, n, d), g_bag.device)
        xa, pa, ga = L.ptr_array(xs), L.ptr_array(params), L.ptr_array(grads)
        L.call("mpo_omic_snn_backward", xa, widths, n, n_slides, d, pa, drop_p, seed, off, _epoch(), L.ptr(g_bag),
               L.ptr(saved), L.ptr(d_g.contiguous()), ga, L.ptr(ws), ws.numel(),
               L.stream_of(g_bag))
        return (None, None, None, *([None] * n), *grads)


def omic_snn(omics, g_modules, training: bool, tokens: "TokenPair | None" = None):
    params = []
    for g in g_modules:
        params += [g[0][0].weight, g[0][0].bias, g[1][0].weight, g[1][0].bias]
    p = g_modules[0][0][2].p if training else 0.0
    return OmicSnnFn.apply(p, len(omics), tokens, *[o.float() for o in omics], *params)


class MapBlockNormFn(torch.autograd.Function):

    @staticmethod
    def forward(ctx, flat_map, batch: BagBatch, n_q: int):
        flat_map = flat_map.contiguous()
        sq = torch.empty(batch.n_slides * n_q, device=flat_map.device, dtype=torch.float32)
        L.call("mpo_map_block_dot", L.ptr(flat_map), L.ptr(flat_map), L.ptr(batch.cu), batch.n_slides, n_q, L.ptr(sq),
               L.stream_of(flat_map))
        norm = sq.view(batch.n_slides, n_q).sum(1).sqrt()
        ctx.save_for_backward(flat_map, norm)
        ctx.batch, ctx.n_q = batch, n_q
        return norm

    @staticmethod
    def backward(ctx, d_norm):
        flat_map, norm = ctx.saved_tensors
        scale = (d_norm / norm.clamp_min(1e-30)).contiguous()
        d_map = torch.empty_like(flat_map)
        L.call("mpo_map_block_scale", L.ptr(flat_map), L.ptr(scale), L.ptr(ctx.batch.cu), ctx.batch.n_slides, ctx.n_q,
               L.ptr(d_map), L.stream_of(flat_map))
        return d_map, None, None


def map_block_norm(maps) -> torch.Tensor:
    return MapBlockNormFn.apply(maps.flat, maps.batch, maps.n_q)


class SurvivalHeadFn(torch.autograd.Function):

    @staticmethod
    def forward(ctx, logits):
        ctx.set_materialize_grads(False)
        logits = logits.contiguous()
        b, c = logits.shape
        hz, sv, y = (torch.empty_like(logits) for _ in range(3))
        L.call("mpo_survival_head_forward", L.ptr(logits), b, c, L.ptr(hz), L.ptr(sv), L.ptr(y), L.stream_of(logits))
        ctx.save_for_backward(hz, sv, y)
        return hz, sv, y

    @staticmethod
    def backward(ctx, dhz, dsv, dy):
        hz, sv, y = ctx.saved_tensors
        b, c = hz.shape
        dhz, dsv, dy = (t.contiguous() if t is not None else None for t in (dhz, dsv, dy))
        dl = torch.empty_like(hz)
        L.call("mpo_survival_head_backward", L.ptr(hz), L.ptr(sv), L.ptr(y), L.ptr(dhz), L.ptr(dsv), L.ptr(dy), b, c,
               L.ptr(dl), L.stream_of(hz))
        return dl


def survival_head(logits):
    return SurvivalHeadFn.apply(logits)


class CesLossFn(torch.autograd.Function):

    @staticmethod
    def forward(ctx, hazards, survs, label, censorship, alpha, eps):
        ctx.set_materialize_grads(False)
        hazards, survs = hazards.contiguous(), survs.contiguous()
        label = label.view(-1).to(torch.int64).contiguous()
        censorship = censorship.view(-1).to(torch.float32).contiguous()
        b, c = hazards.shape
        loss = torch.empty(b, device=hazards.device, dtype=torch.float32)
        risk = torch.empty(b, device=hazards.device, dtype=torch.float32)
        L.call("mpo_ces_loss_forward", L.ptr(hazards), L.ptr(survs), L.ptr(label), L.ptr(censorship), b, c, float(alpha),
               float(eps), L.ptr(loss), L.ptr(risk), L.stream_of(hazards))
        ctx.save_for_backward(hazards, survs, label, censorship)
        ctx.cfg = (float(alpha), float(eps))
        ctx.mark_non_differentiable(risk)
        return loss, risk

    @staticmethod
# ... 434 lines not shown
```

Before: 28770 slides/s.

## Defer tail weight-gradient GEMMs and drain them inside spare patch-wgrad workgroups

Weight-gradient GEMMs from the encoder and gated-pool backward passes are no longer launched inline. They are recorded in a host-side list and later run by spare workgroups of the large patch weight-gradient kernel: 224 workgroups do the main work while the remaining ones drain the deferred tiles. A list too large for the kernel-argument segment, or a backward that never reaches the patch wgrad, falls back to grouped launches at flush. This removes several small serial launches and fills idle CUs during the long bag-side kernel. The cost is fewer workgroups on the main patch reduction, a large kernel-argument payload, and more host-side state that must be flushed correctly inside graph capture.

```diff
diff --git a/include/mpo_deferred_wgrad.h b/include/mpo_deferred_wgrad.h
--- /dev/null
+++ b/include/mpo_deferred_wgrad.h
@@ -0,0 +1,23 @@
+#ifndef MPO_DEFERRED_WGRAD_H
+#define MPO_DEFERRED_WGRAD_H
+#ifndef MPO_HIP_H
+#error "include mpo_hip.h: it defines mpo_stream_t and includes this header"
+#endif
+
+#ifdef __cplusplus
+extern "C" {
+#endif
+
+int mpo_deferred_wgrad_capacity(void);
+size_t mpo_deferred_wgrad_member_bytes(void);
+int mpo_deferred_wgrad_enable(int enabled);
+int mpo_deferred_wgrad_enabled(void);
+int mpo_deferred_wgrad_pending(void);
+int mpo_deferred_wgrad_flush(mpo_stream_t stream);
+int mpo_deferred_wgrad_push(const float* dy, const float* x, float* d_weight, float* d_bias , int rows,
+                            int in_features, int out_features, mpo_stream_t stream);
+
+#ifdef __cplusplus
+}
+#endif
+#endif
diff --git a/include/mpo_hip.h b/include/mpo_hip.h
--- a/include/mpo_hip.h
+++ b/include/mpo_hip.h
@@ -278,6 +278,7 @@
                            int n_q, int max_rows, const mpo_bag_plan* plan , mpo_stream_t stream);
 
 #include "mpo_bag_sample.h"
+#include "mpo_deferred_wgrad.h"
 
 #ifdef __cplusplus
 }
diff --git a/multimodal_path_omic_amd/_lib.py b/multimodal_path_omic_amd/_lib.py
--- a/multimodal_path_omic_amd/_lib.py
+++ b/multimodal_path_omic_amd/_lib.py
@@ -10,7 +10,8 @@
 _HERE = os.path.dirname(os.path.abspath(__file__))
 LIB_PATH = os.path.join(_HERE, "libmpo_hip.so")
 HEADER_PATH = os.path.join(os.path.dirname(_HERE), "include", "mpo_hip.h")
-COMPANION_HEADER_PATHS = [os.path.join(os.path.dirname(_HERE), "include", "mpo_bag_sample.h")]
+COMPANION_HEADER_PATHS = [os.path.join(os.path.dirname(_HERE), "include", name)
+                          for name in ("mpo_bag_sample.h", "mpo_deferred_wgrad.h")]
 
 _SCALARS = {"int": c_int, "int32_t": c_int, "int64_t": c_int64, "uint64_t": c_uint64, "size_t": c_size_t, "float": c_float,
             "mpo_stream_t": c_void_p}
@@ -67,7 +68,7 @@
 
 
 def _read_companions():
-    out = {}
+    out, seen = {}, set()
     for path in COMPANION_HEADER_PATHS:
         if not os.path.exists(path):
             raise RuntimeError(f"{path} is missing: include/mpo_hip.h includes it and the package binds its entries")
@@ -76,9 +77,10 @@
         if not signatures or constants or version is not None:
             raise RuntimeError(f"{path}: a companion header declares entries only (no enum, no MPO_ABI_VERSION)")
         for name in signatures:
-            if name in _signatures or name in out:
+            if name in _signatures or name in seen:
                 raise RuntimeError(f"{path}: {name} is declared twice")
-        out.update(signatures)
+        seen.update(signatures)
+        out[os.path.basename(path)] = signatures
     return out
 
 
@@ -87,7 +89,8 @@
 ACT = {k[len("MPO_ACT_"):-1].lower(): v for k, v in _constants.items() if k.startswith("MPO_ACT_")}
 OPTIM = {k[len("MPO_OPTIM_"):].lower(): v for k, v in _constants.items() if k.startswith("MPO_OPTIM_")}
 GEMM_ROUTE = {k[len("MPO_GEMM_ROUTE_"):].lower(): v for k, v in _constants.items() if k.startswith("MPO_GEMM_ROUTE_")}
-_companion_signatures = _read_companions()
+_companion_by_header = _read_companions()
+_companion_signatures = {name: sig for entries in _companion_by_header.values() for name, sig in entries.items()}
 
 
 class BagPlanC(ctypes.Structure):
@@ -102,8 +105,8 @@
     return list(_signatures)
 
 
-def companion_symbols():
-    return list(_companion_signatures)
+def companion_symbols(header: str = "mpo_bag_sample.h"):
+    return list(_companion_by_header[header])
 
 
 def check_abi_version(found: int, expected: int):
diff --git a/multimodal_path_omic_amd/csrc/capi.hip b/multimodal_path_omic_amd/csrc/capi.hip
--- a/multimodal_path_omic_amd/csrc/capi.hip
+++ b/multimodal_path_omic_amd/csrc/capi.hip
@@ -624,10 +624,30 @@
                                   static_cast<hipStream_t>(stream));
 }
 
+int mpo_deferred_wgrad_capacity(void) { return kDeferMax; }
+size_t mpo_deferred_wgrad_member_bytes(void) { return sizeof(GemmArgs); }
+int mpo_deferred_wgrad_pending(void) { return mpo_defer_list().n; }
+int mpo_deferred_wgrad_enabled(void) { return mpo_defer_enabled() ? 1 : 0; }
+int mpo_deferred_wgrad_flush(mpo_stream_t stream) { return mpo_defer_flush(static_cast<hipStream_t>(stream)); }
+int mpo_deferred_wgrad_enable(int enabled) { return mpo_defer_enable(enabled); }
+int mpo_deferred_wgrad_push(const float* dy, const float* x, float* d_weight, float* d_bias, int rows, int in_features,
+                            int out_features, mpo_stream_t stream) {
+    MPO_CHECK(dy && x && d_weight, "deferred weight gradient: null argument");
+    MPO_CHECK(rows >= 1 && in_features >= 1 && out_features >= 1, "deferred weight gradient: bad geometry (%d rows, %d -> %d)", rows,
+              in_features, out_features);
+    const GemmArgs g = mpo_args_bwd_weight(dy, x, d_weight, d_bias, rows, in_features, out_features, 1.0f);
+    if (mpo_defer_try(g)) return 0;
+    return mpo_launch_gemm(g, 0, 0, static_cast<hipStream_t>(stream));
+}
+#define MPO_CHECK_NOTHING_DEFERRED(who) \
+    MPO_CHECK(mpo_defer_list().n == 0, who ": %d deferred weight-gradient products were never computed (call " \
+              "mpo_deferred_wgrad_flush at the end of a backward whose patch weight gradient did not drain them)", mpo_defer_list().n)
+
 int mpo_adam_step_flat(float* params, const float* grads, float* exp_avg, float* exp_avg_sq, int64_t n, float lr,
                        float beta1, float beta2, float eps, float weight_decay, int step, const int32_t* step_dev,
                        mpo_stream_t stream) {
     MPO_CHECK(step >= 1 || step_dev, "adam: step counts from 1 (got %d)", step);
+    MPO_CHECK_NOTHING_DEFERRED("adam");
     return mpo_launch_adam_flat(params, grads, exp_avg, exp_avg_sq, (size_t)n, lr, beta1, beta2, eps, weight_decay,
                                 step < 1 ? 1 : step, step_dev, stream);
 }
@@ -636,6 +656,7 @@
                         const float* lr_dev, float beta1, float beta2, float eps, float weight_decay, float l1, int step,
                         const int32_t* step_dev, mpo_stream_t stream) {
     MPO_CHECK(algorithm >= MPO_OPTIM_ADAM && algorithm <= MPO_OPTIM_SGD, "flat optimiser: unknown algorithm %d", algorithm);
+    MPO_CHECK_NOTHING_DEFERRED("flat optimiser");
     MPO_CHECK(n >= 0, "flat optimiser: n = %lld", (long long)n);
     MPO_CHECK(params && grads, "flat optimiser: null parameter or gradient buffer");
     const bool stateful = algorithm != MPO_OPTIM_SGD;
diff --git a/multimodal_path_omic_amd/csrc/gemm_f32.hip b/multimodal_path_omic_amd/csrc/gemm_f32.hip
--- a/multimodal_path_omic_amd/csrc/gemm_f32.hip
+++ b/multimodal_path_omic_amd/csrc/gemm_f32.hip
@@ -156,6 +156,44 @@
 }
 int mpo_launch_gemm_mixed(const GemmGroup& grp, hipStream_t stream) { return launch_group("mixed grouped gemm", grp, -1, stream); }
 
+namespace {
+bool g_defer = false;
+DeferredList g_deferred;
+}
+int mpo_defer_enable(int enabled) {
+    const int was = g_defer ? 1 : 0;
+    g_defer = enabled != 0;
+    return was;
+}
+bool mpo_defer_enabled() { return g_defer; }
+bool mpo_defer_try(const GemmArgs& g) {
+    if (!g_defer || g_deferred.n >= kDeferMax || g.layout != 0) return false;
+    const int fc = fast_class(g);
+    if (fc < 0 || fc > 2 || longk_class(g, 0) >= 0) return false;
+    const int tiles = (g.M / DB) * (g.N / DB);
+    DeferredList& d = g_deferred;
+    d.g[d.n] = g;
+    d.n_pairs += (tiles + 1) / 2;
+    d.pair_end[d.n++] = d.n_pairs;
+    return true;
+}
+const DeferredList& mpo_defer_list() { return g_deferred; }
+void mpo_defer_clear() { g_deferred = DeferredList(); }
+int mpo_defer_flush(hipStream_t stream) {
+    const DeferredList d = g_deferred;
+    mpo_defer_clear();
+    for (int cls = 0; cls <= 2; ++cls) {
+        GemmGroup grp;
+        for (int i = 0; i < d.n; ++i) {
+            if (fast_class(d.g[i]) != cls) continue;
+            grp.g[grp.n++] = d.g[i];
+            if (grp.n == 8) { RC(mpo_launch_gemm_mixed(grp, stream)); grp.n = 0; }
+        }
+        if (grp.n) RC(mpo_launch_gemm_mixed(grp, stream));
+    }
+    return 0;
+}
+
 int mpo_launch_colsum(const float* x, float* out, int M, int N, int ld, int accumulate, hipStream_t stream) {
     if (N <= 0) return 0;
     colsum_kernel<<<(N + 15) / 16, 256, 0, stream>>>(x, out, M, N, ld, accumulate);
diff --git a/multimodal_path_omic_amd/csrc/gemm_f32_fast.h b/multimodal_path_omic_amd/csrc/gemm_f32_fast.h
--- a/multimodal_path_omic_amd/csrc/gemm_f32_fast.h
+++ b/multimodal_path_omic_amd/csrc/gemm_f32_fast.h
@@ -78,53 +78,56 @@
 };
 
 template <bool A_KC, bool B_KC, int GC, int NBMAX>
-__device__ __forceinline__ void gemm_f32_fast_body(const GemmArgs& g, FastLds& lds) {
-    if ((int)blockIdx.y * FB >= g.M || (int)blockIdx.x * FB >= g.N) return;
-    const int tid = threadIdx.x, lane = tid & 63, wave = __builtin_amdgcn_readfirstlane(tid >> 6);
-    const int m0 = blockIdx.y * FB, n0 = blockIdx.x * FB;
+__device__ __forceinline__ void gemm_f32_fast_body(const GemmArgs& g, FastLds& lds, int tile_m, int tile_n, int tid, bool active = true) {
+    if (tile_m * FB >= g.M || tile_n * FB >= g.N) return;
+    const int lane = tid & 63, wave = __builtin_amdgcn_readfirstlane(tid >> 6);
+    const int m0 = tile_m * FB, n0 = tile_n * FB;
     const int i16 = lane & 15, kq = lane >> 4;
-    GateFn gf;
-    gf.g = g.gate; gf.mode = g.gate_mode; gf.p = g.gate_p; gf.seed = g.gate_seed;
-    gf.off = epoch_offset(g.gate_off, g.rng_epoch);
-    gf.inv_keep = g.gate_p > 0.f ? 1.0f / (1.0f - g.gate_p) : 1.0f;
-    const bool want_bsum = g.bias_grad != nullptr && blockIdx.x == 0;
-
+    const bool want_bsum = g.bias_grad != nullptr && tile_n == 0;
     const int erow = tid >> 4, ecol = tid & 15;
     const size_t eo = (size_t)(m0 + erow) * g.ldc + n0 + ecol;
-    const float e_bias = g.bias ? g.bias[n0 + ecol] : 0.f;
-    const float e_mask = g.mask ? g.mask[eo] : 1.0f;
-    const float e_res = g.residual ? g.residual[eo] : 0.f;
-    const float e_old = g.accumulate ? g.C[eo] : 0.f;
-    float e_keep = 1.0f;
-    if (g.drop_p > 0.f) {
-        const unsigned long long doff = epoch_offset(g.drop_off, g.rng_epoch);
-        e_keep = dropout_keep(g.drop_seed, doff, eo, g.drop_p, g.alpha_dropout ? 1.0f : 1.0f / (1.0f - g.drop_p));
-    }
+    float e_bias = 0.f, e_mask = 1.0f, e_res = 0.f, e_old = 0.f, e_keep = 1.0f;
+    if (active) {
+        GateFn gf;
+        gf.g = g.gate; gf.mode = g.gate_mode; gf.p = g.gate_p; gf.seed = g.gate_seed;
+        gf.off = epoch_offset(g.gate_off, g.rng_epoch);
+        gf.inv_keep = g.gate_p > 0.f ? 1.0f / (1.0f - g.gate_p) : 1.0f;
 
-    const int kw = ((g.K + 63) >> 6) << 4;
-    const int kbeg = wave * kw;
-    const int nkb = max(0, min(kw, g.K - kbeg)) >> 4;
-    f32x4 acc0 = {0.f, 0.f, 0.f, 0.f}, acc1 = acc0;
-    float bsum = 0.f;
-    FastCtx<A_KC, B_KC, GC> cx{g, gf, m0 + i16, n0 + i16, kq, lane, want_bsum};
-    int kb = 0;
-    for (; kb + NBMAX <= nkb; kb += NBMAX) cx.template chunk<NBMAX>(kbeg + 16 * kb, acc0, acc1, bsum);
-    const int rem = nkb - kb;
-    if (rem >= 4) { cx.template chunk<4>(kbeg + 16 * kb, acc0, acc1, bsum); kb += 4; }
-    switch (nkb - kb) {
-        case 3: cx.template chunk<3>(kbeg + 16 * kb, acc0, acc1, bsum); break;
-        case 2: cx.template chunk<2>(kbeg + 16 * kb, acc0, acc1, bsum); break;
-        case 1: cx.template chunk<1>(kbeg + 16 * kb, acc0, acc1, bsum); break;
-        default: break;
-    }
+        e_bias = g.bias ? g.bias[n0 + ecol] : 0.f;
+        e_mask = g.mask ? g.mask[eo] : 1.0f;
+        e_res = g.residual ? g.residual[eo] : 0.f;
+        e_old = g.accumulate ? g.C[eo] : 0.f;
+        if (g.drop_p > 0.f) {
+            const unsigned long long doff = epoch_offset(g.drop_off, g.rng_epoch);
+            e_keep = dropout_keep(g.drop_seed, doff, eo, g.drop_p, g.alpha_dropout ? 1.0f : 1.0f / (1.0f - g.drop_p));
+        }
+
+        const int kw = ((g.K + 63) >> 6) << 4;
+        const int kbeg = wave * kw;
+        const int nkb = max(0, min(kw, g.K - kbeg)) >> 4;
+        f32x4 acc0 = {0.f, 0.f, 0.f, 0.f}, acc1 = acc0;
+        float bsum = 0.f;
+        FastCtx<A_KC, B_KC, GC> cx{g, gf, m0 + i16, n0 + i16, kq, lane, want_bsum};
+        int kb = 0;
+        for (; kb + NBMAX <= nkb; kb += NBMAX) cx.template chunk<NBMAX>(kbeg + 16 * kb, acc0, acc1, bsum);
+        const int rem = nkb - kb;
+        if (rem >= 4) { cx.template chunk<4>(kbeg + 16 * kb, acc0, acc1, bsum); kb += 4; }
+        switch (nkb - kb) {
+            case 3: cx.template chunk<3>(kbeg + 16 * kb, acc0, acc1, bsum); break;
+            case 2: cx.template chunk<2>(kbeg + 16 * kb, acc0, acc1, bsum); break;
+            case 1: cx.template chunk<1>(kbeg + 16 * kb, acc0, acc1, bsum); break;
+            default: break;
+        }
 #pragma unroll
-    for (int r = 0; r < 4; ++r) lds.part[wave][(4 * kq + r) * 16 + i16] = acc0[r] + acc1[r];
-    if (want_bsum) {
-        bsum += __shfl_xor(bsum, 16);
-        bsum += __shfl_xor(bsum, 32);
-        if (lane < 16) lds.bsum[wave][lane] = bsum;
+        for (int r = 0; r < 4; ++r) lds.part[wave][(4 * kq + r) * 16 + i16] = acc0[r] + acc1[r];
+        if (want_bsum) {
+            bsum += __shfl_xor(bsum, 16);
+            bsum += __shfl_xor(bsum, 32);
+            if (lane < 16) lds.bsum[wave][lane] = bsum;
+        }
     }
     __syncthreads();
+    if (!active) return;
     {
         float v = (lds.part[0][tid] + lds.part[1][tid]) + (lds.part[2][tid] + lds.part[3][tid]);
         v = (v + e_bias) * g.alpha;
@@ -142,8 +145,8 @@
 
 template <bool A_KC, bool B_KC, int GCL, int NBMAX>
 __device__ __forceinline__ void gemm_f32_fast_member(const GemmArgs& g, FastLds& lds) {
-    if (g.gate_mode == MPO_GATE_NONE) gemm_f32_fast_body<A_KC, B_KC, 0, NBMAX>(g, lds);
-    else gemm_f32_fast_body<A_KC, B_KC, GCL, NBMAX>(g, lds);
+    if (g.gate_mode == MPO_GATE_NONE) gemm_f32_fast_body<A_KC, B_KC, 0, NBMAX>(g, lds, blockIdx.y, blockIdx.x, threadIdx.x);
+    else gemm_f32_fast_body<A_KC, B_KC, GCL, NBMAX>(g, lds, blockIdx.y, blockIdx.x, threadIdx.x);
 }
 
 template <int GCL, int NBMAX>
diff --git a/multimodal_path_omic_amd/csrc/mpo_kernels.h b/multimodal_path_omic_amd/csrc/mpo_kernels.h
--- a/multimodal_path_omic_amd/csrc/mpo_kernels.h
+++ b/multimodal_path_omic_amd/csrc/mpo_kernels.h
@@ -52,6 +52,26 @@
 int mpo_launch_gemm_group(const GemmGroup& grp, int a_kc, int b_kc, hipStream_t stream);
 int mpo_launch_gemm_mixed(const GemmGroup& grp, hipStream_t stream);
 int mpo_launch_colsum(const float* x, float* out, int M, int N, int ld, int accumulate, hipStream_t stream);
+
+constexpr int kKernargBytes = 4096;
+constexpr int kWgradOwnArgBytes = 48;
+constexpr int kHiddenArgBytes = 256;
+constexpr int kDeferMax = 20;
+struct DeferredList {
+    int n = 0;
+    int n_pairs = 0;
+    int pair_end[kDeferMax] = {};
+    GemmArgs g[kDeferMax];
+};
+static_assert(kDeferMax == (kKernargBytes - kHiddenArgBytes - kWgradOwnArgBytes) / (int)(sizeof(GemmArgs) + sizeof(int)) / 4 * 4,
+              "kDeferMax: as many GemmArgs (and their pair counts), rounded down to a multiple of four, as fit the kernel-argument segment");
+static_assert(kWgradOwnArgBytes + sizeof(DeferredList) + kHiddenArgBytes <= kKernargBytes, "the deferred list must fit the kernel-argument segment");
+int mpo_defer_enable(int enabled);
+bool mpo_defer_enabled();
+bool mpo_defer_try(const GemmArgs& g);
+const DeferredList& mpo_defer_list();
+void mpo_defer_clear();
+int mpo_defer_flush(hipStream_t stream);
 
 inline GemmArgs mpo_args_fwd(const float* x, const float* w, const float* b, float* y, int R, int I, int O,
                              float alpha, int act, const float* residual = nullptr, DropSpec drop = DropSpec()) {
diff --git a/multimodal_path_omic_amd/csrc/patch_wgrad.hip b/multimodal_path_omic_amd/csrc/patch_wgrad.hip
--- a/multimodal_path_omic_amd/csrc/patch_wgrad.hip
+++ b/multimodal_path_omic_amd/csrc/patch_wgrad.hip
@@ -1,5 +1,6 @@
 #include "coattn_tile.h"
 #include "mpo_kernels.h"
+#include "gemm_f32_fast.h"
 
 namespace {
 
@@ -12,6 +13,7 @@
 constexpr int WG_LDS = WG_STAGES * WG_STAGE;
 constexpr int WG_WAVES = 8;
 constexpr int WG_WGS = 256;
+constexpr int WG_DRAIN_MAIN = 224;
 
 __device__ __forceinline__ void wait_vm(int n) {
     switch (n) {
@@ -21,13 +23,13 @@
     }
 }
 
-__global__ __launch_bounds__(WG_WAVES * 64, 1)
-void patch_wgrad_kernel(const __bf16* __restrict__ g, const __bf16* __restrict__ x, int total_rows, int patch_dim,
-                        int g_dim,
-                        int e_rows,
-                        int rows_per_range, float* __restrict__ part) {
+__device__ __forceinline__
+void patch_wgrad_main(char* lds,
+                      const __bf16* __restrict__ g, const __bf16* __restrict__ x, int total_rows, int patch_dim,
+                      int g_dim,
+                      int e_rows,
+                      int rows_per_range, float* __restrict__ part) {
     using G = TileGeom<WG_E>;
-    __shared__ __attribute__((aligned(1024))) char lds[WG_LDS];
     const int lane = threadIdx.x & 63;
     const int wave = __builtin_amdgcn_readfirstlane(threadIdx.x >> 6);
     const int n_cb = patch_dim < WG_CB ? 1 : patch_dim / WG_CB;
@@ -146,6 +148,65 @@
                 out[(size_t)(16 * (4 * wm + i) + 4 * (lane >> 4) + r) * patch_dim + 16 * (8 * wn + j) + (lane & 15)] = acc[i][j][r];
 }
 
+__global__ __launch_bounds__(WG_WAVES * 64, 1)
+void patch_wgrad_kernel(const __bf16* __restrict__ g, const __bf16* __restrict__ x, int total_rows, int patch_dim, int g_dim, int e_rows,
+                        int rows_per_range, float* __restrict__ part) {
+    __shared__ __attribute__((aligned(1024))) char lds[WG_LDS];
+    patch_wgrad_main(lds, g, x, total_rows, patch_dim, g_dim, e_rows, rows_per_range, part);
+}
+
+struct WgradDrainArgs {
+    const __bf16* g; const __bf16* x;
+    int total_rows, patch_dim, g_dim, e_rows, rows_per_range, n_main;
+    float* part;
+    DeferredList list;
+};
+static_assert(offsetof(WgradDrainArgs, list) == kWgradOwnArgBytes, "kWgradOwnArgBytes: the arguments in front of the list");
+static_assert(4 * sizeof(FastLds) <= WG_LDS, "the workers' FastLds copies come out of the pass's own LDS");
+static_assert(sizeof(GemmArgs) % 8 == 0 && offsetof(DeferredList, g) % 8 == 0, "members are read as 8-byte words");
+
+#define MPO_KARG __attribute__((address_space(4)))
+__device__ __forceinline__ void wgrad_worker(char* lds_raw, int worker, int n_workers) {
+    const char MPO_KARG* ka = (const char MPO_KARG*)__builtin_amdgcn_kernarg_segment_ptr();
+    const int MPO_KARG* head = reinterpret_cast<const int MPO_KARG*>(ka + offsetof(WgradDrainArgs, list));
+    const int MPO_KARG* pair_end = head + offsetof(DeferredList, pair_end) / sizeof(int);
+    const int n_pairs = head[offsetof(DeferredList, n_pairs) / sizeof(int)];
+    const int tid = threadIdx.x & 255, grp = __builtin_amdgcn_readfirstlane(threadIdx.x >> 8);
+    FastLds* fl = reinterpret_cast<FastLds*>(lds_raw);
+    int member = 0, first = 0, turn = 0;
+    for (int p = worker; p < n_pairs; p += n_workers, turn ^= 1) {
+        while (p >= pair_end[member]) first = pair_end[member++];
+        constexpr int NW = sizeof(GemmArgs) / 8;
+        const unsigned long long MPO_KARG* src = reinterpret_cast<const unsigned long long MPO_KARG*>(
+            ka + offsetof(WgradDrainArgs, list) + offsetof(DeferredList, g) + (size_t)member * sizeof(GemmArgs));
+        unsigned long long words[NW];
+#pragma unroll
+        for (int i = 0; i < NW; ++i) words[i] = src[i];
+        GemmArgs m;
+        __builtin_memcpy(&m, words, sizeof(GemmArgs));
+        const int tiles_n = m.N / FB, n_tiles = (m.M / FB) * tiles_n;
+        const int t = 2 * (p - first) + grp;
+        const bool active = t < n_tiles;
+        const int tm = active ? t / tiles_n : 0, tn = active ? t - tm * tiles_n : 0;
+        FastLds& l = fl[2 * turn + grp];
+        if (m.gate_mode == MPO_GATE_NONE) gemm_f32_fast_body<false, false, 0, 4>(m, l, tm, tn, tid, active);
+        else if (m.gate_mode == MPO_GATE_RNG) gemm_f32_fast_body<false, false, 2, 4>(m, l, tm, tn, tid, active);
+        else gemm_f32_fast_body<false, false, 1, 4>(m, l, tm, tn, tid, active);
+    }
+}
+#undef MPO_KARG
+
+__global__ __launch_bounds__(WG_WAVES * 64, 1)
+void patch_wgrad_kernel_drain(const __bf16* __restrict__ g, const __bf16* __restrict__ x, int total_rows, int patch_dim, int g_dim,
+                              int e_rows, int rows_per_range, int n_main, float* __restrict__ part, DeferredList list) {
+    __shared__ __attribute__((aligned(1024))) char lds[WG_LDS];
+    if ((int)blockIdx.x >= n_main) {
+        wgrad_worker(lds, blockIdx.x - n_main, gridDim.x - n_main);
+        return;
+    }
+    patch_wgrad_main(lds, g, x, total_rows, patch_dim, g_dim, e_rows, rows_per_range, part);
+}
+
 __global__ __launch_bounds__(256)
 void patch_wgrad_reduce_kernel(const float* __restrict__ part, float* __restrict__ out, int n4, int n_parts, int accumulate) {
     const int i = blockIdx.x * 256 + threadIdx.x;
@@ -174,18 +235,28 @@
     const int n_cb = patch_dim < WG_CB ? 1 : patch_dim / WG_CB;
     MPO_CHECK(workgroups == 0 || (workgroups >= 8 * n_cb && workgroups <= WG_WGS && workgroups % (8 * n_cb) == 0),
               "patch weight gradient: workgroups must be 0 or a multiple of %d up to %d (got %d)", 8 * n_cb, WG_WGS, workgroups);
-    const int ranges = (workgroups ? workgroups : WG_WGS) / n_cb;
     const int e_rows = embed < WG_E ? embed : WG_E;
     const int wide = patch_dim > embed ? patch_dim : embed;
     const int64_t seg_rows = ((((int64_t)1 << 32) - 1) / ((int64_t)wide * 2)) / WG_BK * WG_BK;
+    const bool drain = mpo_defer_list().n > 0 && patch_dim == 1024 && embed == 256 && total_rows <= seg_rows &&
+                       (workgroups == 0 || workgroups == WG_DRAIN_MAIN);
+    if (mpo_defer_list().n > 0 && !drain) RC(mpo_defer_flush(stream));
+    if (drain) workgroups = WG_DRAIN_MAIN;
+    const int ranges = (workgroups ? workgroups : WG_WGS) / n_cb;
     const __bf16* gb = static_cast<const __bf16*>(g);
     const __bf16* xb = static_cast<const __bf16*>(x);
     for (int64_t s0 = 0; s0 < total_rows; s0 += seg_rows) {
         const int rows = (int)(total_rows - s0 < seg_rows ? total_rows - s0 : seg_rows);
         const int rpr = ((rows + ranges - 1) / ranges + WG_BK - 1) / WG_BK * WG_BK;
         for (int c0 = 0; c0 < embed; c0 += WG_E) {
-            patch_wgrad_kernel<<<ranges * n_cb, WG_WAVES * 64, 0, stream>>>(gb + (size_t)s0 * embed + c0, xb + (size_t)s0 * patch_dim, rows, patch_dim,
-                                                                          embed, e_rows, rpr, part);
+            if (drain) {
+                patch_wgrad_kernel_drain<<<WG_WGS, WG_WAVES * 64, 0, stream>>>(gb, xb, rows, patch_dim, embed, e_rows, rpr, WG_DRAIN_MAIN, part,
+                                                                             mpo_defer_list());
+                mpo_defer_clear();
+            } else {
+                patch_wgrad_kernel<<<ranges * n_cb, WG_WAVES * 64, 0, stream>>>(gb + (size_t)s0 * embed + c0, xb + (size_t)s0 * patch_dim, rows, patch_dim,
+                                                                              embed, e_rows, rpr, part);
+            }
             MPO_LAUNCH_CHECK();
             const int n4 = e_rows * patch_dim / 4;
             patch_wgrad_reduce_kernel<<<(n4 + 255) / 256, 256, 0, stream>>>(part, d_weight + (size_t)c0 * patch_dim, n4, ranges, s0 > 0);
diff --git a/multimodal_path_omic_amd/csrc/tail_api.hip b/multimodal_path_omic_amd/csrc/tail_api.hip
--- a/multimodal_path_omic_amd/csrc/tail_api.hip
+++ b/multimodal_path_omic_amd/csrc/tail_api.hip
@@ -115,11 +115,13 @@
     }
     int launch(hipStream_t s) { return g.n ? mpo_launch_gemm_mixed(g, s) : 0; }
 };
-template <class MkDx, class MkDw> int launch_pairs(int n_branches, hipStream_t stream, MkDx&& mk_dx, MkDw&& mk_dw) {
+inline int add_or_defer(GroupBuilder& g, const GemmArgs& dw) { return mpo_defer_try(dw) ? 0 : g.add(dw); }
+template <class MkDx, class MkDw> int launch_pairs(int n_branches, hipStream_t stream, MkDx&& mk_dx, MkDw&& mk_dw, bool may_defer = true) {
     GroupBuilder g;
     for (int br = 0; br < n_branches; ++br) {
         RC(g.add(mk_dx(br)));
-        RC(g.add(mk_dw(br)));
+        if (may_defer) RC(add_or_defer(g, mk_dw(br)));
+        else RC(g.add(mk_dw(br)));
     }
     return g.launch(stream);
 }
@@ -351,8 +353,8 @@
     auto pairs = [&](auto&& mk_dx, auto&& mk_dw) { return launch_pairs(NB, stream, mk_dx, mk_dw); };
     const size_t h_off = h_interleaved ? (size_t)d : Bd;
     const int h_ld = h_interleaved ? NB * d : d;
-    RC(pairs([&](int br) { GemmArgs m = mpo_args_bwd_input(dh + br * h_off, P(br, 6), dhpool + br * Bd, n_slides, d, d, 1.0f, 0, gate(h + br * h_off, MPO_GATE_RELU, rho_drop_p)); m.lda = h_ld; return m; },
-             [&](int br) { GemmArgs m = mpo_args_bwd_weight(dh + br * h_off, hpool + br * Bd, G(br, 6), G(br, 7), n_slides, d, d, 1.0f, gate(h + br * h_off, MPO_GATE_RELU, rho_drop_p)); m.lda = h_ld; return m; }));
+    RC(launch_pairs(NB, stream, [&](int br) { GemmArgs m = mpo_args_bwd_input(dh + br * h_off, P(br, 6), dhpool + br * Bd, n_slides, d, d, 1.0f, 0, gate(h + br * h_off, MPO_GATE_RELU, rho_drop_p)); m.lda = h_ld; return m; },
+             [&](int br) { GemmArgs m = mpo_args_bwd_weight(dh + br * h_off, hpool + br * Bd, G(br, 6), G(br, 7), n_slides, d, d, 1.0f, gate(h + br * h_off, MPO_GATE_RELU, rho_drop_p)); m.lda = h_ld; return m; }, false));
     if (pool_fuses_scorer(NB, L, d)) {
         PoolScorer ps;
         for (int br = 0; br < NB; ++br) { ps.wc[br] = P(br, 4); ps.bc[br] = P(br, 5); }
@@ -370,8 +372,8 @@
             const GateSpec ga = gate(a + br * Rd, MPO_GATE_TANH, head_drop_p), gb = gate(b + br * Rd, MPO_GATE_SIGMOID, head_drop_p);
             RC(first.add(mpo_args_bwd_input(da + br * Rd, P(br, 0), dx + br * Rd, R, d, d, 1.0f, 1, ga)));
             RC(second.add(mpo_args_bwd_input(db + br * Rd, P(br, 2), dx + br * Rd, R, d, d, 1.0f, 1, gb)));
-            RC(first.add(mpo_args_bwd_weight(da + br * Rd, x + br * Rd, G(br, 0), G(br, 1), R, d, d, 1.0f, ga)));
-            RC(first.add(mpo_args_bwd_weight(db + br * Rd, x + br * Rd, G(br, 2), G(br, 3), R, d, d, 1.0f, gb)));
+            RC(add_or_defer(first, mpo_args_bwd_weight(da + br * Rd, x + br * Rd, G(br, 0), G(br, 1), R, d, d, 1.0f, ga)));
+            RC(add_or_defer(first, mpo_args_bwd_weight(db + br * Rd, x + br * Rd, G(br, 2), G(br, 3), R, d, d, 1.0f, gb)));
             if (pool_fuses_scorer(NB, L, d)) {
                 const float* ds = dscores + (size_t)br * R;
                 GemmArgs m3;
diff --git a/multimodal_path_omic_amd/harness.py b/multimodal_path_omic_amd/harness.py
--- a/multimodal_path_omic_amd/harness.py
+++ b/multimodal_path_omic_amd/harness.py
@@ -87,6 +87,17 @@
 
 def train_window(model, bags: BagBatch, omics, labels, cens, grad_acc_step: int, loss: str = "ces", lambda_reg: float = 0.01,
                  alpha: float = 0.75, l1: float = 0.0, sample_rows: "int | None" = None):
+    from . import ops
+    was = ops.defer_tail_weight_grads
+    ops.defer_tail_weight_grads = not ops.defer_patch_weight_grad
+    try:
+        return _train_window(model, bags, omics, labels, cens, grad_acc_step, loss, lambda_reg, alpha, l1, sample_rows)
+    finally:
+        ops.defer_tail_weight_grads = was
+        ops.flush_tail_weight_grads()
+
+
+def _train_window(model, bags, omics, labels, cens, grad_acc_step, loss, lambda_reg, alpha, l1, sample_rows):
     from . import ops
     bags = sample_window_rows(model, bags, sample_rows)
     if loss == "cesar":
diff --git a/multimodal_path_omic_amd/ops.py b/multimodal_path_omic_amd/ops.py
--- a/multimodal_path_omic_amd/ops.py
+++ b/multimodal_path_omic_amd/ops.py
@@ -254,6 +254,37 @@
         _deferred_patch.append((g, x, dw))
     else:
         patch_weight_grad(g, x, dw)
+
+
+defer_tail_weight_grads = False
+_deferred_tail_keep = []
+
+
+def set_defer_tail_weight_grads(on: bool):
+    global defer_tail_weight_grads
+    defer_tail_weight_grads = bool(on)
+    if not on:
+        flush_tail_weight_grads()
+
+
+def flush_tail_weight_grads():
+    if _deferred_tail_keep:
+        L.call("mpo_deferred_wgrad_flush", torch.cuda.current_stream().cuda_stream)
+        _deferred_tail_keep.clear()
+
+
+def _call_tail_backward(entry, params, grads, operands, *args):
+    on = defer_tail_weight_grads and all(getattr(p, "_mpo_grad_view", None) is not None and g.data_ptr() == p._mpo_grad_view.data_ptr()
+                                         for p, g in zip(params, grads))
+    lib = L.lib()
+    before = lib.mpo_deferred_wgrad_pending()
+    lib.mpo_deferred_wgrad_enable(int(on))
+    try:
+        L.call(entry, *args)
+    finally:
+        lib.mpo_deferred_wgrad_enable(0)
+    if lib.mpo_deferred_wgrad_pending() > before:
+        _deferred_tail_keep.append(operands)
 
 
 class PatchFcFn(torch.autograd.Function):
@@ -331,6 +362,7 @@
         wgs = 0
     L.call("mpo_patch_weight_grad", L.ptr(g), L.ptr(x), g.shape[0], e, k, L.ptr(out), wgs, L.ptr(ws), ws.numel(),
            L.stream_of(g))
+    _deferred_tail_keep.clear()
     return out
 
 
@@ -608,7 +640,7 @@
         ws = _workspace(lib.mpo_encoder_workspace_bytes(branches * n_slides, T, d, ff), x.device)
         pa, ga = L.ptr_array(params), L.ptr_array(grads)
         dy = dy.contiguous()
-        L.call("mpo_encoder_backward",
+        _call_tail_backward("mpo_encoder_backward", ctx.param_refs, grads, (x, saved, dy, ws),
             L.ptr(x), branches, n_slides, T, d, ff, heads, layers, pa, drop_p, seed, off, _epoch(), L.ptr(saved), L.ptr(dy),
             L.ptr(dx), ga, L.ptr(ws), ws.numel(), L.stream_of(x))
         return (dx, None, None, *grads)
@@ -734,7 +766,7 @@
         pa, ga = L.ptr_array(params), L.ptr_array(grads)
         dh = dh.contiguous()
         d_sc = d_scores.contiguous() if d_scores is not None else None
-        L.call("mpo_gated_pool_backward",
+        _call_tail_backward("mpo_gated_pool_backward", ctx.param_refs, grads, (x, saved, h, dh, ws),
             L.ptr(x), branches, n_slides, Lr, d, pa, head_p, rho_p, L.ptr(saved), L.ptr(h), L.ptr(dh), int(ctx.interleave),
             L.ptr(d_sc), L.ptr(dx), ga, L.ptr(ws), ws.numel(), L.stream_of(x))
         return (dx, None, None, None, None, *grads)
```

Result: slower. 23200 slides/s (-19.4%).
